# soldasim/BOSS.jl

Measured on AMD Instinct MI355X. Metric: gp_posterior_updates_per_sec (+ acq_evals_per_sec), N=4096 d=8 fp64, higher is better.
Workload: dtype f64; 1 GPU; d=8 synthetic blackbox, GaussianProcess(Matern52) surrogate, N=4096 fp64 posterior update + ExpectedImprovement over 8192 candidates per GPU (BASELINE.json configs[1]+[2]); N=4096, d=8, M_per_gpu=8192, kernel=matern52, parallelism=single GPU: no exchange

## Files before the change

boss.jl_amd/api.py:

```python
from __future__ import annotations

import ctypes as C
import os
from typing import Optional, Sequence

import numpy as np

_HERE = os.path.dirname(os.path.abspath(__file__))
LIB_PATH = os.environ.get("BOSS_LIB_PATH") or os.path.join(_HERE, "libbosship.so")

BOSS_OK, BOSS_E_INVALID, BOSS_E_NO_DEVICE, BOSS_E_NOT_PD, BOSS_E_NEG_VAR, BOSS_E_NOT_FITTED, BOSS_E_ALLOC = range(7)
KERNELS = {"matern32": 0, "matern52": 1, "sqexp": 2}
FIT_NO_SYNC = 1

_c_dp = C.POINTER(C.c_double)
_c_ucp = C.POINTER(C.c_ubyte)

SIGNATURES = {
    "boss_version": (C.c_char_p, []),
    "boss_last_error": (C.c_char_p, []),
    "boss_device_count": (C.c_int, [C.POINTER(C.c_int)]),
    "boss_set_stream": (C.c_int, [C.c_int, C.c_void_p]),
    "boss_device_sync": (C.c_int, [C.c_int]),
    "boss_gp_create": (C.c_int, [C.c_int, C.c_int, C.c_int, C.c_int, _c_dp, _c_dp, _c_ucp, C.POINTER(C.c_void_p)]),
# ... 1942 lines not shown
    def _set_args(self, gps, Xs, mean_Xs, mean_grad):
        S = len(gps)
        P = len(gps[0]) if S else 0
        if S < 1 or P < 1 or any(len(row) != P for row in gps):
            raise BossError(BOSS_E_INVALID, "gps must be S rows of P posteriors")
        Xs = _f64(Xs, 2)
        du, M = Xs.shape
        dm = self.d_model if self.d_model is not None else du
        arr = (C.c_void_p * (P * S))()
        for s in range(S):
            for p in range(P):
                arr[p + P * s] = gps[s][p]._h
        ms = None if mean_Xs is None else np.ascontiguousarray(np.asarray(mean_Xs, dtype=np.float64).reshape(S, P, M))
        mg = None
        if mean_grad is not None:
            mg = np.ascontiguousarray(np.asarray(mean_grad, dtype=np.float64).reshape(S, P, dm, M).transpose(0, 1, 3, 2))
        return S, P, M, du, arr, Xs, ms, mg

    def predict(self, gps, Xs, mean_Xs=None):
        S, P, M, du, arr, Xs, ms, _ = self._set_args(gps, Xs, mean_Xs, None)
        mu, var = np.zeros((S, P, M)), np.zeros((S, P, M))
        bad = C.c_long(-1)
        try:
            _check(load_library().boss_warp_predict(self._h, P, S, arr, M, _dp(Xs), _dp(ms), _dp(mu), _dp(var), C.byref(bad)))
        except DomainError as e:
            e.bad_index = bad.value
            raise
        return mu, var

    def predict_grad(self, gps, Xs, mean_Xs=None, mean_grad=None):
        S, P, M, du, arr, Xs, ms, mg = self._set_args(gps, Xs, mean_Xs, mean_grad)
        mu, var = np.zeros((S, P, M)), np.zeros((S, P, M))
        dmu, dvar = np.zeros((S, P, M, du)), np.zeros((S, P, M, du))
        bad = C.c_long(-1)
        try:
            _check(load_library().boss_warp_predict_grad(self._h, P, S, arr, M, _dp(Xs), _dp(ms), _dp(mg), _dp(mu), _dp(var), _dp(dmu),
                                                         _dp(dvar), C.byref(bad)))
        except DomainError as e:
            e.bad_index = bad.value
            raise
        return mu, var, dmu.transpose(0, 1, 3, 2), dvar.transpose(0, 1, 3, 2)

    @staticmethod
    def _acq_args(fit_coefs, y_max, valid_mask):
        coefs = _f64(np.asarray(fit_coefs).reshape(-1), 1)
        ym = None if y_max is None else _f64(np.asarray(y_max).reshape(-1), 1)
        mask = None if valid_mask is None else np.ascontiguousarray(np.asarray(valid_mask, dtype=bool).astype(np.uint8))
        return coefs, ym, mask

    def acq_ei(self, gps, Xs, fit_coefs, y_max=None, best=None, valid_mask=None, mean_Xs=None, want_acq: bool = True):
        S, P, M, du, arr, Xs, ms, _ = self._set_args(gps, Xs, mean_Xs, None)
        coefs, ym, mask = self._acq_args(fit_coefs, y_max, valid_mask)
        acq = np.zeros(M) if want_acq else None
        am = C.c_long(-1)
        mx = C.c_double(0.0)
        _check(load_library().boss_acq_ei_warp(self._h, P, S, arr, M, _dp(Xs), _dp(ms), _dp(coefs), _dp(ym), 0 if best is None else 1,
                                               0.0 if best is None else float(best), _ucp(mask), _dp(acq), C.byref(am), C.byref(mx)))
        return acq, am.value, mx.value

    def acq_ei_grad(self, gps, Xs, fit_coefs, y_max=None, best=None, valid_mask=None, mean_Xs=None, mean_grad=None):
        S, P, M, du, arr, Xs, ms, mg = self._set_args(gps, Xs, mean_Xs, mean_grad)
        coefs, ym, mask = self._acq_args(fit_coefs, y_max, valid_mask)
        acq = np.zeros(M)
        dacq = np.zeros((du, M), order="F")
        _check(load_library().boss_acq_ei_grad_warp(self._h, P, S, arr, M, _dp(Xs), _dp(ms), _dp(mg), _dp(coefs), _dp(ym),
                                                    0 if best is None else 1, 0.0 if best is None else float(best), _ucp(mask), _dp(acq),
                                                    _dp(dacq)))
        return acq, dacq

    def workgroup(self, stage: int, n: int, grad: bool, d_model: int = 0):
        lib = load_library()
        lib.boss_debug_warp_block.restype = C.c_int
        lib.boss_debug_warp_block.argtypes = [C.c_void_p, C.c_int, C.c_int, C.c_int, C.c_int, C.POINTER(C.c_int)]
        lds = C.c_int(0)
        return lib.boss_debug_warp_block(self._h, int(stage), 1 if grad else 0, int(n), int(d_model), C.byref(lds)), lds.value

    def close(self):
        if self._h:
            load_library().boss_warp_free(self._h)
            self._h = C.c_void_p()

    def __del__(self):
        try:
            self.close()
        except Exception:
            pass


def init() -> int:
    n = C.c_int(0)
    _check(load_library().boss_init(C.byref(n)))
    return n.value


def comm_info():
    n, r = C.c_int(0), C.c_int(0)
    _check(load_library().boss_comm_info(C.byref(n), C.byref(r)))
    return n.value, bool(r.value)


def shutdown():
    load_library().boss_shutdown()


def multi_update(replicas: Sequence[GP], lengthscale, amplitude, noise_std, mean_X=None) -> float:
    G = len(replicas)
    arr = (C.c_void_p * G)(*[r._h for r in replicas])
    lam = _f64(np.asarray(lengthscale).reshape(-1), 1)
    if lam.shape[0] != replicas[0].d:
        raise BossError(BOSS_E_INVALID, "length(lengthscales) must equal x_dim")
    m = None if mean_X is None else _f64(np.asarray(mean_X).reshape(-1), 1)
    out = C.c_double(0.0)
    _check(load_library().boss_multi_gp_update(G, arr, _dp(lam), float(amplitude), float(noise_std), _dp(m), C.byref(out)))
    for r in replicas:
        r.logpdf = out.value
    return out.value


def _acq_common(P, S, M, fit_coefs, y_max, valid_mask, mean_Xs):
    coefs = _f64(np.asarray(fit_coefs).reshape(-1), 1)
    ym = None if y_max is None else _f64(np.asarray(y_max).reshape(-1), 1)
    mask = None if valid_mask is None else np.ascontiguousarray(np.asarray(valid_mask, dtype=bool).astype(np.uint8))
    ms = None
    if mean_Xs is not None:
        a = np.asarray(mean_Xs, dtype=np.float64).reshape(S, P, M)
        ms = np.ascontiguousarray(a.transpose(0, 2, 1))
    return coefs, ym, mask, ms


def multi_acq_ei(replicas: Sequence[Sequence[Sequence[GP]]], Xs, fit_coefs, y_max=None, best=None, valid_mask=None,
                 mean_Xs=None, want_acq: bool = True):
    G, S, P = len(replicas), len(replicas[0]), len(replicas[0][0])
    Xs = _f64(Xs, 2)
    M = Xs.shape[1]
    arr = (C.c_void_p * (G * S * P))()
    for g in range(G):
        for s in range(S):
            for p in range(P):
                arr[p + P * (s + S * g)] = replicas[g][s][p]._h
    coefs, ym, mask, ms = _acq_common(P, S, M, fit_coefs, y_max, valid_mask, mean_Xs)
    acq = np.zeros(M) if want_acq else None
    am, mx = C.c_long(-1), C.c_double(0.0)
    _check(load_library().boss_multi_acq_ei(G, P, S, arr, M, _dp(Xs), _dp(ms), _dp(coefs), _dp(ym), 0 if best is None else 1,
                                            0.0 if best is None else float(best), _ucp(mask), _dp(acq), C.byref(am), C.byref(mx)))
    return acq, am.value, mx.value


class MultiCandidates:

    def __init__(self, Xs, G: int):
        Xs = _f64(Xs, 2)
        self.d, self.M, self.G = Xs.shape[0], Xs.shape[1], int(G)
        self._h = C.c_void_p()
        _check(load_library().boss_multi_cand_create(self.G, self.d, self.M, _dp(Xs), C.byref(self._h)))

    def close(self):
        if getattr(self, "_h", None) is not None and self._h:
            load_library().boss_multi_cand_free(self._h)
            self._h = None

    def __del__(self):
        try:
            self.close()
        except Exception:
            pass


def multi_acq_ei_cand(replicas: Sequence[Sequence[Sequence[GP]]], cand: MultiCandidates, fit_coefs, y_max=None, best=None,
                      valid_mask=None, mean_Xs=None, want_acq: bool = True):
    G, S, P = len(replicas), len(replicas[0]), len(replicas[0][0])
    M = cand.M
    arr = (C.c_void_p * (G * S * P))()
    for g in range(G):
        for s in range(S):
            for p in range(P):
                arr[p + P * (s + S * g)] = replicas[g][s][p]._h
    coefs, ym, mask, ms = _acq_common(P, S, M, fit_coefs, y_max, valid_mask, mean_Xs)
    acq = np.zeros(M) if want_acq else None
    am, mx = C.c_long(-1), C.c_double(0.0)
    _check(load_library().boss_multi_acq_ei_cand(G, P, S, arr, cand._h, _dp(ms), _dp(coefs), _dp(ym), 0 if best is None else 1,
                                                 0.0 if best is None else float(best), _ucp(mask), _dp(acq), C.byref(am), C.byref(mx)))
    return acq, am.value, mx.value


def _multi_handles(fn_name, gps, Xs, fit_coefs, y_max, best, valid_mask, mean_Xs, want_acq):
    S, P = len(gps), len(gps[0])
    Xs = _f64(Xs, 2)
    M = Xs.shape[1]
    arr = (C.c_void_p * (P * S))()
    for s in range(S):
        for p in range(P):
            arr[p + P * s] = gps[s][p]._h
    coefs, ym, mask, ms = _acq_common(P, S, M, fit_coefs, y_max, valid_mask, mean_Xs)
    acq = np.zeros(M) if want_acq else None
    am, mx = C.c_long(-1), C.c_double(0.0)
    _check(getattr(load_library(), fn_name)(P, S, arr, M, _dp(Xs), _dp(ms), _dp(coefs), _dp(ym), 0 if best is None else 1,
                                            0.0 if best is None else float(best), _ucp(mask), _dp(acq), C.byref(am), C.byref(mx)))
    return acq, am.value, mx.value


def multi_acq_ei_outputs(gps: Sequence[Sequence[GP]], Xs, fit_coefs, y_max=None, best=None, valid_mask=None, mean_Xs=None,
                         want_acq: bool = True):
    return _multi_handles("boss_multi_acq_ei_outputs", gps, Xs, fit_coefs, y_max, best, valid_mask, mean_Xs, want_acq)


def multi_acq_ei_samples(gps: Sequence[Sequence[GP]], Xs, fit_coefs, y_max=None, best=None, valid_mask=None, mean_Xs=None,
                         want_acq: bool = True):
    return _multi_handles("boss_multi_acq_ei_samples", gps, Xs, fit_coefs, y_max, best, valid_mask, mean_Xs, want_acq)


def multi_loglike_batch(G: int, X, y, kernel, lengthscales, amplitudes, noise_stds, mean_X=None, discrete=None):
    X = _f64(X, 2)
    y = _f64(np.asarray(y).reshape(-1), 1)
    lam = _f64(lengthscales, 2)
    d, N = X.shape
    S = lam.shape[1]
    if lam.shape[0] != d:
        raise BossError(BOSS_E_INVALID, "lengthscales must be d×S")
    amp = _f64(np.asarray(amplitudes).reshape(-1), 1)
    sig = _f64(np.asarray(noise_stds).reshape(-1), 1)
    stride, m = 0, None
    if mean_X is not None:
        m = np.asarray(mean_X, dtype=np.float64)
        if m.ndim == 2:
            m, stride = np.ascontiguousarray(m), N
        else:
            m = np.ascontiguousarray(m.reshape(-1))
    disc = None if discrete is None else np.ascontiguousarray(np.asarray(discrete, dtype=bool).astype(np.uint8))
    ll = np.zeros(S)
    st = np.zeros(S, dtype=np.int32)
    _check(load_library().boss_multi_loglike_batch(G, _kernel_id(kernel), d, N, _dp(X), _dp(y), _dp(m), stride, _ucp(disc), S,
                                                   _dp(lam), _dp(amp), _dp(sig), _dp(ll), st.ctypes.data_as(C.POINTER(C.c_int))))
    return ll, st


def bench_mfma_f64(device: int = 0, iters: int = 20000) -> float:
    out = C.c_double(0.0)
    _check(load_library().boss_bench_mfma_f64(device, iters, C.byref(out)))
    return out.value


def prof_enable(device: int, on: bool):
    _check(load_library().boss_prof_enable(device, 1 if on else 0))


def prof_reset(device: int):
    _check(load_library().boss_prof_reset(device))


def prof_get(device: int, kernel_class: str):
    ms = C.c_double(0.0)
    n = C.c_long(0)
    _check(load_library().boss_prof_get(device, kernel_class.encode(), C.byref(ms), C.byref(n)))
    return ms.value, n.value


def _update_path(g: GP):
    lib = load_library()
    fn = lib.boss_debug_update_path
    fn.restype = C.c_int
    fn.argtypes = [C.c_void_p, C.POINTER(C.c_int), C.POINTER(C.c_int), C.POINTER(C.c_int)]
    ch, tm, fb = C.c_int(0), C.c_int(0), C.c_int(0)
    _check(fn(g._h, C.byref(ch), C.byref(tm), C.byref(fb)))
    return ch.value, tm.value, fb.value


def _append_path(g: GP) -> int:
    fn = load_library().boss_debug_append_path
    fn.restype = C.c_int
    fn.argtypes = [C.c_void_p, C.POINTER(C.c_int)]
    out = C.c_int(-1)
    _check(fn(g._h, C.byref(out)))
    return out.value


def _fallbacks(device: int = 0):
    lib = load_library()
    fn = lib.boss_debug_fallbacks
    fn.restype = C.c_int
    fn.argtypes = [C.c_int, C.POINTER(C.c_long), C.POINTER(C.c_int)]
    n, off = C.c_long(0), C.c_int(0)
    _check(fn(device, C.byref(n), C.byref(off)))
    return n.value, off.value


def _set_launches(device: int = 0):
    lib = load_library()
    fn = lib.boss_debug_set_launches
    fn.restype = C.c_int
    fn.argtypes = [C.c_int, C.POINTER(C.c_long), C.POINTER(C.c_long)]
    a, b = C.c_long(0), C.c_long(0)
    fn(device, C.byref(a), C.byref(b))
    return a.value, b.value


def _set_grad_launches(device: int = 0):
    lib = load_library()
    fn = lib.boss_debug_set_grad_launches
    fn.restype = C.c_int
    fn.argtypes = [C.c_int, C.POINTER(C.c_long)]
    a = C.c_long(0)
    fn(device, C.byref(a))
    return a.value
```

boss.jl_amd/csrc/bosship.hip:

```cpp
#include "../../include/bosship.h"

#include <hip/hip_runtime.h>

#include <algorithm>
#include <cmath>
#include <cstdint>
#include <cstdio>
#include <cstdlib>
#include <atomic>
#include <chrono>
#include <cstring>
#include <functional>
#include <limits>
#include <map>
#include <mutex>
#include <string>
#include <thread>
#include <vector>

#include "gp_kernels.hpp"
#include "potrf.hpp"
#include "chain.hpp"
#include "small_calls.hpp"
#include "rider.hpp"
#include "latent_kernels.hpp"
#include "nfit_kernels.hpp"
#include "fitness.hpp"
#include "mean_program.hpp"
#include "warp_kernels.hpp"

using namespace boss;

#ifndef BOSS_PRED_D
#define BOSS_PRED_D 10
#endif
typedef GemmDirect<4, 1, 4, 2, BOSS_PRED_D> PredG32;
typedef GemmDirect<4, 1, 2, 4, 4> PredG64;

static thread_local std::string g_last_error;
static int fail(int code, const std::string& msg) {
    g_last_error = msg;
    return code;
}
#define HIPCHK(expr)                                                                                     \
    do {                                                                                                 \
        hipError_t e_ = (expr);                                                                          \
        if (e_ != hipSuccess)                                                                            \
            return fail(e_ == hipErrorOutOfMemory ? BOSS_E_ALLOC : BOSS_E_NO_DEVICE,                     \
                        std::string(#expr) + ": " + hipGetErrorString(e_));                              \
    } while (0)

constexpr size_t PINNED_UP_OFF = 4096, PINNED_UP_BYTES = 1024 * 1024, PINNED_DOWN_OFF = PINNED_UP_OFF + PINNED_UP_BYTES,
                 PINNED_DOWN_BYTES = 512 * 1024, PINNED_BYTES = PINNED_DOWN_OFF + PINNED_DOWN_BYTES;

static bool release_cached_slabs();
static std::atomic<int> g_fail_allocs{0};
static hipError_t dev_malloc(void** p, size_t bytes) {
    static const bool poison = getenv("BOSS_POISON_ALLOC") && atoi(getenv("BOSS_POISON_ALLOC"));
    hipError_t e = hipErrorOutOfMemory;
    if (g_fail_allocs.load(std::memory_order_relaxed) > 0 && g_fail_allocs.fetch_sub(1) > 0) *p = nullptr;
    else e = hipMalloc(p, bytes);
    if (e != hipSuccess) (void)hipGetLastError();
    if (e != hipSuccess && release_cached_slabs()) {
        e = hipMalloc(p, bytes);
        if (e != hipSuccess) (void)hipGetLastError();
    }
    if (e == hipSuccess && poison) {
        (void)hipMemset(*p, 0xff, bytes);
        (void)hipDeviceSynchronize();
    }
    return e;
}

constexpr size_t MULTI_RES_OFF = 384;
constexpr size_t FEW_RES_OFF = 400;

struct Workspace {
    void* p = nullptr;
    size_t bytes = 0;
};

struct Ctx {
    int device = -1;
    int logical = -1;
    hipStream_t own_stream = nullptr;
    hipStream_t stream = nullptr;
    hipStream_t side_stream = nullptr;
    std::vector<hipEvent_t> ev_panel, ev_rest;
    hipEvent_t ev_fork = nullptr, ev_up = nullptr;
    unsigned long long* sig_panel = nullptr;
    unsigned long long* sig_panel_host = nullptr;
    unsigned long long sig_seq = 0;
    hipStream_t chain_stream = nullptr, strip_stream = nullptr;
    unsigned long long chain_seq = 0, crit_seq = 0, up_seq = 0;
    int n_cus = 256;
    bool chain_ok = false;
    bool test_drop_chain = false;
    unsigned long long acq_seq = 0;
    unsigned long long few_seq = 0;
    std::mutex slab_mtx;
    void* slab_cache = nullptr;
    size_t slab_cache_bytes = 0;
    void* hostblk_cache = nullptr;
    size_t hostblk_cache_bytes = 0;
    unsigned long long* few_done = nullptr;
    unsigned long long few_done_cnt = 0;
    long set_launches = 0, set_pre_launches = 0;
    long set_grad_launches = 0;
    bool lookahead = true;
    bool prof_on = false;
    std::map<std::string, std::vector<std::pair<hipEvent_t, hipEvent_t>>> prof;
    std::vector<hipEvent_t> ev_pool;
    Workspace vscratch, csc, pred, acq, batchA, batchX, batchMisc, craw, lgA, lgB, lgC, few, setdesc, setmom, gsetdesc, nlatjobs, mceps, meanws, warpws;
    static constexpr int LLG_BANKS = 4;
    Workspace lgbank[LLG_BANKS - 1][3];
    hipStream_t llg_stream[LLG_BANKS - 1] = {nullptr, nullptr, nullptr};
    hipEvent_t llg_join[LLG_BANKS - 1] = {nullptr, nullptr, nullptr};
    void* pinned = nullptr;
    struct TrailTab {
        TrailWork* dev = nullptr;
        std::vector<TrailWork> host;
        std::vector<int> off;
    };
    TrailTab trail[65];
    std::mutex mtx;
};

static void chain_quiesce(Ctx* c) {
    if (c->chain_stream) (void)hipStreamSynchronize(c->chain_stream);
    if (c->strip_stream) (void)hipStreamSynchronize(c->strip_stream);
}

static std::mutex g_ctx_mtx;
static std::map<int, Ctx*> g_ctx;

static bool release_cached_slabs() {
    int dev = -1;
    if (hipGetDevice(&dev) != hipSuccess) return false;
    std::vector<void*> blocks;
    {
        std::lock_guard<std::mutex> lk(g_ctx_mtx);
        for (auto& kv : g_ctx) {
            Ctx* c = kv.second;
            if (c->device != dev) continue;
            std::lock_guard<std::mutex> sl(c->slab_mtx);
            if (c->slab_cache) blocks.push_back(c->slab_cache);
            c->slab_cache = nullptr;
            c->slab_cache_bytes = 0;
        }
    }
    for (void* b : blocks) (void)hipFree(b);
    return !blocks.empty();
}
extern "C" int boss_debug_fail_next_alloc(int n) {
    g_fail_allocs.store(n > 0 ? n : 0);
    return BOSS_OK;
}
extern "C" int boss_debug_slab_cache_bytes(int device, size_t* bytes_out) {
    std::lock_guard<std::mutex> lk(g_ctx_mtx);
    auto it = g_ctx.find(device);
    if (bytes_out) *bytes_out = 0;
    if (it != g_ctx.end() && bytes_out) {
        std::lock_guard<std::mutex> sl(it->second->slab_mtx);
        *bytes_out = it->second->slab_cache_bytes;
    }
    return BOSS_OK;
}

extern "C" int boss_debug_set_launches(int device, long* all_out, long* pre_out) {
    std::lock_guard<std::mutex> lk(g_ctx_mtx);
    auto it = g_ctx.find(device);
    if (all_out) *all_out = it != g_ctx.end() ? it->second->set_launches : 0;
    if (pre_out) *pre_out = it != g_ctx.end() ? it->second->set_pre_launches : 0;
    return BOSS_OK;
}

extern "C" int boss_debug_set_grad_launches(int device, long* out) {
    std::lock_guard<std::mutex> lk(g_ctx_mtx);
    auto it = g_ctx.find(device);
    if (out) *out = it != g_ctx.end() ? it->second->set_grad_launches : 0;
    return BOSS_OK;
}

static void ctx_destroy(Ctx* c) {
    if (!c) return;
    if (c->own_stream) (void)hipStreamDestroy(c->own_stream);
    if (c->side_stream) (void)hipStreamDestroy(c->side_stream);
    if (c->chain_stream) (void)hipStreamDestroy(c->chain_stream);
    if (c->strip_stream) (void)hipStreamDestroy(c->strip_stream);
    if (c->ev_fork) (void)hipEventDestroy(c->ev_fork);
    if (c->sig_panel && !c->sig_panel_host) (void)hipFree(c->sig_panel);
    if (c->few_done) (void)hipFree(c->few_done);
    for (auto& t : c->trail)
        if (t.dev) (void)hipFree(t.dev);
    if (c->slab_cache) (void)hipFree(c->slab_cache);
    if (c->hostblk_cache) (void)hipHostFree(c->hostblk_cache);
    if (c->ev_up) (void)hipEventDestroy(c->ev_up);
    for (int i = 0; i < Ctx::LLG_BANKS - 1; ++i) {
        if (c->llg_stream[i]) (void)hipStreamDestroy(c->llg_stream[i]);
        if (c->llg_join[i]) (void)hipEventDestroy(c->llg_join[i]);
    }
    if (c->pinned) (void)hipHostFree(c->pinned);
    delete c;
}

static int ctx_init(Ctx* c) {
    {
        int least = 0, greatest = 0;
        (void)hipDeviceGetStreamPriorityRange(&least, &greatest);
        static const int cu_mask = getenv("BOSS_CU_MASK") ? atoi(getenv("BOSS_CU_MASK")) : 0;
        if (cu_mask) {
            hipDeviceProp_t prop;
            HIPCHK(hipGetDeviceProperties(&prop, c->device));
            const int ncu = prop.multiProcessorCount, words = (ncu + 31) / 32;
            auto make = [&](hipStream_t* st, int lo, int hi) {
                std::vector<uint32_t> m(words, 0u);
                for (int b = lo; b < hi && b < ncu; ++b) m[b / 32] |= 1u << (b % 32);
                return hipExtStreamCreateWithCUMask(st, (uint32_t)words, m.data());
            };
            HIPCHK(make(&c->chain_stream, 0, 16));
            HIPCHK(make(&c->strip_stream, 16, 32));
            HIPCHK(make(&c->own_stream, 32, ncu));
            HIPCHK(make(&c->side_stream, cu_mask >= 2 ? 40 : 32, cu_mask >= 2 ? ncu : ncu - 8));
            c->stream = c->own_stream;
            std::fprintf(stderr, "[bosship] BOSS_CU_MASK=%d: chain on CU bits 0-15, strips on 16-31, main stream on 32-%d, side stream %d-%d\n",
                         cu_mask, ncu - 1, cu_mask >= 2 ? 40 : 32, (cu_mask >= 2 ? ncu : ncu - 8) - 1);
        } else {
        HIPCHK(hipStreamCreateWithPriority(&c->own_stream, hipStreamNonBlocking, greatest));
        c->stream = c->own_stream;
        HIPCHK(hipStreamCreateWithPriority(&c->side_stream, hipStreamNonBlocking, least));
        HIPCHK(hipStreamCreateWithPriority(&c->chain_stream, hipStreamNonBlocking, greatest));
        HIPCHK(hipStreamCreateWithPriority(&c->strip_stream, hipStreamNonBlocking, greatest));
        }
    }
    HIPCHK(hipEventCreateWithFlags(&c->ev_fork, hipEventDisableTiming));
    HIPCHK(hipEventCreateWithFlags(&c->ev_up, hipEventDisableTiming));
    for (int i = 0; i < Ctx::LLG_BANKS - 1; ++i) {
        HIPCHK(hipStreamCreateWithFlags(&c->llg_stream[i], hipStreamNonBlocking));
        HIPCHK(hipEventCreateWithFlags(&c->llg_join[i], hipEventDisableTiming));
    }
    c->lookahead = !(getenv("BOSS_NO_LOOKAHEAD") && atoi(getenv("BOSS_NO_LOOKAHEAD")));
    {
        auto set_nonzero = [](const char* name) {
            const char* v = getenv(name);
            return v && *v && std::strcmp(v, "0") != 0;
        };
        static const bool gate_off = set_nonzero("BOSS_NO_GATE") || set_nonzero("ROCPROF_COUNTER_COLLECTION") || getenv("ROCPROF_COUNTERS") ||
                                     getenv("ROCPROF_COUNTER_GROUPS") || set_nonzero("ROCPROF_ADVANCED_THREAD_TRACE") ||
                                     getenv("ROCPROF_ATT_PARAM_SERIALIZE_ALL") || getenv("ROCP_METRICS") || set_nonzero("AMD_SERIALIZE_KERNEL");
        if (!gate_off) {
            if (set_nonzero("BOSS_DEBUG_WATCH")) {
                unsigned long long* hp = nullptr;
                HIPCHK(hipHostMalloc((void**)&hp, SIG_WORDS * sizeof(unsigned long long), hipHostMallocMapped));
                std::memset(hp, 0, SIG_WORDS * sizeof(unsigned long long));
                HIPCHK(hipHostGetDevicePointer((void**)&c->sig_panel, hp, 0));
                c->sig_panel_host = hp;
#ifdef BOSS_DEBUG_WATCH_BUILD
                HIPCHK(hipMemcpyToSymbol(HIP_SYMBOL(boss::g_dbg), &c->sig_panel, sizeof(void*)));
#endif
                std::thread([hp]() {
                    unsigned long long last[SIG_WORDS] = {0};
                    for (;;) {
                        std::this_thread::sleep_for(std::chrono::milliseconds(500));
                        unsigned long long now[SIG_WORDS];
                        for (int i = 0; i < SIG_WORDS; ++i) now[i] = ((volatile unsigned long long*)hp)[i];
                        if (std::memcmp(now, last, sizeof now) == 0) continue;
                        std::memcpy(last, now, sizeof now);
                        std::fprintf(stderr, "[bosship watch] up %llu wdone %llu panel %llu crit %llu | gate %llu near %llu bulk %llu | strips",
                                     now[SIGW_UP], now[SIGW_WDONE], now[SIGW_PANEL], now[SIGW_CRIT], now[SIGW_GATE], now[SIGW_NEAR], now[SIGW_BULK]);
                        for (int q = 0; q < 8; ++q) std::fprintf(stderr, " %llu", now[SIGW_PROG + SIGW_PROG_STRIDE * q]);
                        std::fprintf(stderr, " | give-ups: first %llu n %llu last %llu; waits ended by mark %llu, by clock %llu", now[SIGW_DBG], now[SIGW_DBG + 1],
                                     now[SIGW_DBG + 2], now[SIGW_DBG + 4], now[SIGW_DBG + 5]);
                        std::fprintf(stderr, "\n");
                    }
                }).detach();
            } else {
                HIPCHK(hipMalloc((void**)&c->sig_panel, SIG_WORDS * sizeof(unsigned long long)));
                HIPCHK(hipMemset(c->sig_panel, 0, SIG_WORDS * sizeof(unsigned long long)));
            }
        }
        c->chain_ok = !gate_off && !set_nonzero("BOSS_NO_CHAIN") && !set_nonzero("HIP_LAUNCH_BLOCKING");
        c->test_drop_chain = set_nonzero("BOSS_TEST_DROP_CHAIN");
        if (c->chain_ok) {
            int* okw = nullptr;
            HIPCHK(hipMalloc((void**)&okw, 4 * sizeof(int)));
            HIPCHK(hipMemset(okw, 0, 4 * sizeof(int)));
            hipStream_t probed[4] = {c->own_stream, c->side_stream, c->chain_stream, c->strip_stream};
            for (int i = 0; i < 4; ++i)
                hipLaunchKernelGGL(chain_probe_wait_kernel, dim3(1), dim3(64), 0, probed[i], c->sig_panel + SIGW_NEAR + 1, 4ull, okw + i);
            int okh[4] = {0, 0, 0, 0};
            bool fine = hipDeviceSynchronize() == hipSuccess && hipMemcpy(okh, okw, sizeof okh, hipMemcpyDeviceToHost) == hipSuccess;
            (void)hipFree(okw);
            if (!(fine && okh[0] && okh[1] && okh[2] && okh[3])) c->chain_ok = false;
            if (getenv("BOSS_CHAIN_VERBOSE"))
                std::fprintf(stderr, "[bosship] resident chain: %s (main / side / chain / strip streams side by side: %d %d %d %d)\n",
                             c->chain_ok ? "on" : "off", okh[0], okh[1], okh[2], okh[3]);
        }
    }
    HIPCHK(hipHostMalloc(&c->pinned, PINNED_BYTES, hipHostMallocDefault));
    std::memset(c->pinned, 0, PINNED_UP_OFF);
    HIPCHK(hipFuncSetAttribute((const void*)potrf_diag_kernel, hipFuncAttributeMaxDynamicSharedMemorySize, DIAG_LDS_BYTES));
    HIPCHK(hipFuncSetAttribute((const void*)potrf_chain_kernel, hipFuncAttributeMaxDynamicSharedMemorySize, CHAIN_LDS_BYTES));
    HIPCHK(hipFuncSetAttribute((const void*)potrf_strips_kernel, hipFuncAttributeMaxDynamicSharedMemorySize, STRIPS_LDS_BYTES));
    {
        int cus = 0;
        if (hipDeviceGetAttribute(&cus, hipDeviceAttributeMultiprocessorCount, c->device) != hipSuccess) cus = 0;
        if (cus > 0) c->n_cus = cus;
    }
    HIPCHK(hipFuncSetAttribute((const void*)small_fit_kernel, hipFuncAttributeMaxDynamicSharedMemorySize, SMALL_LDS_BYTES));
    HIPCHK(hipFuncSetAttribute((const void*)small_llgrad_kernel, hipFuncAttributeMaxDynamicSharedMemorySize, SMALL_LLG_LDS_BYTES));
    HIPCHK(hipFuncSetAttribute((const void*)small_fit_batch_kernel, hipFuncAttributeMaxDynamicSharedMemorySize, SMALL_LDS_BYTES));
    HIPCHK(hipFuncSetAttribute((const void*)small_predict_grad_kernel<true>, hipFuncAttributeMaxDynamicSharedMemorySize, SPG_LDS_BYTES));
    HIPCHK(hipFuncSetAttribute((const void*)small_predict_grad_kernel<false>, hipFuncAttributeMaxDynamicSharedMemorySize, SPG_LDS_BYTES));
    HIPCHK(hipFuncSetAttribute((const void*)potrf_syrk_kernel<2, true>, hipFuncAttributeMaxDynamicSharedMemorySize, 96 * 1024));
    HIPCHK(hipFuncSetAttribute((const void*)rider_step_kernel, hipFuncAttributeMaxDynamicSharedMemorySize, 96 * 1024));
    HIPCHK(hipFuncSetAttribute((const void*)predict_kernel<PredG32>, hipFuncAttributeMaxDynamicSharedMemorySize,
                               PredictLds<PredG32>::BYTES));
    HIPCHK(hipFuncSetAttribute((const void*)predict_kernel_set<PredG32>, hipFuncAttributeMaxDynamicSharedMemorySize,
                               PredictLds<PredG32>::BYTES));
    HIPCHK(hipFuncSetAttribute((const void*)grad_accum_kernel, hipFuncAttributeMaxDynamicSharedMemorySize, 150 * 1024));
    HIPCHK(hipFuncSetAttribute((const void*)winv_gemv_kernel<1>, hipFuncAttributeMaxDynamicSharedMemorySize, 150 * 1024));
    HIPCHK(hipFuncSetAttribute((const void*)winv_gemv_kernel<2>, hipFuncAttributeMaxDynamicSharedMemorySize, 150 * 1024));
    HIPCHK(hipFuncSetAttribute((const void*)winv_gemv_kernel<4>, hipFuncAttributeMaxDynamicSharedMemorySize, 150 * 1024));
    HIPCHK(hipFuncSetAttribute((const void*)winv_args_kernel<1>, hipFuncAttributeMaxDynamicSharedMemorySize, 150 * 1024));
    HIPCHK(hipFuncSetAttribute((const void*)winv_args_kernel<2>, hipFuncAttributeMaxDynamicSharedMemorySize, 150 * 1024));
    HIPCHK(hipFuncSetAttribute((const void*)winv_args_kernel<4>, hipFuncAttributeMaxDynamicSharedMemorySize, 150 * 1024));
    HIPCHK(hipFuncSetAttribute((const void*)winv_args_kernel<1, true>, hipFuncAttributeMaxDynamicSharedMemorySize, 150 * 1024));
    HIPCHK(hipFuncSetAttribute((const void*)few_back_finish_kernel<PredG32>, hipFuncAttributeMaxDynamicSharedMemorySize,
                               PredictLds<PredG32>::BYTES));
    HIPCHK(hipFuncSetAttribute((const void*)few_w_kernel<PredG32>, hipFuncAttributeMaxDynamicSharedMemorySize, PredictLds<PredG32>::BYTES));
    HIPCHK(hipFuncSetAttribute((const void*)few_finish_kernel<PredG32>, hipFuncAttributeMaxDynamicSharedMemorySize,
                               PredictLds<PredG32>::BYTES));
    HIPCHK(hipFuncSetAttribute((const void*)linvt_kernel<PredG32>, hipFuncAttributeMaxDynamicSharedMemorySize,
                               PredictLds<PredG32>::BYTES));
    HIPCHK(hipFuncSetAttribute((const void*)backsolve_kernel<PredG32>, hipFuncAttributeMaxDynamicSharedMemorySize,
                               PredictLds<PredG32>::BYTES));
    HIPCHK(hipFuncSetAttribute((const void*)backsolve_set_kernel<PredG32>, hipFuncAttributeMaxDynamicSharedMemorySize,
                               PredictLds<PredG32>::BYTES));
    HIPCHK(hipFuncSetAttribute((const void*)grad_accum_set_kernel, hipFuncAttributeMaxDynamicSharedMemorySize, 150 * 1024));
    HIPCHK(hipFuncSetAttribute((const void*)predict_kernel<PredG64>, hipFuncAttributeMaxDynamicSharedMemorySize,
                               PredictLds<PredG64>::BYTES));
    HIPCHK(hipFuncSetAttribute((const void*)predict_kernel<PredG32, true>, hipFuncAttributeMaxDynamicSharedMemorySize,
                               PredictLds<PredG32>::BYTES));
    HIPCHK(hipFuncSetAttribute((const void*)predict_kernel<PredG64, true>, hipFuncAttributeMaxDynamicSharedMemorySize,
                               PredictLds<PredG64>::BYTES));
    HIPCHK(hipFuncSetAttribute((const void*)ei_mc_grad_set_kernel, hipFuncAttributeMaxDynamicSharedMemorySize, MC_GRAD_MAX_LDS));
    HIPCHK(hipFuncSetAttribute((const void*)mean_eval_kernel<true>, hipFuncAttributeMaxDynamicSharedMemorySize, MEAN_MAX_LDS));
    return BOSS_OK;
}

static int virtual_devices() {
    static const int v = getenv("BOSS_VIRTUAL_DEVICES") ? std::max(0, atoi(getenv("BOSS_VIRTUAL_DEVICES"))) : 0;
    return v;
}
static int visible_devices(int* nphys_out = nullptr) {
    int n = 0;
    if (hipGetDeviceCount(&n) != hipSuccess || n <= 0) return 0;
    if (nphys_out) *nphys_out = n;
    return virtual_devices() > 0 ? virtual_devices() : n;
}

static int get_ctx(int device, Ctx** out) {
    std::lock_guard<std::mutex> lk(g_ctx_mtx);
    auto it = g_ctx.find(device);
    if (it != g_ctx.end()) {
        *out = it->second;
        HIPCHK(hipSetDevice(it->second->device));
        return BOSS_OK;
    }
    int nphys = 0;
    const int n = visible_devices(&nphys);
    if (n <= 0) return fail(BOSS_E_NO_DEVICE, "no HIP device visible (bosship has no CPU fallback)");
    if (device < 0 || device >= n) return fail(BOSS_E_INVALID, "device index out of range");
    const int phys = device % nphys;
    HIPCHK(hipSetDevice(phys));
    Ctx* c = new Ctx();
    c->device = phys;
    c->logical = device;
    int rc = ctx_init(c);
    if (rc) {
        ctx_destroy(c);
        return rc;
    }
    g_ctx[device] = c;
    *out = c;
    return BOSS_OK;
}

static int ws_reserve(Workspace& w, size_t bytes) {
    if (w.bytes >= bytes) return BOSS_OK;
    if (w.p) (void)hipFree(w.p);
    w.p = nullptr;
    w.bytes = 0;
    HIPCHK(dev_malloc(&w.p, bytes));
    w.bytes = bytes;
    return BOSS_OK;
}

struct ProfScope {
    Ctx* c;
    hipEvent_t e0 = nullptr, e1 = nullptr;
    const char* name;
    ProfScope(Ctx* ctx, const char* n) : c(ctx), name(n) {
        if (!c->prof_on) return;
        e0 = take();
        e1 = take();
        (void)hipEventRecord(e0, c->stream);
    }
    ~ProfScope() {
        if (!c->prof_on) return;
        (void)hipEventRecord(e1, c->stream);
        c->prof[name].push_back({e0, e1});
    }
    hipEvent_t take() {
        if (!c->ev_pool.empty()) {
            hipEvent_t e = c->ev_pool.back();
            c->ev_pool.pop_back();
            return e;
        }
        hipEvent_t e;
        (void)hipEventCreate(&e);
        return e;
    }
};

struct boss_gpset {
    Ctx* ctx = nullptr;
    std::atomic<int> refs{0};
    void* slab = nullptr;
    void* host_block = nullptr;
    size_t slab_bytes = 0, host_bytes = 0;
};
static bool slab_cache_on() {
    static const bool v = !(getenv("BOSS_SLAB_CACHE") && atoi(getenv("BOSS_SLAB_CACHE")) == 0) &&
                          !(getenv("BOSS_POISON_ALLOC") && atoi(getenv("BOSS_POISON_ALLOC")));
    return v;
}
static void gpset_release_storage(boss_gpset* st) {
    Ctx* c = st->ctx;
    void *slab = st->slab, *hb = st->host_block;
    if (c && slab_cache_on()) {
        std::lock_guard<std::mutex> lk(c->slab_mtx);
        if (slab && st->slab_bytes > c->slab_cache_bytes) {
            std::swap(slab, c->slab_cache);
            c->slab_cache_bytes = st->slab_bytes;
        }
        if (hb && st->host_bytes > c->hostblk_cache_bytes) {
            std::swap(hb, c->hostblk_cache);
            c->hostblk_cache_bytes = st->host_bytes;
        }
    }
    if (slab) (void)hipFree(slab);
    if (hb) (void)hipHostFree(hb);
    st->slab = st->host_block = nullptr;
}

struct boss_gp {
    Ctx* ctx = nullptr;
    boss_gpset* set = nullptr;
    int kernel = 0, d = 0, N = 0, Np = 0, nblk = 0, ld = 0;
    double *Xraw = nullptr, *Xsc = nullptr, *y = nullptr, *mean = nullptr, *A = nullptr;
    double *LT = nullptr, *DT2 = nullptr, *avec = nullptr;
    bool have_lt = false;
    double *inv16 = nullptr, *Dinv = nullptr, *Dinv2 = nullptr, *hyp = nullptr, *invlam = nullptr, *scal = nullptr;
    int* info = nullptr;
    unsigned char* discrete_dev = nullptr;
    std::vector<unsigned char> discrete;
    double amp2 = 0.0;
    bool has_mean = false, fitted = false, pending = false, have_dinv = false;
    bool dinv_used = false;
    bool dinv_used_prev = false;
    bool gated = false;
    bool chained = false;
    bool fell_back = false;
    int trail_used = -1;
    double* host_res = nullptr;
    double* host_res_dev = nullptr;
    bool par_in_args = false;
    unsigned long long res_seq = 0;
    bool res_polled = false;
    double* host_par = nullptr;
    hipEvent_t par_ev = nullptr;
    unsigned long long epoch = 0;
    unsigned long long factor_gen = 0, dinv0_gen = ~0ull;
    hipEvent_t dinv_ev = nullptr;
    bool dinv_pending = false;
    bool aug = false;
    int npts = 0, ldx = 0, nhead = 0;
    bool gibbs = false;
    double *lamX = nullptr, *ampX = nullptr, *noiseX = nullptr;
    double *Winv = nullptr, *Linv = nullptr;
    double* W2 = nullptr;
    int w2_np = 0;
    unsigned long long w2_gen = ~0ull;
    bool w2_used = false;
    bool have_winv = false;
    int few_calls = 0;
    int append_calls = 0;
    int append_path = 0;
};

struct boss_cand {
    Ctx* ctx = nullptr;
    int d = 0, M = 0, Mp = 0;
    double* Craw = nullptr;
};

struct boss_track {
    Ctx* ctx = nullptr;
    boss_gp* gp = nullptr;
    int d = 0, M = 0, Mp = 0, tiles = 0, Ncap = 0, N = 0;
    unsigned long long epoch = 0;
    double *V = nullptr, *Csc = nullptr, *mu = nullptr, *var = nullptr, *mean = nullptr;
    bool has_mean = false;
    bool gibbs = false;
    double *Clam = nullptr, *Camp = nullptr;
    bool aug = false;
};

static inline int round_up(int x, int m) { return (x + m - 1) / m * m; }
struct SetBatch {
    int nb = 1;
    size_t sA = 0, sInv16 = 0, sDinv = 0, sDinv2 = 0, sW = 0, sX = 0;
    size_t sPar = 0;
};
struct MeanFold {
    const double* J = nullptr;
    size_t sJ = 0;
    int T = 0;
    double* dmean = nullptr;
    double* dtheta = nullptr;
};
static void linv_enqueue(boss_gp* g, hipStream_t s, double* U, double* Lw, const SetBatch& B = SetBatch());
constexpr int MAX_ROWS = 46080;

extern "C" const char* boss_version(void) { return "bosship 0.1.0 (gfx950, fp64 MFMA)"; }
extern "C" const char* boss_last_error(void) { return g_last_error.c_str(); }

extern "C" int boss_device_count(int* n_out) {
    const int n = visible_devices();
    hipError_t e = n > 0 ? hipSuccess : hipErrorNoDevice;
    if (e != hipSuccess || n <= 0) {
        if (n_out) *n_out = 0;
        return fail(BOSS_E_NO_DEVICE, "no HIP device visible (bosship has no CPU fallback)");
    }
    if (n_out) *n_out = n;
    return BOSS_OK;
}

extern "C" int boss_set_stream(int device, void* hip_stream) {
    Ctx* c;
    int rc = get_ctx(device, &c);
    if (rc) return rc;
    std::lock_guard<std::mutex> lk(c->mtx);
    HIPCHK(hipStreamSynchronize(c->stream));
    c->stream = hip_stream ? (hipStream_t)hip_stream : c->own_stream;
    return BOSS_OK;
}

extern "C" int boss_device_sync(int device) {
    Ctx* c;
    int rc = get_ctx(device, &c);
    if (rc) return rc;
    HIPCHK(hipStreamSynchronize(c->stream));
    return BOSS_OK;
}

static bool few_done_ensure(Ctx* c, hipStream_t s) {
    if (c->few_done) return true;
    if (hipMalloc((void**)&c->few_done, sizeof(unsigned long long)) != hipSuccess) {
        (void)hipGetLastError();
        c->few_done = nullptr;
        return false;
    }
    (void)hipMemsetAsync(c->few_done, 0, sizeof(unsigned long long), s);
    c->few_done_cnt = 0;
    return true;
}
static bool few_fused() {
    static const bool v = !(getenv("BOSS_FEW_FUSED") && atoi(getenv("BOSS_FEW_FUSED")) == 0);
    return v;
}

#include "host_factor.inc"
#include "host_append.inc"
#include "host_batch.inc"
#include "host_latent.inc"
#include "host_nfit.inc"
struct McEpi {
    const FitProg* g;
    int n_eps;
    const double* eps;
};
static int mc_stage(Ctx* c, hipStream_t s, int P, const McEpi& mc, const double** deps_out);
static void mc_accumulate_launch(hipStream_t s, const double* mu, const double* var, size_t sstride, int ldm, int M, int s0, int s1, int S_total,
                                 const EiPar& par, const McEpi& mc, const double* deps, double* acq_sum, int add);
static void mc_grad_launch(hipStream_t s, const double* mu, const double* var, const double* dmu, const double* dvar, int M, int d, int S,
                           const EiPar& par, const McEpi& mc, const double* deps, const unsigned char* mask, double* acq, double* dacq);
#include "host_predict.inc"
#include "host_acq.inc"
#include "host_fitness.inc"
#include "host_mean.inc"
#include "host_warp.inc"
#include "host_rider.inc"
#include "host_track.inc"
#include "host_multi.inc"

extern "C" int boss_bench_mfma_f64(int device, int iters, double* tflops_out) {
    Ctx* c;
    int rc = get_ctx(device, &c);
    if (rc) return rc;
    hipDeviceProp_t prop;
    HIPCHK(hipGetDeviceProperties(&prop, device));
    const int blocks = prop.multiProcessorCount;
    double* sink;
    HIPCHK(dev_malloc((void**)&sink, 8));
    hipEvent_t e0, e1;
    HIPCHK(hipEventCreate(&e0));
    HIPCHK(hipEventCreate(&e1));
    hipLaunchKernelGGL(mfma_f64_rate_kernel, dim3(blocks), dim3(256), 0, c->stream, iters / 8 + 1, sink);
    HIPCHK(hipEventRecord(e0, c->stream));
    hipLaunchKernelGGL(mfma_f64_rate_kernel, dim3(blocks), dim3(256), 0, c->stream, iters, sink);
    HIPCHK(hipEventRecord(e1, c->stream));
    HIPCHK(hipEventSynchronize(e1));
    float ms = 0.f;
    HIPCHK(hipEventElapsedTime(&ms, e0, e1));
    const double flops = (double)blocks * 4.0 * (double)iters * 16.0 * 2048.0;
    if (tflops_out) *tflops_out = flops / (ms * 1e-3) / 1e12;
    (void)hipEventDestroy(e0);
    (void)hipEventDestroy(e1);
    (void)hipFree(sink);
    return BOSS_OK;
}

extern "C" int boss_prof_enable(int device, int on) {
    Ctx* c;
    int rc = get_ctx(device, &c);
    if (rc) return rc;
    c->prof_on = on != 0;
    return BOSS_OK;
}

extern "C" int boss_prof_reset(int device) {
    Ctx* c;
    int rc = get_ctx(device, &c);
    if (rc) return rc;
    HIPCHK(hipStreamSynchronize(c->stream));
    for (auto& kv : c->prof)
        for (auto& pr : kv.second) {
            c->ev_pool.push_back(pr.first);
            c->ev_pool.push_back(pr.second);
        }
    c->prof.clear();
    return BOSS_OK;
}

extern "C" int boss_prof_get(int device, const char* kernel_class, double* ms_total, long* launches) {
    Ctx* c;
    int rc = get_ctx(device, &c);
    if (rc) return rc;
    if (!kernel_class) return fail(BOSS_E_INVALID, "kernel_class is NULL");
    HIPCHK(hipStreamSynchronize(c->stream));
    double tot = 0.0;
    long n = 0;
    auto it = c->prof.find(kernel_class);
    if (it != c->prof.end()) {
        for (auto& pr : it->second) {
            float ms = 0.f;
            if (hipEventElapsedTime(&ms, pr.first, pr.second) == hipSuccess) tot += ms;
            ++n;
        }
    }
    if (ms_total) *ms_total = tot;
    if (launches) *launches = n;
    return BOSS_OK;
}

extern "C" int boss_debug_colupd_decode(int G, int k, int m, int ncols, int jfirst, int skipdiag, int xblk, int critical,
                                        int* R0, int* C0, int* crit) {
    if (G < 1 || !R0 || !C0 || !crit) return fail(BOSS_E_INVALID, "bad argument");
    for (int t = 0; t < G; ++t) {
        const ColupdWork w = colupd_decode(t, G, k, m, ncols, jfirst, skipdiag, xblk, critical != 0);
        R0[t] = w.R0;
        C0[t] = w.C0;
        crit[t] = w.crit;
    }
    return BOSS_OK;
}

extern "C" int boss_debug_trail_plan(int nblk, int panels, int lag, int* n_items, int* off, int* items, int cap) {
    if (nblk < 2 || nblk > 64 || panels < 1 || panels > 8 || lag < 1 || lag > 8 || !n_items || !off) return fail(BOSS_E_INVALID, "bad argument");
    std::vector<TrailWork> plan;
    std::vector<int> o;
    trail_plan(nblk, panels, lag, plan, o);
    *n_items = (int)plan.size();
    for (int k = 0; k < nblk; ++k) off[k] = o[k];
    if (!items) return BOSS_OK;
    if (cap < (int)plan.size()) return fail(BOSS_E_INVALID, "cap too small");
    for (size_t t = 0; t < plan.size(); ++t) {
        const TrailWork& w = plan[t];
        int* it = items + 5 * t;
        it[0] = w.R0;
        it[1] = w.C0;
        it[2] = w.k0;
        it[3] = w.npc & 255;
        it[4] = w.npc >> 8;
    }
    return BOSS_OK;
}

extern "C" int boss_debug_update_path(const boss_gp* g, int* chained, int* trail_mode, int* fell_back) {
    if (!g || !chained || !trail_mode || !fell_back) return fail(BOSS_E_INVALID, "bad argument");
    *chained = g->chained ? 1 : 0;
    *trail_mode = g->chained ? g->trail_used : -1;
    *fell_back = g->fell_back ? 1 : 0;
    return BOSS_OK;
}

#ifdef BOSS_CHAIN_TRACE
extern "C" int boss_debug_ctrace(unsigned long long* chain , unsigned long long* colupd , int reset) {
    if (hipDeviceSynchronize() != hipSuccess) return 1;
    if (chain && hipMemcpyFromSymbol(chain, HIP_SYMBOL(boss::g_ctrace), sizeof(unsigned long long) * 64 * 16) != hipSuccess) return 1;
    if (colupd && hipMemcpyFromSymbol(colupd, HIP_SYMBOL(boss::g_cutrace), sizeof(unsigned long long) * 64 * 4) != hipSuccess) return 1;
    if (colupd && hipMemcpyFromSymbol(colupd + 64 * 4, HIP_SYMBOL(boss::g_ptrace), sizeof(unsigned long long) * 64 * 32) != hipSuccess) return 1;
    if (reset) {
        static unsigned long long a[64 * 16], b[64 * 4];
        for (int i = 0; i < 64; ++i) {
            for (int j = 0; j < 16; ++j) a[i * 16 + j] = (j == 5) ? ~0ull : 0ull;
            b[i * 4 + 0] = ~0ull;
            b[i * 4 + 1] = b[i * 4 + 2] = b[i * 4 + 3] = 0;
        }
        (void)hipMemcpyToSymbol(HIP_SYMBOL(boss::g_ctrace), a, sizeof a);
        (void)hipMemcpyToSymbol(HIP_SYMBOL(boss::g_cutrace), b, sizeof b);
    }
    return 0;
}
extern "C" int boss_debug_rtrace(unsigned long long* rider , int reset) {
    if (hipDeviceSynchronize() != hipSuccess) return 1;
    if (rider && hipMemcpyFromSymbol(rider, HIP_SYMBOL(boss::g_rtrace), sizeof(unsigned long long) * 64 * 4) != hipSuccess) return 1;
    if (reset) {
        static unsigned long long a[64 * 4];
        for (int i = 0; i < 64; ++i) {
            a[i * 4 + 0] = ~0ull;
            a[i * 4 + 1] = a[i * 4 + 2] = a[i * 4 + 3] = 0;
        }
        (void)hipMemcpyToSymbol(HIP_SYMBOL(boss::g_rtrace), a, sizeof a);
    }
    return 0;
}
#endif
```

boss.jl_amd/csrc/host_acq.inc:

```

static int acq_ei_impl(int P, int S, boss_gp_t* const* gps, const boss_cand_t* cand, const double* mean_Xs,
                       const double* fit_coefs, const double* y_max, int has_best, double best,
                       const unsigned char* valid_mask, double* acq_out, long* argmax_out, double* max_out,
                       double* dpair, long idx_off, bool defer, const McEpi* mc = nullptr) {
    if (P < 1 || S < 1 || !gps || !cand || (!fit_coefs && !mc)) return fail(BOSS_E_INVALID, "bad arguments");
    Ctx* c = cand->ctx;
    HIPCHK(hipSetDevice(c->device));
    for (int i = 0; i < P * S; ++i) {
        if (!gps[i]) return fail(BOSS_E_INVALID, "NULL posterior handle");
        if (gps[i]->ctx != c) return fail(BOSS_E_INVALID, "all handles and candidates must live on one device");
        if (!gps[i]->fitted) return fail(BOSS_E_NOT_FITTED, "handle has no valid factorisation");
    }
    std::lock_guard<std::mutex> lk(c->mtx);
    hipStream_t s = c->stream;
    const int M = cand->M;
    const size_t nd = (size_t)3 * P * M + M + 2 * P;
    {
        int rc = ws_reserve(c->acq, sizeof(double) * nd + M);
        if (rc) return rc;
    }
    double* dev = (double*)c->acq.p;
    double* dmu = dev;
    double* dvar = dmu + (size_t)P * M;
    double* dacq = dvar + (size_t)P * M;
    double* dmean = dacq + M;
    double* dcoef = dmean + (size_t)P * M;
    double* dymax = dcoef + P;
    unsigned char* dmask = (unsigned char*)(dev + nd);
    double* hres = (double*)c->pinned + (defer ? MULTI_RES_OFF : 0);
    EiPar par;
    const double no_coefs[EI_MAXP] = {};
    int rc = ei_params(c, s, P, mc ? no_coefs : fit_coefs, y_max, has_best, best, &par, dcoef, dymax);
    if (rc) return rc;
    const double* deps = nullptr;
    if (mc) {
        rc = mc_stage(c, s, P, *mc, &deps);
        if (rc) return rc;
    }
    EiPar par0 = par;
    par0.mode = 0;
    if (valid_mask) (void)hipMemcpyAsync(dmask, valid_mask, M, hipMemcpyHostToDevice, s);
    if (S > 1) (void)hipMemsetAsync(dacq, 0, sizeof(double) * M, s);
    std::vector<double> hmean;
    static const bool set_off = getenv("BOSS_NO_SET_PREDICT") && atoi(getenv("BOSS_NO_SET_PREDICT"));
    if (S > 1 && par.mode != 0 && !set_off && predict_set_ok(P * S, gps, cand)) {
        const size_t pm = (size_t)P * M;
        rc = ws_reserve(c->setmom, sizeof(double) * pm * S * (mean_Xs ? 3 : 2));
        if (rc) return rc;
        double* mu_all = (double*)c->setmom.p;
        double* var_all = mu_all + pm * S;
        double* mean_all = mean_Xs ? var_all + pm * S : nullptr;
        if (mean_Xs) {
            hmean.resize(pm * S);
            for (int sm = 0; sm < S; ++sm)
                for (int j = 0; j < M; ++j)
                    for (int p = 0; p < P; ++p) hmean[pm * sm + (size_t)p * M + j] = mean_Xs[p + (size_t)P * (j + (size_t)M * sm)];
            (void)hipMemcpyAsync(mean_all, hmean.data(), sizeof(double) * pm * S, hipMemcpyHostToDevice, s);
            (void)hipStreamSynchronize(s);
        }
        rc = predict_set_enqueue(P * S, gps, cand, mean_all, mu_all, var_all, (size_t)M);
        if (rc) {
            (void)hipStreamSynchronize(s);
            return rc;
        }
        if (mc) mc_accumulate_launch(s, mu_all, var_all, pm, M, M, 0, S, S, par, *mc, deps, dacq, 0);
        else
        hipLaunchKernelGGL(ei_accumulate_set_kernel, dim3((M + 255) / 256), dim3(256), 0, s, (const double*)mu_all, (const double*)var_all, pm, M, M,
                           0, S - 1, par, dcoef, dymax, dacq);
        hipLaunchKernelGGL(acq_epilogue_kernel, dim3(1), dim3(ACQ_EPI_THREADS), 0, s, (const double*)(mu_all + pm * (S - 1)),
                           (const double*)(var_all + pm * (S - 1)), M, M, mc ? par0 : par, dcoef, dymax, dacq, 1, 1.0 / S, valid_mask ? dmask : nullptr, hres,
                           (acq_out || defer) ? 0ull : ++c->acq_seq, dpair, idx_off);
    } else
    for (int sm = 0; sm < S; ++sm) {
        if (par.mode != 0) {
            if (mean_Xs) {
                hmean.resize((size_t)P * M);
                for (int j = 0; j < M; ++j)
                    for (int p = 0; p < P; ++p) hmean[(size_t)p * M + j] = mean_Xs[p + (size_t)P * (j + (size_t)M * sm)];
                (void)hipMemcpyAsync(dmean, hmean.data(), sizeof(double) * P * M, hipMemcpyHostToDevice, s);
                (void)hipStreamSynchronize(s);
            }
            for (int p = 0; p < P; ++p) {
                rc = predict_enqueue(gps[p + (size_t)P * sm], cand, mean_Xs ? dmean + (size_t)p * M : nullptr,
                                     dmu + (size_t)p * M, dvar + (size_t)p * M);
                if (rc) {
                    (void)hipStreamSynchronize(s);
                    return rc;
                }
            }
        }
        ProfScope ps(c, sm + 1 < S ? "ei" : "argmax");
        if (mc) {
            mc_accumulate_launch(s, dmu, dvar, 0, M, M, 0, 1, S, par, *mc, S > 1 ? deps + (size_t)sm * P : deps, dacq, sm > 0 ? 1 : 0);
            if (sm + 1 == S)
                hipLaunchKernelGGL(acq_epilogue_kernel, dim3(1), dim3(ACQ_EPI_THREADS), 0, s, dmu, dvar, M, M, par0, dcoef, dymax, dacq, 1, 1.0 / S,
                                   valid_mask ? dmask : nullptr, hres, (acq_out || defer) ? 0ull : ++c->acq_seq, dpair, idx_off);
        } else if (sm + 1 < S)
            hipLaunchKernelGGL(ei_accumulate_kernel, dim3((M + 255) / 256), dim3(256), 0, s, dmu, dvar, M, M, par, dcoef, dymax,
                               dacq);
        else
            hipLaunchKernelGGL(acq_epilogue_kernel, dim3(1), dim3(ACQ_EPI_THREADS), 0, s, dmu, dvar, M, M, par, dcoef, dymax,
                               dacq, S > 1 ? 1 : 0, 1.0 / S, valid_mask ? dmask : nullptr, hres, (acq_out || defer) ? 0ull : ++c->acq_seq,
                               dpair, idx_off);
    }
    if (acq_out) (void)hipMemcpyAsync(acq_out, dacq, sizeof(double) * M, hipMemcpyDeviceToHost, s);
    if (defer) {
        hipError_t e0 = hipGetLastError();
        return e0 == hipSuccess ? BOSS_OK : fail(BOSS_E_NO_DEVICE, hipGetErrorString(e0));
    }
    bool got = false;
    if (!acq_out) {
        volatile unsigned long long* seq = reinterpret_cast<volatile unsigned long long*>(hres) + 2;
        for (unsigned long i = 1;; ++i) {
            if (*seq == c->acq_seq) {
                got = true;
                break;
            }
            if ((i & 0x3fff) == 0 && hipStreamQuery(s) != hipErrorNotReady) break;
        }
        std::atomic_thread_fence(std::memory_order_acquire);
    }
    hipError_t e = got ? hipSuccess : hipStreamSynchronize(s);
    hipError_t e2 = hipGetLastError();
    if (e != hipSuccess) return fail(BOSS_E_NO_DEVICE, hipGetErrorString(e));
    if (e2 != hipSuccess) return fail(BOSS_E_NO_DEVICE, hipGetErrorString(e2));
    if (argmax_out) std::memcpy(argmax_out, &hres[1], sizeof(long));
    if (max_out) *max_out = hres[0];
    return BOSS_OK;
}

extern "C" int boss_acq_ei(int P, int S, boss_gp_t* const* gps, const boss_cand_t* cand, const double* mean_Xs,
                           const double* fit_coefs, const double* y_max, int has_best, double best,
                           const unsigned char* valid_mask, double* acq_out, long* argmax_out, double* max_out) {
    return acq_ei_impl(P, S, gps, cand, mean_Xs, fit_coefs, y_max, has_best, best, valid_mask, acq_out, argmax_out, max_out, nullptr, 0, false);
}

extern "C" int boss_acq_ei_moments(int device, int P, int S, int M, const double* mu, const double* var,
                                   const double* fit_coefs, const double* y_max, int has_best, double best,
                                   const unsigned char* valid_mask, double* acq_out, long* argmax_out,
                                   double* max_out) {
    if (P < 1 || S < 1 || M < 1 || !mu || !var || !fit_coefs) return fail(BOSS_E_INVALID, "bad arguments");
    Ctx* c;
    int rc = get_ctx(device, &c);
    if (rc) return rc;
    HIPCHK(hipSetDevice(c->device));
    std::lock_guard<std::mutex> lk(c->mtx);
    hipStream_t s = c->stream;
    const size_t pm = (size_t)P * M;
    const size_t nd = 2 * pm * S + M + 2 * P;
    rc = ws_reserve(c->acq, sizeof(double) * nd + M);
    if (rc) return rc;
    double* dev = (double*)c->acq.p;
    double* dmu = dev;
    double* dvar = dmu + pm * S;
    double* dacq = dvar + pm * S;
    double* dcoef = dacq + M;
    double* dymax = dcoef + P;
    unsigned char* dmask = (unsigned char*)(dev + nd);
    double* hres = (double*)c->pinned;
    EiPar par;
    rc = ei_params(c, s, P, fit_coefs, y_max, has_best, best, &par, dcoef, dymax);
    if (rc) return rc;
    (void)hipMemcpyAsync(dmu, mu, sizeof(double) * pm * S, hipMemcpyHostToDevice, s);
    (void)hipMemcpyAsync(dvar, var, sizeof(double) * pm * S, hipMemcpyHostToDevice, s);
    if (valid_mask) (void)hipMemcpyAsync(dmask, valid_mask, M, hipMemcpyHostToDevice, s);
    if (S > 1) (void)hipMemsetAsync(dacq, 0, sizeof(double) * M, s);
    for (int sm = 0; sm + 1 < S; ++sm)
        hipLaunchKernelGGL(ei_accumulate_kernel, dim3((M + 255) / 256), dim3(256), 0, s, dmu + pm * sm, dvar + pm * sm, M, M, par,
                           dcoef, dymax, dacq);
    hipLaunchKernelGGL(acq_epilogue_kernel, dim3(1), dim3(ACQ_EPI_THREADS), 0, s, dmu + pm * (S - 1), dvar + pm * (S - 1), M, M,
                       par, dcoef, dymax, dacq, S > 1 ? 1 : 0, 1.0 / S, valid_mask ? dmask : nullptr, hres, 0ull);
    if (acq_out) (void)hipMemcpyAsync(acq_out, dacq, sizeof(double) * M, hipMemcpyDeviceToHost, s);
    hipError_t e = hipStreamSynchronize(s);
    if (e != hipSuccess) return fail(BOSS_E_NO_DEVICE, hipGetErrorString(e));
    if (argmax_out) std::memcpy(argmax_out, &hres[1], sizeof(long));
    if (max_out) *max_out = hres[0];
    return BOSS_OK;
}

static int llgrad_enqueue(boss_gp* g, hipStream_t s, double* sums_out, int bank, const SetBatch& B, const double* amp2_dev,
                          int amp2_stride, const MeanFold* mf) {
    Ctx* c = g->ctx;
    const int d = g->d, N = g->N, Np = g->Np, ld = g->ld, nb = B.nb;
    const int nt = Np / 64, ntiles = nt * (nt + 1) / 2, nv = g->aug ? d + 3 : d + 2, nch = 8;
    const int gibbs_js = std::max(1, std::min(16, Np / 64));
    const size_t sW = (size_t)ld * Np,
                 sC = (size_t)nch * Np + (g->gibbs ? (size_t)gibbs_js * 4 * (d + 1) * Np : (size_t)ntiles * nv);
    Workspace &wA = bank ? c->lgbank[bank - 1][0] : c->lgA, &wB = bank ? c->lgbank[bank - 1][1] : c->lgB,
              &wC = bank ? c->lgbank[bank - 1][2] : c->lgC;
    int rc = ws_reserve(wA, sizeof(double) * sW * nb);
    if (rc) return rc;
    rc = ws_reserve(wB, sizeof(double) * sW * nb);
    if (rc) return rc;
    rc = ws_reserve(wC, sizeof(double) * sC * nb);
    if (rc) return rc;
    double* LinvT = (double*)wA.p;
    double* Kinv = (double*)wB.p;
    double* apart = (double*)wC.p;
    double* parts = apart + (size_t)nch * Np;
    SetBatch Bw = B;
    Bw.sW = nb > 1 ? sW : 0;
    dinv_join(g);
    if (!g->have_dinv) {
        dinv_launch(g, s, B);
        g->have_dinv = true;
    }
    g->dinv_used = true;
    typedef PredG32 G;
    static const bool linvt_solve = getenv("BOSS_LINVT_SOLVE") && atoi(getenv("BOSS_LINVT_SOLVE"));
    if (linvt_solve && nb == 1) {
        hipLaunchKernelGGL(linvt_kernel<G>, dim3(Np / 32), dim3(G::NTHREADS), PredictLds<G>::BYTES, s, (const double*)g->A, ld, Np,
                           (const double*)g->Dinv2, LinvT, ld);
    } else {
        linv_enqueue(g, s, LinvT, Kinv, Bw);
    }
    hipLaunchKernelGGL(kinv_syrk_kernel<SyrkG>, dim3(g->nblk * (g->nblk + 1) / 2, 1, nb), dim3(256), 0, s, (const double*)LinvT, ld, Np,
                       Kinv, ld, Bw.sW);
    hipLaunchKernelGGL(avec_partial_kernel, dim3(Np / 256, nch, nb), dim3(256), 0, s, (const double*)LinvT, ld, Np, N,
                       (const double*)g->A, ld, apart, Bw.sW, B.sA, nb > 1 ? sC : (size_t)0);
    if (mf && (mf->dmean || (mf->dtheta && mf->T > 0))) {
        const int T = mf->dtheta ? mf->T : 0;
        hipLaunchKernelGGL(mean_fold_kernel, dim3(std::max(1, (T + MFOLD_COLS - 1) / MFOLD_COLS), 1, nb), dim3(MFOLD_THREADS), 0, s,
                           (const double*)apart, nch, Np, N, T ? mf->J : (const double*)nullptr, T, mf->dmean, T ? mf->dtheta : (double*)nullptr,
                           nb > 1 ? sC : (size_t)0, mf->sJ);
    }
    const size_t zC = nb > 1 ? sC : (size_t)0, zPar = nb > 1 ? B.sPar : (size_t)0;
    if (g->gibbs) {
        hipLaunchKernelGGL(mirror_lower_kernel, dim3(Np / 64, Np / 64, nb), dim3(256), 0, s, Kinv, ld, Np, Bw.sW);
        hipLaunchKernelGGL(mirror_diag_kernel, dim3(Np / 64, 1, nb), dim3(256), 0, s, Kinv, ld, Bw.sW);
        hipLaunchKernelGGL(gibbs_llgrad_kernel, dim3(Np / 64, gibbs_js, nb), dim3(256), 0, s, (const double*)g->Xraw, (const double*)g->lamX,
                           (const double*)g->ampX, d, N, Np, (const double*)Kinv, ld, (const double*)apart, nch, parts, zPar, Bw.sW, zC);
        hipLaunchKernelGGL(gibbs_llgrad_reduce_kernel, dim3((Np + 255) / 256, 1, nb), dim3(256), 0, s, (const double*)parts, gibbs_js * 4, d, N,
                           Np, (const double*)g->noiseX, (const double*)Kinv, ld, (const double*)apart, nch, sums_out, zPar, Bw.sW, zC,
                           nb > 1 ? (size_t)(d + 3) * Np : (size_t)0);
        return BOSS_OK;
    }
    if (g->aug)
        hipLaunchKernelGGL(aug_llgrad_tile_kernel, dim3(ntiles, 1, nb), dim3(256), 0, s, (const double*)g->Xraw, g->ldx, d, g->nhead, N, Np,
                           g->kernel, (const double*)g->hyp, (const double*)g->invlam, zPar, (const double*)Kinv, ld, (const double*)apart, nch,
                           parts, Bw.sW, zC);
    else
    hipLaunchKernelGGL(llgrad_tile_kernel, dim3(ntiles, 1, nb), dim3(256), 0, s, (const double*)g->Xsc, d, N, Np, g->kernel, amp2_dev,
                       amp2_stride, (const double*)Kinv, ld, (const double*)apart, nch, parts, B.sX, Bw.sW, nb > 1 ? sC : (size_t)0,
                       nb > 1 ? sC : (size_t)0);
    hipLaunchKernelGGL(llgrad_reduce_kernel, dim3(nv, 1, nb), dim3(256), 0, s, (const double*)parts, ntiles, nv, sums_out,
                       nb > 1 ? sC : (size_t)0, (size_t)nv);
    return BOSS_OK;
}

static void llgrad_finalize(int d, int N, const double* invlam, double amp2, double sig2, double zz, const double* h, double* grad_out) {
    const double amp = std::sqrt(amp2), sig = std::sqrt(sig2), trK = h[d], aa = h[d + 1];
    for (int m = 0; m < d; ++m) grad_out[m] = -h[m] * invlam[m];
    grad_out[d] = (zz - N - sig2 * (aa - trK)) / amp;
    grad_out[d + 1] = sig * (aa - trK);
}

static int llgrad_download(boss_gp* g, std::vector<double>& h, size_t n_mean = 0) {
    Ctx* c = g->ctx;
    hipStream_t s = c->stream;
    int rc = ws_reserve(c->pred, sizeof(double) * h.size());
    if (rc) return rc;
    double* sums = (double*)c->pred.p;
    MeanFold mf;
    if (n_mean) mf.dmean = sums + (h.size() - n_mean);
    rc = llgrad_enqueue(g, s, sums, 0, SetBatch(), g->gibbs ? (const double*)nullptr : (const double*)g->hyp, 0, n_mean ? &mf : nullptr);
    if (rc) return rc;
    HIPCHK(hipMemcpyAsync(h.data(), sums, sizeof(double) * h.size(), hipMemcpyDeviceToHost, s));
    HIPCHK(hipStreamSynchronize(s));
    HIPCHK(hipGetLastError());
    return BOSS_OK;
}

extern "C" int boss_gp_loglike_grad(boss_gp_t* g, double* logpdf_out, double* grad_out) {
    if (!g || !grad_out) return fail(BOSS_E_INVALID, "NULL argument");
    NOT_FOR_AUG(g);
    Ctx* c = g->ctx;
    HIPCHK(hipSetDevice(c->device));
    std::lock_guard<std::mutex> lk(c->mtx);
    int rc = gp_settle(g);
    if (rc) return rc;
    const int d = g->d, nv = d + 2;
    if (d > LLG_MAX_D) return fail(BOSS_E_INVALID, "x_dim too large for the likelihood-gradient kernel");
    hipStream_t s = c->stream;
    if (small_fit_ok(c, g->N, d) && !g->gibbs) {
        dinv_join(g);
        hipLaunchKernelGGL(small_llgrad_kernel, dim3(1), dim3(DIAG_THREADS), SMALL_LLG_LDS_BYTES, s, (const double*)g->A, g->ld, g->Np,
                           g->N, d, g->kernel, g->amp2, (const double*)g->inv16, (const double*)g->Xsc, g->ldx, g->host_res_dev + 8, (size_t)0, (size_t)0,
                           (size_t)0, (const double*)nullptr, 0, 0, ++g->res_seq, (const double*)nullptr, 0, (size_t)0, (double*)nullptr,
                           (double*)nullptr);
        HIPCHK(hipGetLastError());
        {
            volatile unsigned long long* seq = reinterpret_cast<volatile unsigned long long*>(g->host_res + 7);
            bool got = false;
            for (unsigned long i = 1;; ++i) {
                if (*seq == g->res_seq) {
                    got = true;
                    break;
                }
                if ((i & 0x3fff) == 0 && hipStreamQuery(s) != hipErrorNotReady) break;
            }
            std::atomic_thread_fence(std::memory_order_acquire);
            if (!got) HIPCHK(hipStreamSynchronize(s));
        }
        llgrad_finalize(d, g->N, g->host_par, g->host_par[d], g->host_par[d + 1], g->host_res[1], g->host_res + 8, grad_out);
        if (logpdf_out) *logpdf_out = loglik(g->N, g->host_res[0], g->host_res[1]);
        return BOSS_OK;
    }
    std::vector<double> h(nv);
    rc = llgrad_download(g, h);
    if (rc) return rc;
    llgrad_finalize(d, g->N, g->host_par, g->host_par[d], g->host_par[d + 1], g->host_res[1], h.data(), grad_out);
    if (logpdf_out) *logpdf_out = loglik(g->N, g->host_res[0], g->host_res[1]);
    return BOSS_OK;
}

extern "C" int boss_gp_loglike_grad_mean(boss_gp_t* g, double* logpdf_out, double* grad_out, double* dmean_out) {
    if (!g || !grad_out || !dmean_out) return fail(BOSS_E_INVALID, "NULL argument");
    NOT_FOR_AUG(g);
    Ctx* c = g->ctx;
    HIPCHK(hipSetDevice(c->device));
    std::lock_guard<std::mutex> lk(c->mtx);
    int rc = gp_settle(g);
    if (rc) return rc;
    const int d = g->d, nv = d + 2, N = g->N;
    if (d > LLG_MAX_D) return fail(BOSS_E_INVALID, "x_dim too large for the likelihood-gradient kernel");
    hipStream_t s = c->stream;
    std::vector<double> h((size_t)nv + N);
    if (small_fit_ok(c, N, d)) {
        rc = ws_reserve(c->pred, sizeof(double) * h.size());
        if (rc) return rc;
        double* sums = (double*)c->pred.p;
        dinv_join(g);
        hipLaunchKernelGGL(small_llgrad_kernel, dim3(1), dim3(DIAG_THREADS), SMALL_LLG_LDS_BYTES, s, (const double*)g->A, g->ld, g->Np, N, d,
                           g->kernel, g->amp2, (const double*)g->inv16, (const double*)g->Xsc, g->ldx, sums, (size_t)0, (size_t)0, (size_t)0,
                           (const double*)nullptr, 0, 0, 0ull, (const double*)nullptr, 0, (size_t)0, sums + nv, (double*)nullptr);
        HIPCHK(hipGetLastError());
        HIPCHK(hipMemcpyAsync(h.data(), sums, sizeof(double) * h.size(), hipMemcpyDeviceToHost, s));
        HIPCHK(hipStreamSynchronize(s));
    } else {
        rc = llgrad_download(g, h, (size_t)N);
        if (rc) return rc;
    }
    llgrad_finalize(d, N, g->host_par, g->host_par[d], g->host_par[d + 1], g->host_res[1], h.data(), grad_out);
    std::copy(h.begin() + nv, h.end(), dmean_out);
    if (logpdf_out) *logpdf_out = loglik(N, g->host_res[0], g->host_res[1]);
// ... 53 lines not shown
```

boss.jl_amd/csrc/host_factor.inc:

```


struct LaunchStamps {
    static constexpr int CAP = 512;
    int n = 0;
    int tag[CAP];
    std::chrono::steady_clock::time_point t[CAP];
    void reset() { n = 0; }
    void add(int what) {
        if (n < CAP) {
            tag[n] = what;
            t[n++] = std::chrono::steady_clock::now();
        }
    }
};
static std::atomic<int> g_stamps_on{-1};
static std::atomic<long long> g_stall_us{2500};
static std::mutex g_stall_mtx;
static std::string g_stall_log;
static bool launch_stamps_on() {
    int v = g_stamps_on.load(std::memory_order_relaxed);
    if (v < 0) {
        v = (getenv("BOSS_LAUNCH_STAMPS") && atoi(getenv("BOSS_LAUNCH_STAMPS"))) ? 1 : 0;
        if (getenv("BOSS_STALL_MS")) g_stall_us.store((long long)(atof(getenv("BOSS_STALL_MS")) * 1000.0));
        g_stamps_on.store(v);
// ... 173 lines not shown
    p.cbase = c->chain_seq;
    c->chain_seq += 8ull * nblk + 16;
    p.critbase = c->crit_seq;
    c->crit_seq += 8ull * (nblk - 2);
#ifdef BOSS_EXPERIMENTS
    static const bool drop_chain = getenv("BOSS_EXP_DROP_CHAIN") && atoi(getenv("BOSS_EXP_DROP_CHAIN"));
#else
    constexpr bool drop_chain = false;
#endif
    if (!(drop_chain || c->test_drop_chain)) {
        const unsigned budget = poll_budget_ticks(Np);
        hipLaunchKernelGGL(potrf_chain_kernel, dim3(2), dim3(DIAG_THREADS), CHAIN_LDS_BYTES, c->chain_stream, A, ld, nblk, inv16, info, c->sig_panel,
                           p.cbase, p.critbase, budget);
        hipLaunchKernelGGL(potrf_strips_kernel, dim3(8), dim3(TRSM_THREADS), STRIPS_LDS_BYTES, c->strip_stream, A, ld, nblk, (const double*)inv16,
                           c->sig_panel, p.cbase, p.critbase, info, budget);
        c->up_seq += 2 + 8;
        p.up_want = c->up_seq;
    }
    return p;
}
static void chain_ready(Ctx* c, const ChainPlan& p, int Np, int* info) {
    if (!p.on || c->test_drop_chain) return;
    static const int force = getenv("BOSS_CHAIN_READY") ? atoi(getenv("BOSS_CHAIN_READY")) : -1;
    const int followers = (Np - 2 * BLK) / 16 + 1;
    const bool need = followers + 16 > c->n_cus;
    if (force == 0 || (force < 0 && !need)) return;
    hipLaunchKernelGGL(chain_ready_kernel, dim3(1), dim3(64), 0, c->stream, c->sig_panel, p.up_want, info, poll_budget_ticks(Np));
}
static void potrf_enqueue(Ctx* c, double* A, int ld, int Np, int batch, size_t bstride, double* inv16,
                          size_t inv16_bstride, int* info, bool gates = true, const ChainPlan* plan = nullptr,
                          const std::function<void(int)>* step_hook = nullptr) {
    const int nblk = Np / BLK;
    hipStream_t s = c->stream;
    const unsigned budget = poll_budget_ticks(Np);
    if (Np > 8192) gates = false;
    static const int pair_min_batch = getenv("BOSS_PAIR_MIN_BATCH") ? atoi(getenv("BOSS_PAIR_MIN_BATCH")) : 4;
    static const int la_batch_max = getenv("BOSS_LA_BATCH_MAX") ? atoi(getenv("BOSS_LA_BATCH_MAX")) : 8;
    const bool la_batch = batch <= la_batch_max && c->lookahead && !c->prof_on && nblk >= 3;
    if (batch >= pair_min_batch && nblk >= 3 && !la_batch) {
        for (int k = 0; k < nblk; k += 2) {
            for (int kk = k; kk < k + 2 && kk < nblk; ++kk) {
                {
                    ProfScope ps(c, "potrf_diag");
                    hipLaunchKernelGGL(potrf_diag_kernel, dim3(1, 1, batch), dim3(DIAG_THREADS), DIAG_LDS_BYTES, s, A, ld, bstride,
                                       kk, inv16, inv16_bstride, info, (unsigned long long*)nullptr, 0ull);
                }
                const int nrows16 = (Np - (kk + 1) * BLK) / 16 + 1;
                {
                    ProfScope ps(c, "potrf_trsm");
                    hipLaunchKernelGGL(potrf_trsm_kernel, dim3(nrows16, 1, batch), dim3(TRSM_THREADS), 0, s, A, ld, bstride, kk, inv16,
                                       inv16_bstride, (kk + 1) * BLK);
                }
                const int m = nblk - 1 - kk;
                if (kk == k && m > 0) {
                    ProfScope ps(c, "potrf_syrk");
                    hipLaunchKernelGGL(potrf_colupd_kernel, dim3(4 * m + 1, 1, batch), dim3(256), 0, s, A, ld, bstride, kk, m, 1, 0, 1, (unsigned long long*)nullptr, 0ull, info, 0, -1, (unsigned long long*)nullptr, budget);
                }
            }
            const int m2 = nblk - (k + 2);
            if (m2 > 0) {
                ProfScope ps(c, "potrf_syrk");
                hipLaunchKernelGGL(potrf_syrk_kernel<2>, dim3((m2 * (m2 + 1) / 2 + m2) * batch, 1, 1), dim3(256), 0, s, A, ld, bstride,
                                   k, k + 2, m2, batch);
            } else if (m2 == 0 && k + 1 < nblk) {
            }
        }
        return;
    }
    const bool la = c->lookahead && !c->prof_on && nblk >= 3;
    if (la) {
        while ((int)c->ev_panel.size() < nblk) {
            hipEvent_t e0, e1;
            (void)hipEventCreateWithFlags(&e0, hipEventDisableTiming);
            (void)hipEventCreateWithFlags(&e1, hipEventDisableTiming);
            c->ev_panel.push_back(e0);
            c->ev_rest.push_back(e1);
        }
    }
    const int small_m = sched_small_m();
    const bool no_pairs = sched_no_pairs();
    const bool chain = plan && plan->on;
    const unsigned long long cbase = chain ? plan->cbase : 0;
    unsigned long long* const critw = chain ? c->sig_panel + SIGW_CRIT : nullptr;
    auto launch_follow = [&](int kk, unsigned long long gateval) {
        const int row0 = std::min((kk + 2) * BLK, Np);
        const int nrows16 = (Np - row0) / 16 + 1;
        hipLaunchKernelGGL(potrf_follow_kernel, dim3(nrows16), dim3(TRSM_THREADS), 0, s, A, ld, kk, (const double*)inv16, row0,
                           kk + 1 < nblk ? 1 : 0, c->sig_panel, cbase, gateval, info, budget);
        BOSS_STAMP(1000 + kk);
    };
    int kstart = 0, tail_join = -1;
    unsigned long long pending_sig = 0;
    int gated_kk = 0, gated_m3 = 0;
    unsigned long long bulk_pub = 0;
    int bulk_pub_word = SIGW_BULK;
    unsigned long long far_pub = 0;
    std::function<void()> flush_gated_bulk = []() {};
    const int chain_trail = chain_trail_mode(nblk);
    const bool chain_inline = chain && chain_trail != 2;
    static const int pairs_until_env = getenv("BOSS_CHAIN_PAIRS_UNTIL") ? atoi(getenv("BOSS_CHAIN_PAIRS_UNTIL")) : -1;
    const int pairs_until = chain_trail == 1 ? nblk : (chain_trail == 0 && pairs_until_env > 0 ? pairs_until_env : 0);
    if (chain_inline && pairs_until > 0) {
        int k = 0;
        for (; k + 3 < nblk && k < pairs_until; k += 2) {
            launch_follow(k, 0);
            int m = nblk - 1 - k;
            hipLaunchKernelGGL(potrf_colupd_kernel, dim3(4 * m + 1 + 4, 1, 1), dim3(256), 0, s, A, ld, bstride, k, m, 1, 0, 1,
                               (unsigned long long*)nullptr, 0ull, info, 1, k + 2, critw, budget);
            if (step_hook) (*step_hook)(k);
            launch_follow(k + 1, 0);
            m = nblk - 2 - k;
            hipLaunchKernelGGL(potrf_colupd_kernel, dim3(2 * m * (m + 1) + m, 1, 1), dim3(256), 0, s, A, ld, bstride, k + 1, m, m, 0, 2,
                               (unsigned long long*)nullptr, 0ull, info, 1, -1, critw, budget);
            if (step_hook) (*step_hook)(k + 1);
        }
        kstart = k;
    }
    if (!chain_inline && la && !no_pairs && (batch == 1 || la_batch) && nblk - 1 > small_m + 2) {
        int last = -1;
        int k = 0;
        static const bool half_tiles = !(getenv("BOSS_BULK_HALF") && !atoi(getenv("BOSS_BULK_HALF")));
        static const int bulk_lds = (getenv("BOSS_BULK_LDS") ? atoi(getenv("BOSS_BULK_LDS")) : 81) * 1024;
        auto launch_bulk = [=](int kk, int m3, int first, int skip00) {
            if (half_tiles && batch == 1 && Np <= 8192) {
                hipLaunchKernelGGL((potrf_syrk_kernel<2, true>), dim3(m3 * (m3 + 1) / 2 + m3, 2, 1), dim3(256), bulk_lds, c->side_stream,
                                   A, ld, bstride, kk - 1, first, m3, 0, skip00);
            } else
                hipLaunchKernelGGL(potrf_syrk_kernel<2>, dim3(m3 * (m3 + 1) / 2 + m3, 1, batch), dim3(256), 0, c->side_stream, A, ld,
                                   bstride, kk - 1, first, m3, 0, skip00);
            (void)hipEventRecord(c->ev_rest[kk], c->side_stream);
        };
        static const bool split_off = getenv("BOSS_NO_BULK_SPLIT") && atoi(getenv("BOSS_NO_BULK_SPLIT"));
        flush_gated_bulk = [&, launch_bulk]() {
            if (!pending_sig) return;
            hipLaunchKernelGGL(potrf_gate_kernel, dim3(1), dim3(64), 0, c->side_stream, c->sig_panel, pending_sig, info, budget);
            const bool last_pair = nblk - 2 - gated_kk <= small_m + 1;
            if (chain && !split_off && !last_pair && gated_m3 > 2) {
                const int kk = gated_kk, m = gated_m3 + 2;
                hipLaunchKernelGGL(potrf_colupd_kernel, dim3((4 * (m - 2) + 1) + (4 * (m - 3) + 1) + 4, 1, 1), dim3(256), 0, c->side_stream, A, ld,
                                   bstride, kk, m, 2, 2, 2, (unsigned long long*)nullptr, 0ull, info, 1, kk + 5, (unsigned long long*)nullptr, budget);
                bulk_pub = ++c->sig_seq;
                bulk_pub_word = SIGW_NEAR;
                hipLaunchKernelGGL(potrf_publish_kernel, dim3(1), dim3(64), 0, c->side_stream, c->sig_panel + SIGW_NEAR, bulk_pub);
                launch_bulk(kk, gated_m3 - 2, kk + 5, 1);
                far_pub = ++c->sig_seq;
                hipLaunchKernelGGL(potrf_publish_kernel, dim3(1), dim3(64), 0, c->side_stream, c->sig_panel + SIGW_BULK, far_pub);
            } else {
                launch_bulk(gated_kk, gated_m3, gated_kk + 3, chain ? 1 : 0);
                bulk_pub = ++c->sig_seq;
                bulk_pub_word = SIGW_BULK;
                far_pub = bulk_pub;
                hipLaunchKernelGGL(potrf_publish_kernel, dim3(1), dim3(64), 0, c->side_stream, c->sig_panel + SIGW_BULK, bulk_pub);
            }
            pending_sig = 0;
        };
        for (; k + 1 < nblk; k += 2) {
            if (nblk - 1 - k <= small_m + 1) break;
            for (int kk = k; kk < k + 2; ++kk) {
                if (chain) {
                    launch_follow(kk, pending_sig);
                    flush_gated_bulk();
                } else {
                    hipLaunchKernelGGL(potrf_diag_kernel, dim3(1, 1, batch), dim3(DIAG_THREADS), DIAG_LDS_BYTES, s, A, ld, bstride, kk, inv16,
                                       inv16_bstride, info, pending_sig ? c->sig_panel : (unsigned long long*)nullptr, pending_sig);
                    flush_gated_bulk();
                    const int nrows16 = (Np - (kk + 1) * BLK) / 16 + 1;
                    hipLaunchKernelGGL(potrf_trsm_kernel, dim3(nrows16, 1, batch), dim3(TRSM_THREADS), 0, s, A, ld, bstride, kk, inv16, inv16_bstride,
                                       (kk + 1) * BLK);
                }
                const int m = nblk - 1 - kk;
                if (kk == k) {
                    const int xblk = (chain && m >= 2) ? kk + 2 : -1;
                    hipLaunchKernelGGL(potrf_colupd_kernel, dim3(4 * m + 1 + (xblk >= 0 ? 4 : 0), 1, batch), dim3(256), 0, s, A, ld, bstride, kk, m, 1, 0, 1,
                                       (unsigned long long*)nullptr, 0ull, info, chain ? 1 : 0, xblk, critw, budget);
                } else {
                    const bool poll = bulk_pub != 0;
                    if (last >= 0 && !poll) (void)hipStreamWaitEvent(s, c->ev_rest[last], 0);
                    const int nc = m >= 2 ? 2 : 1;
                    const int xblk = (chain && m - 2 > 0) ? kk + 3 : -1;
                    hipLaunchKernelGGL(potrf_colupd_kernel, dim3((4 * m + 1) + (nc == 2 ? 4 * (m - 1) + 1 : 0) + (xblk >= 0 ? 4 : 0), 1, batch), dim3(256), 0, s,
                                       A, ld, bstride, kk, m, nc, 0, 2, poll ? c->sig_panel + bulk_pub_word : (unsigned long long*)nullptr, bulk_pub, info,
                                       chain ? 1 : 0, xblk, critw, budget);
                    const int m3 = m - 2;
                    if (m3 > 0) {
                        if (gates && c->sig_panel && batch == 1) {
                            pending_sig = ++c->sig_seq;
                            gated_kk = kk;
                            gated_m3 = m3;
                        } else {
                            (void)hipEventRecord(c->ev_panel[kk], s);
                            (void)hipStreamWaitEvent(c->side_stream, c->ev_panel[kk], 0);
                            launch_bulk(kk, m3, kk + 3, chain ? 1 : 0);
                        }
                        last = kk;
                    }
                }
            }
        }
        tail_join = last;
        kstart = k;
    }
    int last_rest = tail_join;
    for (int k = kstart; k < nblk; ++k) {
        if (chain) {
            launch_follow(k, pending_sig);
            flush_gated_bulk();
        } else {
            {
                ProfScope ps(c, "potrf_diag");
                hipLaunchKernelGGL(potrf_diag_kernel, dim3(1, 1, batch), dim3(DIAG_THREADS), DIAG_LDS_BYTES, s, A, ld, bstride,
                                   k, inv16, inv16_bstride, info, pending_sig ? c->sig_panel : (unsigned long long*)nullptr, pending_sig);
                flush_gated_bulk();
            }
            const int nrows16 = (Np - (k + 1) * BLK) / 16 + 1;
            {
                ProfScope ps(c, "potrf_trsm");
                hipLaunchKernelGGL(potrf_trsm_kernel, dim3(nrows16, 1, batch), dim3(TRSM_THREADS), 0, s, A, ld, bstride, k, inv16,
                                   inv16_bstride, (k + 1) * BLK);
            }
        }
        const int m = nblk - 1 - k;
        if (m == 0) {
            if (step_hook && chain_inline) (*step_hook)(k);
            break;
        }
        if (la && (m <= small_m + 1 || chain)) {
            const bool poll = last_rest >= 0 && last_rest == tail_join && bulk_pub != 0;
            if (last_rest >= 0 && !poll) (void)hipStreamWaitEvent(s, c->ev_rest[last_rest], 0);
            last_rest = -1;
            if (chain_inline && plan->tab) {
                const int* off = plan->tab_off;
                hipLaunchKernelGGL(potrf_colupd_tab_kernel, dim3(off[k + 1] - off[k]), dim3(256), 0, s, A, ld, plan->tab + off[k], k, critw);
            } else
                hipLaunchKernelGGL(potrf_colupd_kernel, dim3(2 * m * (m + 1) + m, 1, batch), dim3(256), 0, s, A, ld, bstride, k,
                                   m, m, 0, 1, poll ? c->sig_panel + bulk_pub_word : (unsigned long long*)nullptr, bulk_pub, info, chain ? 1 : 0, -1, critw, budget);
            BOSS_STAMP(2000 + k);
            if (step_hook && chain_inline) (*step_hook)(k);
            continue;
        }
        if (!la) {
            ProfScope ps(c, "potrf_syrk");
            hipLaunchKernelGGL(potrf_syrk_kernel<1>, dim3(m * (m + 1) / 2 + m, 1, batch), dim3(256), 0, s, A, ld, bstride, k,
                               k + 1, m, 0);
            continue;
        }
        {
            const bool poll = last_rest >= 0 && last_rest == tail_join && bulk_pub != 0;
            if (last_rest >= 0 && !poll) (void)hipStreamWaitEvent(s, c->ev_rest[last_rest], 0);
            hipLaunchKernelGGL(potrf_colupd_kernel, dim3(4 * m + 1, 1, batch), dim3(256), 0, s, A, ld, bstride, k, m, 1, 0, 1,
                               poll ? c->sig_panel + bulk_pub_word : (unsigned long long*)nullptr, bulk_pub, info, 0, -1, (unsigned long long*)nullptr, budget);
        }
        last_rest = -1;
#ifdef BOSS_EXPERIMENTS
        static const int exp_norest = getenv("BOSS_EXP_NOREST") ? atoi(getenv("BOSS_EXP_NOREST")) : 0;
#else
        constexpr int exp_norest = 0;
#endif
        if (m >= 2 && exp_norest != 1) {
            const int m2 = m - 1;
            (void)hipEventRecord(c->ev_panel[k], s);
            (void)hipStreamWaitEvent(c->side_stream, c->ev_panel[k], 0);
            if (exp_norest != 2)
                hipLaunchKernelGGL(potrf_syrk_kernel<1>, dim3(m2 * (m2 + 1) / 2 + m2, 1, batch), dim3(256), 0, c->side_stream, A,
                                   ld, bstride, k, k + 2, m2, 0);
            (void)hipEventRecord(c->ev_rest[k], c->side_stream);
            last_rest = k;
        }
    }
    if (la && last_rest >= 0) (void)hipStreamWaitEvent(s, c->ev_rest[last_rest], 0);
}

static void gram_enqueue(Ctx* c, const double* Xsc, size_t xs_bstride, int d, int N, int Np, int kern,
                         const double* hyp, double* A, int ld, size_t bstride, int batch) {
    ProfScope ps(c, "gram");
    const int nt = Np / 64;
    hipLaunchKernelGGL(gram_kernel, dim3(nt * (nt + 1) / 2, 1, batch), dim3(256), 0, c->stream, Xsc, xs_bstride, d, N,
                       Np, kern, hyp, A, ld, bstride, 0);
}

static void gp_release(boss_gp* g) {
    if (!g) return;
    if (g->ctx) (void)hipSetDevice(g->ctx->device);
    if (g->ctx) chain_quiesce(g->ctx);
    if (g->set) {
        if (g->ctx) (void)hipStreamSynchronize(g->ctx->stream);
        if (g->dinv_pending && g->ctx) (void)hipStreamSynchronize(g->ctx->side_stream);
        boss_gpset* st = g->set;
        if (st->refs.fetch_sub(1) == 1) {
            gpset_release_storage(st);
            delete st;
        }
        g->Xraw = g->Xsc = g->y = g->mean = g->A = g->inv16 = g->Dinv = g->Dinv2 = g->invlam = g->scal = nullptr;
        g->lamX = g->ampX = g->noiseX = nullptr;
        g->host_res = g->host_par = nullptr;
        g->set = nullptr;
    }
    void* ptrs[] = {g->Xraw, g->Xsc, g->y, g->mean, g->A, g->inv16, g->Dinv, g->Dinv2, g->LT, g->DT2, g->avec, g->invlam, g->scal, g->discrete_dev};
    for (void* p : ptrs)
        if (p) (void)hipFree(p);
    if (g->host_res) (void)hipHostFree(g->host_res);
    if (g->Winv) (void)hipFree(g->Winv);
    if (g->Linv) (void)hipFree(g->Linv);
    if (g->W2) (void)hipFree(g->W2);
    if (g->lamX) (void)hipFree(g->lamX);
    if (g->ampX) (void)hipFree(g->ampX);
    if (g->noiseX) (void)hipFree(g->noiseX);
    if (g->host_par) (void)hipHostFree(g->host_par);
    if (g->par_ev) (void)hipEventDestroy(g->par_ev);
    if (g->dinv_ev) (void)hipEventDestroy(g->dinv_ev);
    delete g;
}

static void pack_points(std::vector<double>& dst, const double* X, int d, int n, int ldp,
                        const unsigned char* discrete) {
    dst.assign((size_t)d * ldp, 0.0);
    for (int j = 0; j < n; ++j)
        for (int k = 0; k < d; ++k) {
            double v = X[(size_t)j * d + k];
            if (discrete && discrete[k]) v = std::nearbyint(v);
            dst[(size_t)k * ldp + j] = v;
        }
}

static int gp_create_common(int device, int kernel, int d, int npts, int N, const double* X, const double* y,
                            const unsigned char* discrete, bool aug, boss_gp_t** out) {
    if (!out) return fail(BOSS_E_INVALID, "out is NULL");
    *out = nullptr;
    if (kernel < 0 || kernel > 2) return fail(BOSS_E_INVALID, "unknown kernel id");
    if (d < 1 || N < 1 || !X || !y) return fail(BOSS_E_INVALID, "need d >= 1, N >= 1 and non-NULL X, y");
    if (N > MAX_ROWS) return fail(BOSS_E_INVALID, "more than 46080 rows (observations, or n (1 + d) with gradients) are not supported");
    Ctx* c;
    int rc = get_ctx(device, &c);
    if (rc) return rc;
    boss_gp* g = new boss_gp();
    g->ctx = c;
    g->kernel = kernel;
    g->d = d;
    g->N = N;
    g->Np = round_up(N, PRED_RB);
    g->nblk = g->Np / BLK;
    g->ld = g->Np + RHS_ROWS;
    g->aug = aug;
    g->npts = npts;
    g->nhead = npts;
    g->ldx = aug ? round_up(npts, 64) : g->Np;
    const size_t Np = g->Np, ldx = g->ldx;
#define GALLOC(ptr, bytes)                                        \
    do {                                                          \
        hipError_t e_ = dev_malloc((void**)&(ptr), (bytes));       \
        if (e_ != hipSuccess) {                                   \
            gp_release(g);                                        \
            return fail(BOSS_E_ALLOC, "device allocation failed"); \
        }                                                         \
    } while (0)
    GALLOC(g->Xraw, sizeof(double) * d * ldx);
    GALLOC(g->Xsc, sizeof(double) * d * ldx);
    GALLOC(g->y, sizeof(double) * Np);
    GALLOC(g->mean, sizeof(double) * Np);
    GALLOC(g->A, sizeof(double) * (size_t)g->ld * Np);
    GALLOC(g->inv16, sizeof(double) * g->nblk * 8 * 256);
    GALLOC(g->Dinv, sizeof(double) * g->nblk * BLK * BLK);
    GALLOC(g->Dinv2, sizeof(double) * (g->Np / PRED_RB) * PRED_RB * PRED_RB);
    GALLOC(g->invlam, sizeof(double) * (d + 4));
    g->hyp = g->invlam + d;
    GALLOC(g->scal, sizeof(double) * 4);
    g->info = (int*)(g->scal + 2);
    if (hipHostMalloc((void**)&g->host_res, 512, hipHostMallocDefault) != hipSuccess ||
        hipHostMalloc((void**)&g->host_par, sizeof(double) * (d + 4), hipHostMallocDefault) != hipSuccess ||
        hipEventCreateWithFlags(&g->par_ev, hipEventDisableTiming) != hipSuccess ||
        hipEventCreateWithFlags(&g->dinv_ev, hipEventDisableTiming) != hipSuccess ||
        hipHostGetDevicePointer((void**)&g->host_res_dev, g->host_res, 0) != hipSuccess) {
        gp_release(g);
        return fail(BOSS_E_ALLOC, "pinned allocation failed");
    }
    std::memset(g->host_res, 0, 512);
    if (discrete) {
        g->discrete.assign(discrete, discrete + d);
        bool any = false;
        for (int k = 0; k < d; ++k) any |= discrete[k] != 0;
        if (any) {
            GALLOC(g->discrete_dev, d);
            (void)hipMemcpy(g->discrete_dev, discrete, d, hipMemcpyHostToDevice);
        } else {
            g->discrete.clear();
        }
    }
#undef GALLOC
    std::vector<double> buf;
    pack_points(buf, X, d, npts, (int)ldx, g->discrete.empty() ? nullptr : g->discrete.data());
    std::vector<double> yb(Np, 0.0);
    std::copy(y, y + N, yb.begin());
    {
        std::lock_guard<std::mutex> lk(c->mtx);
        hipError_t e = hipMemcpyAsync(g->Xraw, buf.data(), sizeof(double) * d * ldx, hipMemcpyHostToDevice, c->stream);
        if (e == hipSuccess) e = hipMemcpyAsync(g->y, yb.data(), sizeof(double) * Np, hipMemcpyHostToDevice, c->stream);
        if (e == hipSuccess) e = hipMemsetAsync(g->mean, 0, sizeof(double) * Np, c->stream);
        if (e == hipSuccess) e = hipMemsetAsync(g->A, 0, sizeof(double) * (size_t)g->ld * Np, c->stream);
        if (e == hipSuccess) e = hipStreamSynchronize(c->stream);
        if (e != hipSuccess) {
            gp_release(g);
            return fail(BOSS_E_NO_DEVICE, std::string("uploading the observations: ") + hipGetErrorString(e));
        }
    }
    *out = g;
    return BOSS_OK;
}

extern "C" int boss_gp_create(int device, int kernel, int d, int N, const double* X, const double* y,
                              const unsigned char* discrete, boss_gp_t** out) {
    return gp_create_common(device, kernel, d, N, N, X, y, discrete, false, out);
}

extern "C" int boss_ggp_create(int device, int kernel, int d, int n, const double* X, const double* y, const double* dY,
                               boss_gp_t** out) {
    if (!out) return fail(BOSS_E_INVALID, "out is NULL");
    *out = nullptr;
    if (d < 1 || n < 1 || !X || !y || !dY) return fail(BOSS_E_INVALID, "need d >= 1, n >= 1 and non-NULL X, y, dY");
    if (d > AUG_MAX_D) return fail(BOSS_E_INVALID, "gradient observations: x_dim above 16 is not supported");
    if ((long long)n * (1 + d) > MAX_ROWS) return fail(BOSS_E_INVALID, "augmented system too large (n (1 + d) > 46080)");
    std::vector<double> yt((size_t)n * (1 + d));
    for (int j = 0; j < n; ++j) {
        yt[j] = y[j];
        for (int l = 0; l < d; ++l) yt[(size_t)n * (1 + l) + j] = dY[(size_t)j * d + l];
    }
    return gp_create_common(device, kernel, d, n, n * (1 + d), X, yt.data(), nullptr, true, out);
}

#define NOT_FOR_AUG(g)                                                                                            \
    do {                                                                                                          \
        if ((g)->aug) return fail(BOSS_E_INVALID, "not available for gradient-observation posteriors (boss_ggp_*)"); \
        if ((g)->gibbs) return fail(BOSS_E_INVALID, "not available for nonstationary posteriors (boss_ngp_*)");      \
    } while (0)

#define NOT_FOR_GIBBS(g, mean_a, mean_b)                                                                            \
    do {                                                                                                            \
        if ((g)->gibbs) return fail(BOSS_E_INVALID, "not available for nonstationary posteriors (boss_ngp_*)");        \
        if ((g)->aug && ((mean_a) || (mean_b)))                                                                      \
            return fail(BOSS_E_INVALID, "gradient-observation posteriors take no prior mean (gradient_gp.jl:307-361)"); \
    } while (0)

extern "C" int boss_ngp_create(int device, int d, int N, const double* X, const double* y, const unsigned char* discrete,
                               boss_gp_t** out) {
    int rc = gp_create_common(device, KERN_SQEXP, d, N, N, X, y, discrete, false, out);
    if (rc) return rc;
    boss_gp* g = *out;
    g->gibbs = true;
    g->kernel = KERN_GIBBS;
    const size_t Np = g->Np;
    if (dev_malloc((void**)&g->lamX, sizeof(double) * d * Np) != hipSuccess ||
        dev_malloc((void**)&g->ampX, sizeof(double) * Np) != hipSuccess ||
        dev_malloc((void**)&g->noiseX, sizeof(double) * Np) != hipSuccess) {
        gp_release(g);
        *out = nullptr;
        return fail(BOSS_E_ALLOC, "device allocation failed");
    }
    return BOSS_OK;
}

struct RiderReq {
    ChainPlan plan;
    unsigned long long end_gate = 0;
    std::function<void(int)> step;
};
static int gp_finish(boss_gp* g, double* logpdf_out);
static int factor_enqueue(boss_gp* g, RiderReq* rider = nullptr);
static int gp_own(boss_gp* g);

constexpr double LOG_2PI = 1.8378770664093453;
static double loglik(int N, double logdet, double zz) { return -0.5 * (N * LOG_2PI + logdet + zz); }

static bool small_fit_ok(const Ctx* c, int N, int d) {
    static const bool small_off = getenv("BOSS_NO_SMALL_FIT") && atoi(getenv("BOSS_NO_SMALL_FIT"));
    return N <= SMALL_MAX_N && d <= SMALL_MAX_D && !c->prof_on && !small_off;
}

static void gp_invalidate(boss_gp* g) {
    g->fitted = false;
    g->have_dinv = false;
    g->have_winv = false;
    g->few_calls = 0;
    g->have_lt = false;
    g->fell_back = false;
    ++g->epoch;
    g->append_calls = 0;
}

static int gp_settle(boss_gp* g, const char* unfitted = "handle has no valid factorisation") {
    if (g->pending) {
        int rc = gp_finish(g, nullptr);
        if (rc) return rc;
    }
    if (!g->fitted) return fail(BOSS_E_NOT_FITTED, unfitted);
    return BOSS_OK;
}

static int update_finish(boss_gp* g, int flags, double* logpdf_out) {
    HIPCHK(hipGetLastError());
    g->pending = true;
    if (flags & BOSS_FIT_NO_SYNC) return BOSS_OK;
    return gp_finish(g, logpdf_out);
}

extern "C" int boss_gp_set_y(boss_gp_t* g, const double* y) {
    if (!g || !y) return fail(BOSS_E_INVALID, "NULL argument");
    if (g->aug) return fail(BOSS_E_INVALID, "not available for gradient-observation posteriors (boss_ggp_*)");
    HIPCHK(hipSetDevice(g->ctx->device));
    std::lock_guard<std::mutex> lk(g->ctx->mtx);
    if (g->pending) (void)gp_finish(g, nullptr);
    {
        int rc = gp_own(g);
        if (rc) return rc;
    }
    HIPCHK(hipMemcpyAsync(g->y, y, sizeof(double) * g->N, hipMemcpyHostToDevice, g->ctx->stream));
    HIPCHK(hipStreamSynchronize(g->ctx->stream));
    g->fitted = false;
    return BOSS_OK;
}

static const char* hyper_fault(int d, const double* lam, double amp, double sig) {
    for (int k = 0; k < d; ++k)
        if (!(lam[k] >= 0.0)) return "lengthscales must be >= 0";
    if (!(amp >= 0.0)) return "amplitude must be >= 0";
    if (!(sig >= 0.0)) return "noise_std must be >= 0";
    return nullptr;
}
static int validate_hyper(int d, const double* lam, double amp, double sig) {
    if (!lam) return fail(BOSS_E_INVALID, "lengthscale is NULL");
    const char* why = hyper_fault(d, lam, amp, sig);
    return why ? fail(BOSS_E_INVALID, why) : BOSS_OK;
}
static bool stage_hyper(int d, const double* lam, double amplitude, double noise_std, double* invlam, double* hyp) {
    const bool ok = !hyper_fault(d, lam, amplitude, noise_std);
    for (int k = 0; k < d; ++k) invlam[k] = 1.0 / ((ok ? lam[k] : 1.0) + MIN_PARAM_VALUE);
    const double amp = (ok ? amplitude : 1.0) + MIN_PARAM_VALUE, sig = (ok ? noise_std : 1.0) + MIN_PARAM_VALUE;
    hyp[0] = amp * amp;
    hyp[1] = sig * sig;
    return ok;
}

static int gp_finish(boss_gp* g, double* logpdf_out) {
    Ctx* c = g->ctx;
    if (g->res_polled) {
        volatile unsigned long long* seq = reinterpret_cast<volatile unsigned long long*>(g->host_res + 3);
        bool got = false;
        static const bool watch = getenv("BOSS_DEBUG_WATCH") && atoi(getenv("BOSS_DEBUG_WATCH"));
        auto t_watch = std::chrono::steady_clock::now();
        for (unsigned long i = 1;; ++i) {
            if (*seq == g->res_seq) {
                got = true;
                break;
            }
            if ((i & 0x3fff) == 0) {
                const hipError_t q = hipStreamQuery(c->stream);
                if (q != hipErrorNotReady) {
                    if (watch) std::fprintf(stderr, "[bosship watch] hipStreamQuery returned %d (%s) before the result word arrived\n", (int)q, hipGetErrorString(q));
                    break;
                }
            }
            if (watch && (i & 0xfffff) == 0 && std::chrono::steady_clock::now() - t_watch > std::chrono::seconds(2) && c->sig_panel) {
                t_watch = std::chrono::steady_clock::now();
                std::fprintf(stderr, "[bosship watch] still waiting for the update's result word\n");
                unsigned long long w[SIG_WORDS];
                int inf = 0;
                (void)hipMemcpy(w, c->sig_panel, sizeof w, hipMemcpyDeviceToHost);
                (void)hipMemcpy(&inf, g->info, sizeof inf, hipMemcpyDeviceToHost);
                const unsigned long long cb = c->chain_seq - (8ull * g->nblk + 16);
                std::fprintf(stderr, "[bosship watch] nblk %d info %d | up %llu/%llu wdone %lld panel %lld (block %lld panel %lld) crit %lld | gate %llu/%llu near %llu bulk %llu | strips",
                             g->nblk, inf, w[SIGW_UP], c->up_seq, (long long)(w[SIGW_WDONE] - cb), (long long)(w[SIGW_PANEL] - cb), (long long)((w[SIGW_PANEL] - cb) / 8),
                             (long long)((w[SIGW_PANEL] - cb) % 8), (long long)(w[SIGW_CRIT] - (c->crit_seq - 8ull * (g->nblk - 2))), w[SIGW_GATE], c->sig_seq,
                             w[SIGW_NEAR], w[SIGW_BULK]);
                for (int q = 0; q < 8; ++q) std::fprintf(stderr, " %lld", (long long)(w[SIGW_PROG + SIGW_PROG_STRIDE * q] - cb));
                std::fprintf(stderr, "\n");
            }
        }
        std::atomic_thread_fence(std::memory_order_acquire);
        g->res_polled = false;
        if (!got) {
            HIPCHK(hipStreamSynchronize(c->stream));
            if (*seq != g->res_seq) {
                g->pending = false;
                g->fitted = false;
                if (c->few_done) (void)hipMemset(c->few_done, 0, sizeof(unsigned long long));
                c->few_done_cnt = 0;
                if (logpdf_out) *logpdf_out = -std::numeric_limits<double>::infinity();
                HIPCHK(hipGetLastError());
                return fail(BOSS_E_NO_DEVICE, "the update's last kernel did not deliver its result (device error)");
            }
        }
    } else {
        HIPCHK(hipStreamSynchronize(c->stream));
    }
    g->pending = false;
    const double logdet = g->host_res[0], zz = g->host_res[1];
    int info;
    std::memcpy(&info, &g->host_res[2], sizeof(int));
    if (info != 0 || !std::isfinite(logdet) || !std::isfinite(zz)) {
        g->fitted = false;
        if (logpdf_out) *logpdf_out = -std::numeric_limits<double>::infinity();
        if (info == INT_MIN) {
            const bool drop_chain = g->chained;
            if (drop_chain || g->gated) {
                (void)hipDeviceSynchronize();
                int code = 0;
                (void)hipMemcpyFromSymbol(&code, HIP_SYMBOL(boss::g_giveup), sizeof(int));
                const int zero = 0;
                (void)hipMemcpyToSymbol(HIP_SYMBOL(boss::g_giveup), &zero, sizeof(int));
// ... 302 lines not shown
```

boss.jl_amd/csrc/host_predict.inc:

```

extern "C" int boss_cand_create(int device, int d, int M, const double* Xs, boss_cand_t** out) {
    if (!out) return fail(BOSS_E_INVALID, "out is NULL");
    *out = nullptr;
    if (d < 1 || M < 1 || !Xs) return fail(BOSS_E_INVALID, "need d >= 1, M >= 1 and non-NULL Xs");
    Ctx* c;
    int rc = get_ctx(device, &c);
    if (rc) return rc;
    boss_cand* cd = new boss_cand();
    cd->ctx = c;
    cd->d = d;
    cd->M = M;
    cd->Mp = round_up(M, 64);
    if (dev_malloc((void**)&cd->Craw, sizeof(double) * d * cd->Mp) != hipSuccess) {
        delete cd;
        return fail(BOSS_E_ALLOC, "device allocation failed");
    }
    std::vector<double> buf;
    pack_points(buf, Xs, d, M, cd->Mp, nullptr);
    HIPCHK(hipMemcpy(cd->Craw, buf.data(), sizeof(double) * d * cd->Mp, hipMemcpyHostToDevice));
    *out = cd;
    return BOSS_OK;
}

static int drain(Ctx* c, int rc) {
    (void)hipStreamSynchronize(c->stream);
    return rc;
}

static int neg_var_error(long* bad_index, unsigned long long bad, double v) {
    if (bad_index) *bad_index = (long)bad;
    char msg[160];
    std::snprintf(msg, sizeof msg, "The posterior GP predicted variance %g but only values above -1e-08 are tolerated. (DomainError)", v);
    return fail(BOSS_E_NEG_VAR, msg);
}

struct DownCopy {
    void* host;
    const void* dev;
    size_t bytes;
};
static int finish(Ctx* c, std::initializer_list<DownCopy> outs) {
    hipStream_t s = c->stream;
    const char* next = (const char*)outs.begin()->dev;
    size_t total = 0;
    bool together = true;
    for (const DownCopy& o : outs) {
        together = together && o.dev == next;
        next = (const char*)o.dev + o.bytes;
        total += o.bytes;
    }
    hipError_t e;
    if (together && total <= PINNED_DOWN_BYTES) {
        char* stage = (char*)c->pinned + PINNED_DOWN_OFF;
        (void)hipMemcpyAsync(stage, outs.begin()->dev, total, hipMemcpyDeviceToHost, s);
        e = hipStreamSynchronize(s);
        for (const DownCopy& o : outs) {
            std::memcpy(o.host, stage, o.bytes);
            stage += o.bytes;
        }
    } else {
        for (const DownCopy& o : outs) (void)hipMemcpyAsync(o.host, o.dev, o.bytes, hipMemcpyDeviceToHost, s);
        e = hipStreamSynchronize(s);
    }
    const hipError_t e2 = hipGetLastError();
    if (e == hipSuccess) e = e2;
    if (e != hipSuccess) return fail(BOSS_E_NO_DEVICE, hipGetErrorString(e));
    return BOSS_OK;
}

static int temp_cand(Ctx* c, int d, int M, const double* Xs, boss_cand* cd) {
    cd->ctx = c;
    cd->d = d;
    cd->M = M;
    cd->Mp = round_up(M, 64);
    int rc = ws_reserve(c->craw, sizeof(double) * (size_t)d * cd->Mp);
    if (rc) return rc;
    cd->Craw = (double*)c->craw.p;
    std::vector<double> buf;
    pack_points(buf, Xs, d, M, cd->Mp, nullptr);
    const size_t bytes = sizeof(double) * d * cd->Mp;
    if (bytes <= PINNED_UP_BYTES) {
        void* stage = (char*)c->pinned + PINNED_UP_OFF;
        HIPCHK(hipEventSynchronize(c->ev_up));
        std::memcpy(stage, buf.data(), bytes);
        HIPCHK(hipMemcpyAsync(cd->Craw, stage, bytes, hipMemcpyHostToDevice, c->stream));
        HIPCHK(hipEventRecord(c->ev_up, c->stream));
        return BOSS_OK;
    }
    HIPCHK(hipMemcpyAsync(cd->Craw, buf.data(), bytes, hipMemcpyHostToDevice, c->stream));
    HIPCHK(hipStreamSynchronize(c->stream));
    return BOSS_OK;
}

extern "C" void boss_cand_free(boss_cand_t* cd) {
    if (!cd) return;
    if (cd->ctx) {
        (void)hipSetDevice(cd->ctx->device);
        (void)hipStreamSynchronize(cd->ctx->stream);
    }
    if (cd->Craw) (void)hipFree(cd->Craw);
    delete cd;
}

__global__ void scale_cand_kernel(const double* __restrict__ Craw, double* __restrict__ Csc, const double* __restrict__ invlam,
                                  const unsigned char* __restrict__ discrete, int d, int Mp) {
    const int j = blockIdx.x * blockDim.x + threadIdx.x;
    if (j >= Mp) return;
    for (int k = 0; k < d; ++k) {
        double v = Craw[(size_t)k * Mp + j];
        if (discrete && discrete[k]) v = rint(v);
        Csc[(size_t)k * Mp + j] = v * invlam[k];
    }
}

static int invgemm_max_tiles() {
    static const int v = getenv("BOSS_INVGEMM_MAX_TILES") ? atoi(getenv("BOSS_INVGEMM_MAX_TILES")) : 128;
    return v;
}

static int slab_bn(int M, bool for_grad) {
    static const bool force64 = getenv("BOSS_FORCE_BN64") && atoi(getenv("BOSS_FORCE_BN64"));
    return !for_grad && (M >= 64 * 256 || force64) ? 64 : 32;
}


static void linv_enqueue(boss_gp* g, hipStream_t s, double* U, double* Lw, const SetBatch& B) {
    const int Np = g->Np, ld = g->ld;
    hipLaunchKernelGGL(linv_seed_kernel, dim3(PRED_RB, Np / PRED_RB, B.nb), dim3(PRED_RB), 0, s, (const double*)g->Dinv2, Lw, ld, U, ld,
                       B.sDinv2, B.sW);
    for (int sz = PRED_RB; sz < Np; sz *= 2) {
        const int pairs = (Np + 2 * sz - 1) / (2 * sz), tiles = (sz / BLK) * (sz / BLK);
        hipLaunchKernelGGL((linv_level_kernel<SyrkG, 1>), dim3(tiles, pairs, B.nb), dim3(256), 0, s, (const double*)g->A, ld, Lw, ld, U, ld,
                           Np, sz, B.sA, B.sW);
        hipLaunchKernelGGL((linv_level_kernel<SyrkG, 2>), dim3(tiles, pairs, B.nb), dim3(256), 0, s, (const double*)g->A, ld, Lw, ld, U, ld,
                           Np, sz, B.sA, B.sW);
    }
}

static void gibbs_kstar32_launch(boss_gp* g, const boss_cand* cd, const double* clam_dev, const double* camp_dev, int tiles,
                                 double* out, hipStream_t s) {
    if (g->d <= GIBBS_KSTAR_MAX_D)
        hipLaunchKernelGGL(gibbs_kstar_cols_kernel, dim3(g->Np / 256, tiles), dim3(256),
                           sizeof(double) * (2 * g->d * 32 + 32 + 2 * 8 * 256), s, (const double*)g->Xraw, (const double*)g->lamX,
                           (const double*)g->ampX, g->d, g->N, g->Np, (const double*)cd->Craw, clam_dev, camp_dev, cd->Mp, out);
    else
        hipLaunchKernelGGL(gibbs_kstar_kernel<32>, dim3(g->Np / 256, tiles), dim3(256), sizeof(double) * (2 * g->d + 1) * 32, s,
                           (const double*)g->Xraw, (const double*)g->lamX, (const double*)g->ampX, g->d, g->N, g->Np,
                           (const double*)cd->Craw, clam_dev, camp_dev, cd->Mp, out);
}

static void small_dinv(boss_gp* g, hipStream_t s) {
    dinv_join(g);
    if (g->have_dinv || g->dinv0_gen == g->factor_gen) return;
    hipLaunchKernelGGL(potrf_dinv_kernel, dim3(8, 1, 1), dim3(64), 0, s, g->A, g->ld, (size_t)0, g->inv16, (size_t)0, g->Dinv, (size_t)0);
    g->dinv0_gen = g->factor_gen;
}
static bool small_predict_ok(const boss_gp* g, int M) {
    const long long cap = std::min<long long>(16384, 1024LL * SMALL_MAX_N * SMALL_MAX_N / ((long long)g->N * g->N));
    return small_fit_ok(g->ctx, g->N, g->d) && M <= cap && !g->aug && !g->gibbs;
}

static int predict_enqueue(boss_gp* g, const boss_cand* cd, const double* mean_s_dev, double* mu, double* var,
                           bool for_grad = false, const double* clam_dev = nullptr, const double* camp_dev = nullptr,
                           bool need_v = false) {
    Ctx* c = g->ctx;
    hipStream_t s = c->stream;
    if (!g->fitted) return fail(BOSS_E_NOT_FITTED, "handle has no valid factorisation");
    if (g->gibbs && !clam_dev)
        return fail(BOSS_E_INVALID, "nonstationary posteriors predict through boss_ngp_predict (λ(x*), α(x*) are needed)");
    if (cd->ctx != c) return fail(BOSS_E_INVALID, "candidates and posterior live on different devices");
    if (cd->d != g->d) return fail(BOSS_E_INVALID, "candidate dimension differs from the model's x_dim");
    if (!for_grad && !need_v && small_predict_ok(g, cd->M)) {
        small_dinv(g, s);
        const int grid = std::min(512, (cd->M + SPG_WAVES - 1) / SPG_WAVES);
        hipLaunchKernelGGL(small_predict_grad_kernel<false>, dim3(grid), dim3(SPG_THREADS), SPG_LDS_BYTES, s, (const double*)g->Dinv,
                           (const double*)g->A, g->ld, g->Np, g->N, g->d, g->kernel, g->amp2, (const double*)g->Xsc, g->ldx,
                           (const double*)cd->Craw, cd->Mp, cd->M, (const double*)g->invlam, (const unsigned char*)g->discrete_dev,
                           mean_s_dev, (const double*)nullptr, mu, var, (double*)nullptr, (double*)nullptr);
        HIPCHK(hipGetLastError());
        return BOSS_OK;
    }
    bool joined = false;
    auto join_dinv = [&]() {
        if (!joined) dinv_join(g);
        joined = true;
    };
    if (!g->have_dinv) {
        join_dinv();
        ProfScope ps(c, "dinv");
        dinv_launch(g, s);
        g->have_dinv = true;
    }
    g->dinv_used = true;
    const int Mp = cd->Mp;
    const int BN = slab_bn(cd->M, for_grad);
    const int tiles = (cd->M + BN - 1) / BN;
    int rc = ws_reserve(c->csc, sizeof(double) * (size_t)g->d * Mp);
    if (rc) return rc;
    rc = ws_reserve(c->vscratch, sizeof(double) * (size_t)tiles * BN * g->Np * (for_grad ? 2 : 1));
    if (rc) return rc;
    double* Csc = (double*)c->csc.p;
    if (!g->gibbs)
        hipLaunchKernelGGL(scale_cand_kernel, dim3((Mp + 255) / 256), dim3(256), 0, s, cd->Craw, Csc, g->invlam,
                           g->discrete_dev, g->d, Mp);
#ifdef BOSS_EXPERIMENTS
    static const int dbg = getenv("BOSS_DBG") ? atoi(getenv("BOSS_DBG")) : 0;
#else
    constexpr int dbg = 0;
#endif
    static const bool no_few = getenv("BOSS_NO_FEW") && atoi(getenv("BOSS_NO_FEW"));
    static const int few_max_tiles = getenv("BOSS_FEW_MAX_TILES") ? atoi(getenv("BOSS_FEW_MAX_TILES")) : 128;
    const int ftiles = (cd->M + 31) / 32;
    const size_t aug_lds = sizeof(double) * ((size_t)g->d * (64 + 256) + g->d);
    if (ftiles <= few_max_tiles && g->Np >= 4 * PRED_RB && g->d <= 64 && !no_few && (BN == 32 || for_grad)) {
        typedef PredG32 G;
        typedef GemmDirect<4, 1, 2, 2, 8> GU;
        ProfScope ps(c, "predict");
        const int nb = g->Np / PRED_RB;
        const int nwg = g->Np / WINV_ROWS;
        const size_t step_part = (size_t)ftiles * nb * FEW_STEP_PARTS * 64;
        rc = ws_reserve(c->few, sizeof(double) * ((size_t)ftiles * ((size_t)g->Np * 32 + 64) + (size_t)nwg * 8 + step_part));
        if (rc) return rc;
        double* R = (double*)c->few.p;
        double* ssmz = R + (size_t)ftiles * g->Np * 32;
        double* part = ssmz + 64 * (size_t)ftiles + (size_t)nwg * 8;
        double* V = (double*)c->vscratch.p;
        static const int winv_after = getenv("BOSS_WINV_AFTER") ? atoi(getenv("BOSS_WINV_AFTER")) : 2;
        const size_t winv_lds = sizeof(double) * (size_t)g->Np * (cd->M == 1 ? 1 : cd->M == 2 ? 2 : WINV_MAX_M);
        if (winv_after > 0 && !g->have_winv && ++g->few_calls >= winv_after) {
            const size_t bytes = sizeof(double) * (size_t)g->ld * g->Np;
            bool ok = (g->Winv != nullptr || dev_malloc((void**)&g->Winv, bytes) == hipSuccess) &&
                      (g->Linv != nullptr || dev_malloc((void**)&g->Linv, bytes) == hipSuccess);
            if (ok) {
                join_dinv();
                linv_enqueue(g, s, g->Winv, g->Linv);
                g->have_winv = true;
            } else {
                (void)hipGetLastError();
                g->few_calls = -(1 << 30);
            }
        }
        const bool use_winv = g->have_winv && !for_grad && !need_v && cd->M <= WINV_MAX_M && winv_lds <= 144 * 1024;
        const bool use_invgemm = g->have_winv && !use_winv && ftiles <= invgemm_max_tiles();
        if (!use_winv) (void)hipMemsetAsync(ssmz, 0, sizeof(double) * 64 * ftiles, s);
        if (g->aug)
            hipLaunchKernelGGL(aug_kstar_kernel, dim3(g->Np / 256, ftiles), dim3(256), aug_lds, s, (const double*)g->Xraw, g->ldx,
                               g->d, g->nhead, g->N, g->Np, (const double*)cd->Craw, Mp, g->kernel, g->amp2,
                               (const double*)g->invlam, R, 32);
        else if (g->gibbs)
            gibbs_kstar32_launch(g, cd, clam_dev, camp_dev, ftiles, R, s);
        else
            hipLaunchKernelGGL(kstar_rows_kernel, dim3(g->Np / 256, ftiles), dim3(256), sizeof(double) * (g->d * 32 + KSTAR_LDS_EXTRA), s,
                               (const double*)g->Xsc, g->Np, g->N, (const double*)Csc, g->d, Mp, g->kernel, g->amp2, R,
                               use_winv ? cd->M : 32);
        join_dinv();
        if (use_invgemm) {
            const int nrb = g->Np / BLK;
            rc = ws_reserve(c->lgC, sizeof(double) * (size_t)ftiles * nrb * 64);
            if (rc) return rc;
            double* ssp = (double*)c->lgC.p;
            hipLaunchKernelGGL(inv_fwd_kernel<GU>, dim3(ftiles, nrb), dim3(GU::NTHREADS), 0, s, (const double*)g->Linv, g->ld, g->Np,
                               (const double*)g->A, g->ld, (const double*)R, V, ssp);
            hipLaunchKernelGGL(inv_fwd_finish_kernel, dim3(ftiles), dim3(256), 0, s, (const double*)ssp, nrb, mean_s_dev, cd->M,
                               g->amp2, g->aug ? 1 : g->gibbs ? 2 : 0, mu, var);
            if (g->gibbs) hipLaunchKernelGGL(gibbs_var_kernel, dim3((cd->M + 255) / 256), dim3(256), 0, s, var, camp_dev, cd->M);
            HIPCHK(hipGetLastError());
            return BOSS_OK;
        }
        if (use_winv) {
            double* part = ssmz + 64 * (size_t)ftiles;
            const int mc = cd->M == 1 ? 1 : cd->M == 2 ? 2 : 4;
            const size_t lds = sizeof(double) * (size_t)g->Np * mc;
            auto kfn = mc == 1 ? winv_gemv_kernel<1> : mc == 2 ? winv_gemv_kernel<2> : winv_gemv_kernel<4>;
            hipLaunchKernelGGL(kfn, dim3(nwg), dim3(256), lds, s, (const double*)g->Winv, g->ld, g->Np,
                               (const double*)g->A, g->ld, (const double*)R, cd->M, part, (double*)nullptr);
            hipLaunchKernelGGL(winv_finish_kernel, dim3(1), dim3(256), 0, s, (const double*)part, nwg, cd->M, mean_s_dev, g->amp2,
                               g->aug ? 1 : g->gibbs ? 2 : 0, mu, var);
            if (g->gibbs) hipLaunchKernelGGL(gibbs_var_kernel, dim3(1), dim3(256), 0, s, var, camp_dev, cd->M);
            HIPCHK(hipGetLastError());
            return BOSS_OK;
        }
        static const bool few_w_off = getenv("BOSS_NO_FEW_W") && atoi(getenv("BOSS_NO_FEW_W"));
        if (!few_w_off && g->W2 && g->w2_np != g->Np) {
            (void)hipStreamSynchronize(s);
            (void)hipFree(g->W2);
            g->W2 = nullptr;
        }
        if (!few_w_off && !g->W2) {
            if (dev_malloc((void**)&g->W2, sizeof(double) * (size_t)nb * FEW_W_SLAB) == hipSuccess) {
                g->w2_np = g->Np;
                g->w2_gen = ~0ull;
            } else {
                (void)hipGetLastError();
                g->W2 = nullptr;
            }
        }
        if (!few_w_off && g->W2) {
            g->w2_used = true;
            if (g->w2_gen != g->factor_gen) {
                hipLaunchKernelGGL(few_w_kernel<G>, dim3(PRED_RB / 32, 2 * nb), dim3(G::NTHREADS), PredictLds<G>::BYTES, s, (const double*)g->A,
                                   g->ld, (const double*)g->Dinv2, g->W2);
                g->w2_gen = g->factor_gen;
            }
            for (int ib = 0; ib < nb; ++ib) {
                const int nblk = ib >= 2 && (ib & 1) == 0 ? (nb - 1 - ib) * (PRED_RB / GU::BM) : 0;
                const int per_x = (nblk >> 3) * ftiles + ((nblk & 7) * ftiles + 7) / 8;
                hipLaunchKernelGGL(few_step_kernel<GU>, dim3(ftiles * FEW_STEP_PARTS + 8 * per_x), dim3(256), 0, s, (const double*)g->A, g->ld,
                                   g->Np, nb, ib, ftiles, R, (const double*)g->Dinv2, (const double*)g->W2, V, part);
            }
            hipLaunchKernelGGL(few_sum_kernel, dim3(ftiles), dim3(256), 0, s, (const double*)part, nb, mean_s_dev, cd->M, g->amp2, mu, var,
                               g->aug ? 1 : g->gibbs ? 2 : 0);
            if (g->gibbs) hipLaunchKernelGGL(gibbs_var_kernel, dim3((cd->M + 255) / 256), dim3(256), 0, s, var, camp_dev, cd->M);
            HIPCHK(hipGetLastError());
            return BOSS_OK;
        }
        for (int ib = 0; ib < nb; ++ib) {
            hipLaunchKernelGGL(few_finish_kernel<G>, dim3(ftiles), dim3(G::NTHREADS), PredictLds<G>::BYTES, s, (const double*)g->A,
                               g->ld, g->Np, ib, (const double*)R, (const double*)g->Dinv2, V, ssmz, ib == nb - 1 ? 1 : 0,
                               mean_s_dev, cd->M, g->amp2, mu, var, g->aug ? 1 : g->gibbs ? 2 : 0);
            const int nupd = (nb - 1 - ib) * (PRED_RB / BLK);
            if (nupd > 0)
                hipLaunchKernelGGL(few_update_kernel<GU>, dim3(ftiles, nupd), dim3(GU::NTHREADS), 0, s, (const double*)g->A, g->ld,
                                   g->Np, ib, (const double*)V, R);
        }
        if (g->gibbs) hipLaunchKernelGGL(gibbs_var_kernel, dim3((cd->M + 255) / 256), dim3(256), 0, s, var, camp_dev, cd->M);
        HIPCHK(hipGetLastError());
        return BOSS_OK;
    }
    join_dinv();
    if (g->aug || g->gibbs) {
        ProfScope ps(c, "predict");
        double* V = (double*)c->vscratch.p;
        if (g->aug)
            hipLaunchKernelGGL(aug_kstar_kernel, dim3(g->Np / 256, tiles), dim3(256), aug_lds, s, (const double*)g->Xraw, g->ldx, g->d,
                               g->nhead, g->N, g->Np, (const double*)cd->Craw, Mp, g->kernel, g->amp2, (const double*)g->invlam, V, BN);
        else if (BN == 32)
            gibbs_kstar32_launch(g, cd, clam_dev, camp_dev, tiles, V, s);
        else
            hipLaunchKernelGGL(gibbs_kstar_kernel<64>, dim3(g->Np / 256, tiles), dim3(256), sizeof(double) * (2 * g->d + 1) * 64, s,
                               (const double*)g->Xraw, (const double*)g->lamX, (const double*)g->ampX, g->d, g->N, g->Np,
                               (const double*)cd->Craw, clam_dev, camp_dev, Mp, V);
        if (BN == 32) {
            typedef PredG32 G;
            hipLaunchKernelGGL((predict_kernel<G, true>), dim3(tiles), dim3(G::NTHREADS), PredictLds<G>::BYTES, s, g->A, g->ld, g->Np,
                               g->N, g->Dinv2, g->Xsc, Csc, g->d, Mp, g->kernel, g->amp2, V, mean_s_dev, cd->M, mu, var, dbg);
        } else {
            typedef PredG64 G;
            hipLaunchKernelGGL((predict_kernel<G, true>), dim3(tiles), dim3(G::NTHREADS), PredictLds<G>::BYTES, s, g->A, g->ld, g->Np,
                               g->N, g->Dinv, g->Xsc, Csc, g->d, Mp, g->kernel, g->amp2, V, mean_s_dev, cd->M, mu, var, dbg);
        }
        if (g->gibbs) hipLaunchKernelGGL(gibbs_var_kernel, dim3((cd->M + 255) / 256), dim3(256), 0, s, var, camp_dev, cd->M);
        HIPCHK(hipGetLastError());
        return BOSS_OK;
    }
    {
        ProfScope ps(c, "predict");
        if (BN == 32) {
            typedef PredG32 G;
            hipLaunchKernelGGL(predict_kernel<G>, dim3(tiles), dim3(G::NTHREADS), PredictLds<G>::BYTES, s, g->A, g->ld, g->Np,
                               g->N, g->Dinv2, g->Xsc, Csc, g->d, Mp, g->kernel, g->amp2, (double*)c->vscratch.p, mean_s_dev, cd->M, mu, var, dbg);
        } else {
            typedef PredG64 G;
            hipLaunchKernelGGL(predict_kernel<G>, dim3(tiles), dim3(G::NTHREADS), PredictLds<G>::BYTES, s, g->A, g->ld, g->Np,
                               g->N, g->Dinv, g->Xsc, Csc, g->d, Mp, g->kernel, g->amp2, (double*)c->vscratch.p, mean_s_dev, cd->M, mu, var, dbg);
        }
    }
    HIPCHK(hipGetLastError());
    return BOSS_OK;
}

__global__ void scale_cand_set_kernel(const double* __restrict__ Craw, const PredSet* __restrict__ sets,
                                      const unsigned char* __restrict__ discrete, int d, int Mp) {
    const PredSet ps = sets[blockIdx.y];
    double* Csc = const_cast<double*>(ps.Csc);
    const int j = blockIdx.x * blockDim.x + threadIdx.x;
    if (j >= Mp) return;
    for (int k = 0; k < d; ++k) {
        double v = Craw[(size_t)k * Mp + j];
        if (discrete && discrete[k]) v = rint(v);
        Csc[(size_t)k * Mp + j] = v * ps.invlam[k];
    }
}

static int set_np_max() {
    static const int v = getenv("BOSS_SET_NP_MAX") ? atoi(getenv("BOSS_SET_NP_MAX")) : 2048;
    return v;
}
static bool predict_set_ok(int n, boss_gp_t* const* gps, const boss_cand* cd, bool with_latents = false) {
    if (n < 2) return false;
    const boss_gp* g0 = gps[0];
    if (!g0 || g0->Np > set_np_max() || g0->ctx->prof_on || g0->d > 64) return false;
    if (g0->gibbs && (!with_latents || g0->d > GIBBS_KSTAR_MAX_D)) return false;
    const bool model = g0->aug || g0->gibbs;
    for (int i = 0; i < n; ++i) {
        const boss_gp* g = gps[i];
        if (!g || g->aug != g0->aug || g->gibbs != g0->gibbs || !g->fitted || g->pending || g->ctx != cd->ctx || g->N != g0->N || g->Np != g0->Np ||
            g->ld != g0->ld || g->d != g0->d || g->d != cd->d || g->kernel != g0->kernel || g->discrete != g0->discrete)
            return false;
        if (model && (g->npts != g0->npts || g->ldx != g0->ldx || g->nhead != g0->nhead)) return false;
    }
    return true;
}
static void set_dinv_enqueue(int n, boss_gp_t* const* gps, hipStream_t s) {
    boss_gp* g0 = gps[0];
    bool uniform = n >= 2 && g0->set != nullptr;
    const ptrdiff_t sA = n >= 2 ? gps[1]->A - gps[0]->A : 0, sI = n >= 2 ? gps[1]->inv16 - gps[0]->inv16 : 0,
                    sD = n >= 2 ? gps[1]->Dinv - gps[0]->Dinv : 0, sD2 = n >= 2 ? gps[1]->Dinv2 - gps[0]->Dinv2 : 0;
    for (int i = 0; i < n && uniform; ++i) {
        const boss_gp* g = gps[i];
        uniform = g->set == g0->set && !g->have_dinv && !g->dinv_pending && g->A - g0->A == sA * i && g->inv16 - g0->inv16 == sI * i &&
                  g->Dinv - g0->Dinv == sD * i && g->Dinv2 - g0->Dinv2 == sD2 * i && sA > 0 && sI > 0 && sD > 0 && sD2 > 0;
    }
    if (uniform) {
        SetBatch B;
        B.nb = n;
        B.sA = (size_t)sA;
        B.sInv16 = (size_t)sI;
        B.sDinv = (size_t)sD;
        B.sDinv2 = (size_t)sD2;
        dinv_launch(gps[0], s, B);
        for (int i = 0; i < n; ++i) gps[i]->have_dinv = true;
    }
    for (int i = 0; i < n; ++i) {
        boss_gp* g = gps[i];
        dinv_join(g);
        if (!g->have_dinv) {
            dinv_launch(g, s);
            g->have_dinv = true;
        }
        g->dinv_used = true;
    }
}
static int predict_set_enqueue(int n, boss_gp_t* const* gps, const boss_cand* cd, const double* mean_all, double* mu_all,
                               double* var_all, size_t mstride, const double* clam_all = nullptr, const double* camp_all = nullptr,
                               const std::function<int(int, int)>* after_group = nullptr) {
    boss_gp* g0 = gps[0];
    Ctx* c = g0->ctx;
    hipStream_t s = c->stream;
    typedef PredG32 G;
    const int Mp = cd->Mp, d = g0->d, Np = g0->Np;
    const int tiles = (cd->M + G::BN - 1) / G::BN;
    set_dinv_enqueue(n, gps, s);
    static const size_t v_cap = (size_t)(getenv("BOSS_SET_V_GIB") ? atof(getenv("BOSS_SET_V_GIB")) : 8.0) * ((size_t)1 << 30);
    const size_t v_one = sizeof(double) * (size_t)tiles * G::BN * Np;
    int group = (int)std::max<size_t>(1, std::min<size_t>((size_t)n, std::min<size_t>(v_cap / v_one, 65535)));
    int rc = ws_reserve(c->vscratch, v_one * group);
    while (rc == BOSS_E_ALLOC && group > 1) {
        group = (group + 1) / 2;
        rc = ws_reserve(c->vscratch, v_one * group);
    }
    if (rc) return rc;
    const bool pre = g0->aug || g0->gibbs;
    if (!pre) rc = ws_reserve(c->csc, sizeof(double) * (size_t)d * Mp * n);
    if (rc) return rc;
    rc = ws_reserve(c->setdesc, sizeof(PredSet) * (size_t)n);
    if (rc) return rc;
    std::vector<PredSet> desc(n);
    for (int i = 0; i < n; ++i) {
        const boss_gp* g = gps[i];
        desc[i].A = g->A;
        desc[i].Dinv = g->Dinv2;
        desc[i].Xsc = g->Xsc;
        desc[i].Csc = pre ? nullptr : (const double*)c->csc.p + (size_t)i * d * Mp;
        desc[i].mean_s = mean_all ? mean_all + (size_t)i * mstride : nullptr;
        desc[i].invlam = g->invlam;
        desc[i].mu = mu_all + (size_t)i * mstride;
        desc[i].var = var_all + (size_t)i * mstride;
        desc[i].amp2 = g->amp2;
        desc[i].Xraw = pre ? g->Xraw : nullptr;
        if (g->gibbs) {
            desc[i].lamX = g->lamX;
            desc[i].ampX = g->ampX;
            desc[i].clam = clam_all + (size_t)i * d * Mp;
            desc[i].camp = camp_all + (size_t)i * Mp;
        }
    }
    const size_t bytes = sizeof(PredSet) * (size_t)n;
    if (bytes <= PINNED_UP_BYTES) {
        void* stage = (char*)c->pinned + PINNED_UP_OFF;
        HIPCHK(hipEventSynchronize(c->ev_up));
        std::memcpy(stage, desc.data(), bytes);
        HIPCHK(hipMemcpyAsync(c->setdesc.p, stage, bytes, hipMemcpyHostToDevice, s));
        HIPCHK(hipEventRecord(c->ev_up, s));
    } else {
        HIPCHK(hipMemcpyAsync(c->setdesc.p, desc.data(), bytes, hipMemcpyHostToDevice, s));
        HIPCHK(hipStreamSynchronize(s));
    }
    const PredSet* dsets = (const PredSet*)c->setdesc.p;
    if (!pre)
        for (int i0 = 0; i0 < n; i0 += 65535)
            hipLaunchKernelGGL(scale_cand_set_kernel, dim3((Mp + 255) / 256, std::min(65535, n - i0)), dim3(256), 0, s, (const double*)cd->Craw,
                               dsets + i0, (const unsigned char*)g0->discrete_dev, d, Mp);
    for (int i0 = 0; i0 < n; i0 += group) {
        const int cnt = std::min(group, n - i0);
        ++c->set_launches;
        if (!pre) {
            hipLaunchKernelGGL(predict_kernel_set<G>, dim3(tiles, cnt), dim3(G::NTHREADS), PredictLds<G>::BYTES, s, dsets + i0, g0->ld, Np, g0->N, d,
                               Mp, g0->kernel, (double*)c->vscratch.p, cd->M);
            if (after_group && (rc = (*after_group)(i0, cnt)) != BOSS_OK) return rc;
            continue;
        }
        ++c->set_pre_launches;
        if (g0->aug)
            hipLaunchKernelGGL(aug_kstar_set_kernel, dim3(Np / 256, tiles, cnt), dim3(256), sizeof(double) * ((size_t)d * (G::BN + 256) + d), s,
                               g0->ldx, d, g0->nhead, g0->N, Np, (const double*)cd->Craw, Mp, g0->kernel, dsets + i0,
                               (double*)c->vscratch.p, (int)G::BN);
        else
            hipLaunchKernelGGL(gibbs_kstar_set_kernel, dim3(Np / 256, tiles, cnt), dim3(256), sizeof(double) * (2 * d * 32 + 32 + 2 * 8 * 256), s,
                               d, g0->N, Np, (const double*)cd->Craw, Mp, dsets + i0, (double*)c->vscratch.p);
        hipLaunchKernelGGL((predict_kernel_set<G, true>), dim3(tiles, cnt), dim3(G::NTHREADS), PredictLds<G>::BYTES, s, dsets + i0, g0->ld, Np,
                           g0->N, d, Mp, g0->kernel, (double*)c->vscratch.p, cd->M);
        if (g0->gibbs) hipLaunchKernelGGL(gibbs_var_set_kernel, dim3((cd->M + 255) / 256, cnt), dim3(256), 0, s, dsets + i0, cd->M);
        if (after_group && (rc = (*after_group)(i0, cnt)) != BOSS_OK) return rc;
    }
    HIPCHK(hipGetLastError());
    return BOSS_OK;
}

extern "C" int boss_gp_predict(boss_gp_t* g, int M, const double* Xs, const double* mean_Xs, double* mu, double* var,
                               long* bad_index) {
    if (!g || !Xs || !mu || !var) return fail(BOSS_E_INVALID, "NULL argument");
    if (M < 1) return fail(BOSS_E_INVALID, "M must be >= 1");
    if (bad_index) *bad_index = -1;
    if (g->aug && mean_Xs) return fail(BOSS_E_INVALID, "gradient-observation posteriors take no prior mean (gradient_gp.jl:334-337)");
    if (!g->fitted) return fail(BOSS_E_NOT_FITTED, "handle has no valid factorisation");
    Ctx* c = g->ctx;
    HIPCHK(hipSetDevice(c->device));
    std::lock_guard<std::mutex> lk(c->mtx);
    {
        static const bool args_off = getenv("BOSS_NO_FEW_ARGS") && atoi(getenv("BOSS_NO_FEW_ARGS"));
        const size_t winv_lds = sizeof(double) * (size_t)g->Np * (M == 1 ? 1 : M == 2 ? 2 : WINV_MAX_M);
        if (!args_off && M <= WINV_MAX_M && g->have_winv && !g->pending && !g->aug && !g->gibbs && g->d <= FEW_ARGS_MAX_D && !c->prof_on &&
// ... 1126 lines not shown
```

Baseline: 894.4 updates/s.

## Add bound-based candidate pruning for expected-improvement argmax

Adds a pruning path to the EI argmax call. It computes cheap per-candidate upper bounds from a partial head factor and an alpha vector, radix-selects the top K candidates and evaluates them exactly. Only candidates whose bound beats the exact threshold are then refined, which avoids the full posterior variance solve over all 8192 candidates. The cost is extra kernels, a host poll on pinned memory, a fallback when the bounds fail, and some risk to correctness in edge cases.

```diff
diff --git a/boss.jl_amd/api.py b/boss.jl_amd/api.py
--- a/boss.jl_amd/api.py
+++ b/boss.jl_amd/api.py
@@ -2268,3 +2268,43 @@
     a = C.c_long(0)
     fn(device, C.byref(a))
     return a.value
+
+
+def _acq_path(device: int = 0):
+    fn = load_library().boss_debug_acq_path
+    fn.restype = C.c_int
+    fn.argtypes = [C.c_int, C.POINTER(C.c_int)]
+    out = (C.c_int * 5)()
+    _check(fn(device, out))
+    return tuple(out)
+
+
+def _acq_prune_set(device: int = 0, min_tiles: int = -1, K: int = -1, s: int = -1, cap: int = -1, slack: Optional[float] = None):
+    lib = load_library()
+    fn = lib.boss_debug_acq_prune_set
+    fn.restype = C.c_int
+    fn.argtypes = [C.c_int] * 5
+    _check(fn(device, int(min_tiles), int(K), int(s), int(cap)))
+    if slack is not None:
+        fs = lib.boss_debug_acq_prune_slack
+        fs.restype = C.c_int
+        fs.argtypes = [C.c_int, C.c_double]
+        _check(fs(device, float(slack)))
+
+
+def _acq_prune_bounds(M: int, device: int = 0):
+    fn = load_library().boss_debug_acq_prune_bounds
+    fn.restype = C.c_int
+    fn.argtypes = [C.c_int, C.c_int, C.c_void_p, C.c_void_p, C.c_void_p]
+    mua, vs, ub = np.zeros(M), np.zeros(M), np.zeros(M)
+    _check(fn(device, int(M), mua.ctypes.data, vs.ctypes.data, ub.ctypes.data))
+    return mua, vs, ub
+
+
+def _acq_counters(g: GP):
+    fn = load_library().boss_debug_acq_counters
+    fn.restype = C.c_int
+    fn.argtypes = [C.c_void_p, C.POINTER(C.c_long)]
+    out = (C.c_long * 4)()
+    _check(fn(g._h, out))
+    return tuple(out)
diff --git a/boss.jl_amd/csrc/bosship.hip b/boss.jl_amd/csrc/bosship.hip
--- a/boss.jl_amd/csrc/bosship.hip
+++ b/boss.jl_amd/csrc/bosship.hip
@@ -28,6 +28,7 @@
 #include "fitness.hpp"
 #include "mean_program.hpp"
 #include "warp_kernels.hpp"
+#include "prune_kernels.hpp"
 
 using namespace boss;
 
@@ -54,10 +55,12 @@
                  PINNED_DOWN_BYTES = 512 * 1024, PINNED_BYTES = PINNED_DOWN_OFF + PINNED_DOWN_BYTES;
 
 static bool release_cached_slabs();
+static std::atomic<long> g_dev_allocs{0};
 static std::atomic<int> g_fail_allocs{0};
 static hipError_t dev_malloc(void** p, size_t bytes) {
     static const bool poison = getenv("BOSS_POISON_ALLOC") && atoi(getenv("BOSS_POISON_ALLOC"));
     hipError_t e = hipErrorOutOfMemory;
+    g_dev_allocs.fetch_add(1, std::memory_order_relaxed);
     if (g_fail_allocs.load(std::memory_order_relaxed) > 0 && g_fail_allocs.fetch_sub(1) > 0) *p = nullptr;
     else e = hipMalloc(p, bytes);
     if (e != hipSuccess) (void)hipGetLastError();
@@ -111,12 +114,15 @@
     bool prof_on = false;
     std::map<std::string, std::vector<std::pair<hipEvent_t, hipEvent_t>>> prof;
     std::vector<hipEvent_t> ev_pool;
-    Workspace vscratch, csc, pred, acq, batchA, batchX, batchMisc, craw, lgA, lgB, lgC, few, setdesc, setmom, gsetdesc, nlatjobs, mceps, meanws, warpws;
+    Workspace vscratch, csc, pred, acq, batchA, batchX, batchMisc, craw, lgA, lgB, lgC, few, setdesc, setmom, gsetdesc, nlatjobs, mceps, meanws, warpws, prunews;
     static constexpr int LLG_BANKS = 4;
     Workspace lgbank[LLG_BANKS - 1][3];
     hipStream_t llg_stream[LLG_BANKS - 1] = {nullptr, nullptr, nullptr};
     hipEvent_t llg_join[LLG_BANKS - 1] = {nullptr, nullptr, nullptr};
     void* pinned = nullptr;
+    int prune_last[5] = {0, 0, 0, 0, 0};
+    long prune_launches = 0;
+    int prune_M = 0;
     struct TrailTab {
         TrailWork* dev = nullptr;
         std::vector<TrailWork> host;
@@ -315,6 +321,8 @@
     HIPCHK(hipFuncSetAttribute((const void*)potrf_syrk_kernel<2, true>, hipFuncAttributeMaxDynamicSharedMemorySize, 96 * 1024));
     HIPCHK(hipFuncSetAttribute((const void*)rider_step_kernel, hipFuncAttributeMaxDynamicSharedMemorySize, 96 * 1024));
     HIPCHK(hipFuncSetAttribute((const void*)predict_kernel<PredG32>, hipFuncAttributeMaxDynamicSharedMemorySize,
+                               PredictLds<PredG32>::BYTES));
+    HIPCHK(hipFuncSetAttribute((const void*)prune_head_kernel<PredG32>, hipFuncAttributeMaxDynamicSharedMemorySize,
                                PredictLds<PredG32>::BYTES));
     HIPCHK(hipFuncSetAttribute((const void*)predict_kernel_set<PredG32>, hipFuncAttributeMaxDynamicSharedMemorySize,
                                PredictLds<PredG32>::BYTES));
@@ -497,6 +505,10 @@
     bool have_winv = false;
     int few_calls = 0;
     int append_calls = 0;
+    double* prune_a = nullptr;
+    int prune_a_np = 0;
+    unsigned long long prune_a_gen = ~0ull;
+    int prune_skip = 0, prune_backoff = 0;
     int append_path = 0;
 };
 
@@ -598,6 +610,7 @@
 static void mc_grad_launch(hipStream_t s, const double* mu, const double* var, const double* dmu, const double* dvar, int M, int d, int S,
                            const EiPar& par, const McEpi& mc, const double* deps, const unsigned char* mask, double* acq, double* dacq);
 #include "host_predict.inc"
+#include "host_prune.inc"
 #include "host_acq.inc"
 #include "host_fitness.inc"
 #include "host_mean.inc"
diff --git a/boss.jl_amd/csrc/host_acq.inc b/boss.jl_amd/csrc/host_acq.inc
--- a/boss.jl_amd/csrc/host_acq.inc
+++ b/boss.jl_amd/csrc/host_acq.inc
@@ -41,6 +41,22 @@
     par0.mode = 0;
     if (valid_mask) (void)hipMemcpyAsync(dmask, valid_mask, M, hipMemcpyHostToDevice, s);
     if (S > 1) (void)hipMemsetAsync(dacq, 0, sizeof(double) * M, s);
+    if (!acq_out && !defer) {
+        for (int i = 0; i < 5; ++i) c->prune_last[i] = 0;
+        if (prune_eligible(gps[0], cand, P, S, par, acq_out != nullptr, defer, mc != nullptr, dpair)) {
+            if (mean_Xs) (void)hipMemcpyAsync(dmean, mean_Xs, sizeof(double) * M, hipMemcpyHostToDevice, s);
+            bool done = false;
+            double pmax = 0.0;
+            long pidx = 0;
+            rc = acq_prune_try(gps[0], cand, mean_Xs ? dmean : nullptr, valid_mask ? dmask : nullptr, par, &done, &pmax, &pidx);
+            if (rc) return rc;
+            if (done) {
+                if (argmax_out) *argmax_out = pidx;
+                if (max_out) *max_out = pmax;
+                return BOSS_OK;
+            }
+        }
+    }
     std::vector<double> hmean;
     static const bool set_off = getenv("BOSS_NO_SET_PREDICT") && atoi(getenv("BOSS_NO_SET_PREDICT"));
     if (S > 1 && par.mode != 0 && !set_off && predict_set_ok(P * S, gps, cand)) {
diff --git a/boss.jl_amd/csrc/host_factor.inc b/boss.jl_amd/csrc/host_factor.inc
--- a/boss.jl_amd/csrc/host_factor.inc
+++ b/boss.jl_amd/csrc/host_factor.inc
@@ -499,6 +499,7 @@
     if (g->Winv) (void)hipFree(g->Winv);
     if (g->Linv) (void)hipFree(g->Linv);
     if (g->W2) (void)hipFree(g->W2);
+    if (g->prune_a) (void)hipFree(g->prune_a);
     if (g->lamX) (void)hipFree(g->lamX);
     if (g->ampX) (void)hipFree(g->ampX);
     if (g->noiseX) (void)hipFree(g->noiseX);
diff --git a/boss.jl_amd/csrc/host_predict.inc b/boss.jl_amd/csrc/host_predict.inc
--- a/boss.jl_amd/csrc/host_predict.inc
+++ b/boss.jl_amd/csrc/host_predict.inc
@@ -162,7 +162,7 @@
 
 static int predict_enqueue(boss_gp* g, const boss_cand* cd, const double* mean_s_dev, double* mu, double* var,
                            bool for_grad = false, const double* clam_dev = nullptr, const double* camp_dev = nullptr,
-                           bool need_v = false) {
+                           bool need_v = false, bool internal = false) {
     Ctx* c = g->ctx;
     hipStream_t s = c->stream;
     if (!g->fitted) return fail(BOSS_E_NOT_FITTED, "handle has no valid factorisation");
@@ -227,7 +227,7 @@
         double* V = (double*)c->vscratch.p;
         static const int winv_after = getenv("BOSS_WINV_AFTER") ? atoi(getenv("BOSS_WINV_AFTER")) : 2;
         const size_t winv_lds = sizeof(double) * (size_t)g->Np * (cd->M == 1 ? 1 : cd->M == 2 ? 2 : WINV_MAX_M);
-        if (winv_after > 0 && !g->have_winv && ++g->few_calls >= winv_after) {
+        if (winv_after > 0 && !g->have_winv && !internal && ++g->few_calls >= winv_after) {
             const size_t bytes = sizeof(double) * (size_t)g->ld * g->Np;
             bool ok = (g->Winv != nullptr || dev_malloc((void**)&g->Winv, bytes) == hipSuccess) &&
                       (g->Linv != nullptr || dev_malloc((void**)&g->Linv, bytes) == hipSuccess);
diff --git a/boss.jl_amd/csrc/host_prune.inc b/boss.jl_amd/csrc/host_prune.inc
--- /dev/null
+++ b/boss.jl_amd/csrc/host_prune.inc
@@ -0,0 +1,256 @@
+
+struct PruneCfg {
+    int min_tiles = -1;
+    int K = 64;
+    int s = 1;
+    int cap = 1024;
+    double slack = 1.0;
+};
+static PruneCfg g_prune;
+constexpr double PRUNE_KMU = 1.2e-4, PRUNE_KVAR = 1e-10;
+constexpr size_t PRUNE_RES_OFF = 16;
+
+static bool prune_enabled() {
+    static const bool on = !(getenv("BOSS_ACQ_PRUNE") && atoi(getenv("BOSS_ACQ_PRUNE")) == 0);
+    static const bool once = [] {
+        if (getenv("BOSS_ACQ_PRUNE_BLOCKS")) g_prune.s = std::max(1, atoi(getenv("BOSS_ACQ_PRUNE_BLOCKS")));
+        if (getenv("BOSS_ACQ_PRUNE_CAP")) g_prune.cap = std::max(0, atoi(getenv("BOSS_ACQ_PRUNE_CAP")));
+        return true;
+    }();
+    (void)once;
+    return on;
+}
+
+extern "C" int boss_debug_acq_path(int device, int* out) {
+    if (!out) return fail(BOSS_E_INVALID, "out is NULL");
+    Ctx* c;
+    int rc = get_ctx(device, &c);
+    if (rc) return rc;
+    std::lock_guard<std::mutex> lk(c->mtx);
+    for (int i = 0; i < 5; ++i) out[i] = c->prune_last[i];
+    return BOSS_OK;
+}
+extern "C" int boss_debug_acq_prune_set(int device, int min_tiles, int K, int s, int cap) {
+    (void)device;
+    (void)prune_enabled();
+    const PruneCfg def;
+    if (min_tiles != -1) g_prune.min_tiles = min_tiles < -1 ? def.min_tiles : min_tiles;
+    if (K != -1) g_prune.K = K < 1 ? def.K : K;
+    if (s != -1) g_prune.s = s < 1 ? def.s : s;
+    if (cap != -1) g_prune.cap = cap < -1 ? def.cap : cap;
+    return BOSS_OK;
+}
+extern "C" int boss_debug_acq_counters(const boss_gp* g, long* out) {
+    if (!g || !out) return fail(BOSS_E_INVALID, "NULL argument");
+    out[0] = g->have_winv ? 1 : 0;
+    out[1] = g->few_calls;
+    out[2] = g_dev_allocs.load();
+    out[3] = g->ctx->prune_launches;
+    return BOSS_OK;
+}
+extern "C" int boss_debug_acq_prune_slack(int device, double scale) {
+    (void)device;
+    if (!(scale >= 0.0)) return fail(BOSS_E_INVALID, "scale must be >= 0");
+    g_prune.slack = scale;
+    return BOSS_OK;
+}
+extern "C" int boss_debug_acq_prune_bounds(int device, int M, double* mua_out, double* vars_out, double* ub_out) {
+    Ctx* c;
+    int rc = get_ctx(device, &c);
+    if (rc) return rc;
+    std::lock_guard<std::mutex> lk(c->mtx);
+    if (M < 1 || M != c->prune_M || !c->prunews.p) return fail(BOSS_E_INVALID, "no pruned attempt with that many candidates");
+    HIPCHK(hipStreamSynchronize(c->stream));
+    const double* base = (const double*)c->prunews.p;
+    if (mua_out) HIPCHK(hipMemcpy(mua_out, base, sizeof(double) * M, hipMemcpyDeviceToHost));
+    if (vars_out) HIPCHK(hipMemcpy(vars_out, base + M, sizeof(double) * M, hipMemcpyDeviceToHost));
+    if (ub_out) HIPCHK(hipMemcpy(ub_out, base + 2 * (size_t)M, sizeof(double) * M, hipMemcpyDeviceToHost));
+    return BOSS_OK;
+}
+
+static int prune_few_max_tiles() {
+    static const int few_max_tiles = getenv("BOSS_FEW_MAX_TILES") ? atoi(getenv("BOSS_FEW_MAX_TILES")) : 128;
+    return few_max_tiles;
+}
+static bool prune_eligible(const boss_gp* g, const boss_cand* cd, int P, int S, const EiPar& par, bool has_out, bool defer, bool has_mc,
+                           const double* dpair) {
+    if (!prune_enabled() || has_out || defer || dpair || has_mc || P != 1 || S != 1 || par.mode != 1) return false;
+    if (g->aug || g->gibbs || g->ctx->prof_on) return false;
+    static const bool no_few = getenv("BOSS_NO_FEW") && atoi(getenv("BOSS_NO_FEW"));
+    const int ftiles = (cd->M + 31) / 32, few_max_tiles = prune_few_max_tiles();
+    const int min_tiles = g_prune.min_tiles >= 0 ? g_prune.min_tiles : few_max_tiles;
+    if (no_few || ftiles <= min_tiles || g->Np < 4 * PRED_RB || g->d > 64 || cd->d != g->d || slab_bn(cd->M, false) != 32) return false;
+    if (small_predict_ok(g, cd->M) || cd->M <= g_prune.K || cd->M > PRUNE_THREADS * PRUNE_CPT_MAX) return false;
+    if (g_prune.K > 32 * few_max_tiles) return false;
+    return g_prune.s < g->Np / PRED_RB;
+}
+
+static bool prune_poll(Ctx* c, hipStream_t s, const double* res, unsigned long long want) {
+    volatile const unsigned long long* seq = reinterpret_cast<volatile const unsigned long long*>(res) + 4;
+    bool got = false;
+    for (unsigned long i = 1;; ++i) {
+        if (*seq == want) {
+            got = true;
+            break;
+        }
+        if ((i & 0x3fff) == 0 && hipStreamQuery(s) != hipErrorNotReady) break;
+    }
+    std::atomic_thread_fence(std::memory_order_acquire);
+    if (!got) {
+        (void)hipStreamSynchronize(s);
+        got = *seq == want;
+    }
+    return got;
+}
+
+static int prune_avec(boss_gp* g, hipStream_t s, const double** a_out, bool* rebuilt) {
+    *rebuilt = false;
+    if (g->have_lt && g->avec) {
+        *a_out = g->avec;
+        return BOSS_OK;
+    }
+    if (g->prune_a && g->prune_a_np != g->Np) {
+        (void)hipStreamSynchronize(s);
+        (void)hipFree(g->prune_a);
+        g->prune_a = nullptr;
+    }
+    if (!g->prune_a) {
+        if (dev_malloc((void**)&g->prune_a, sizeof(double) * 2 * (size_t)g->Np) != hipSuccess) {
+            g->prune_a = nullptr;
+            return fail(BOSS_E_ALLOC, "device allocation failed");
+        }
+        g->prune_a_np = g->Np;
+        g->prune_a_gen = ~0ull;
+    }
+    if (g->prune_a_gen != g->factor_gen) {
+        const int nb = g->Np / PRED_RB;
+        for (int ib = nb - 1; ib >= 0; --ib)
+            hipLaunchKernelGGL(prune_avec_step_kernel, dim3(std::max(1, 2 * ib)), dim3(PRUNE_AVEC_THREADS), 0, s, (const double*)g->A, g->ld, g->Np, g->N,
+                               (const double*)g->Dinv2, ib, ib == nb - 1 ? 1 : 0, g->prune_a + g->Np, g->prune_a);
+        g->prune_a_gen = g->factor_gen;
+        *rebuilt = true;
+    }
+    *a_out = g->prune_a;
+    return BOSS_OK;
+}
+
+static int acq_prune_try(boss_gp* g, const boss_cand* cd, const double* mean_dev, const unsigned char* mask_dev, const EiPar& par,
+                         bool* done, double* res_out, long* idx_out) {
+    *done = false;
+    Ctx* c = g->ctx;
+    hipStream_t s = c->stream;
+    int* last = c->prune_last;
+    last[0] = 0;
+    last[1] = last[2] = last[4] = 0;
+    last[3] = g_prune.s;
+    if (g->prune_skip > 0) {
+        --g->prune_skip;
+        last[0] = 3;
+        return BOSS_OK;
+    }
+    const int M = cd->M, Mp = cd->Mp, d = g->d, Np = g->Np, nch = Np / PRUNE_MU_ROWS, sblk = g_prune.s, K = g_prune.K;
+    const int cap = std::min(g_prune.cap, 32 * prune_few_max_tiles()), tiles = (M + 31) / 32;
+    const size_t nint = (size_t)round_up(std::max(K, cap), 64);
+    const size_t nd = (size_t)4 * M + (size_t)nch * M + 3 * nint + (size_t)d * nint + 2;
+    int rc = ws_reserve(c->prunews, sizeof(double) * nd + sizeof(int) * (nint + (size_t)M) + (size_t)M);
+    if (rc) return rc;
+    rc = ws_reserve(c->csc, sizeof(double) * (size_t)d * Mp);
+    if (rc) return rc;
+    rc = ws_reserve(c->vscratch, sizeof(double) * (size_t)tiles * 32 * Np);
+    if (rc) return rc;
+    double* mua = (double*)c->prunews.p;
+    double* vars = mua + M;
+    double* ub = vars + M;
+    unsigned long long* keys = (unsigned long long*)(ub + M);
+    double* part = ub + 2 * (size_t)M;
+    double* imu = part + (size_t)nch * M;
+    double* ivar = imu + nint;
+    double* imean = ivar + nint;
+    double* icraw = imean + nint;
+    double* tpair = icraw + (size_t)d * nint;
+    int* sel = (int*)(tpair + 2);
+    int* surv = sel + nint;
+    unsigned char* insel = (unsigned char*)(surv + M);
+    c->prune_M = M;
+    double* res = (double*)c->pinned + PRUNE_RES_OFF;
+
+    if (!g->have_dinv) {
+        dinv_join(g);
+        dinv_launch(g, s);
+        g->have_dinv = true;
+    }
+    dinv_join(g);
+    g->dinv_used = true;
+    const double* avec = nullptr;
+    bool rebuilt = false;
+    rc = prune_avec(g, s, &avec, &rebuilt);
+    if (rc) return rc;
+    last[4] = rebuilt ? 1 : 0;
+    c->prune_launches += (rebuilt ? Np / PRED_RB : 0) + 7;
+    double* Csc = (double*)c->csc.p;
+    hipLaunchKernelGGL(scale_cand_kernel, dim3((Mp + 255) / 256), dim3(256), 0, s, cd->Craw, Csc, g->invlam, g->discrete_dev, d, Mp);
+    typedef PredG32 G;
+    hipLaunchKernelGGL(prune_head_kernel<G>, dim3(tiles), dim3(G::NTHREADS), PredictLds<G>::BYTES, s, (const double*)g->A, g->ld, Np, g->N,
+                       (const double*)g->Dinv2, (const double*)g->Xsc, (const double*)Csc, d, Mp, g->kernel, g->amp2, (double*)c->vscratch.p, M,
+                       sblk, vars);
+    const size_t mu_lds = sizeof(double) * ((size_t)d + 1) * PRUNE_MU_STAGE;
+    auto mu_fn = d <= 16 ? prune_mu_kernel<true> : prune_mu_kernel<false>;
+    hipLaunchKernelGGL(mu_fn, dim3((M + PRUNE_MU_CANDS - 1) / PRUNE_MU_CANDS, nch), dim3(256), mu_lds, s, (const double*)g->Xsc, Np, g->N, (const double*)Csc, d, Mp, M,
+                       g->kernel, g->amp2, avec, part);
+    PrunePar pp;
+    pp.coef = par.coefs[0];
+    pp.best = par.best;
+    pp.amp2 = g->amp2;
+    pp.kmu = PRUNE_KMU * g_prune.slack;
+    pp.kvar = PRUNE_KVAR * g_prune.slack;
+    hipLaunchKernelGGL(prune_bound_kernel, dim3((M + 255) / 256), dim3(256), 0, s, (const double*)part, nch, mean_dev, (const double*)vars, mask_dev, M,
+                       pp, mua, ub, keys);
+    hipLaunchKernelGGL(prune_select_kernel, dim3(1), dim3(PRUNE_THREADS), 0, s, (const unsigned long long*)keys, M, K, sel, insel);
+
+    boss_cand icd;
+    icd.ctx = c;
+    icd.d = d;
+    auto finish_exact = [&](const int* list, int n) -> int {
+        icd.M = n;
+        icd.Mp = round_up(n, 64);
+        icd.Craw = icraw;
+        hipLaunchKernelGGL(prune_gather_kernel, dim3((icd.Mp + 255) / 256), dim3(256), 0, s, list, n, (const double*)cd->Craw, Mp, d, mean_dev,
+                           icraw, icd.Mp, mean_dev ? imean : (double*)nullptr);
+        return predict_enqueue(g, &icd, mean_dev ? imean : nullptr, imu, ivar, false, nullptr, nullptr, false, true);
+    };
+    rc = finish_exact(sel, K);
+    if (rc) return drain(c, rc);
+    unsigned long long seq = ++c->acq_seq;
+    hipLaunchKernelGGL(prune_decide_kernel, dim3(1), dim3(PRUNE_THREADS), 0, s, (const int*)sel, K, (const double*)imu, (const double*)ivar,
+                       (const double*)mua, mask_dev, par, pp, M, (const double*)ub, (const unsigned char*)insel, surv, tpair, res, seq);
+    bool ok = prune_poll(c, s, res, seq);
+    hipError_t e = hipGetLastError();
+    if (!ok || e != hipSuccess) return fail(BOSS_E_NO_DEVICE, e != hipSuccess ? hipGetErrorString(e) : "the pruned acquisition did not report");
+    long cnt = reinterpret_cast<const long*>(res)[2], bad = reinterpret_cast<const long*>(res)[3];
+    last[1] = K;
+    last[2] = (int)std::min<long>(cnt, 0x7fffffff);
+    if (!bad && cnt > 0 && cnt <= cap) {
+        rc = finish_exact(surv, (int)cnt);
+        if (rc) return drain(c, rc);
+        c->prune_launches += 2;
+        seq = ++c->acq_seq;
+        hipLaunchKernelGGL(prune_merge_kernel, dim3(1), dim3(PRUNE_THREADS), 0, s, (const int*)surv, (int)cnt, (const double*)imu,
+                           (const double*)ivar, (const double*)mua, mask_dev, par, pp, (const double*)tpair, res, seq);
+        ok = prune_poll(c, s, res, seq);
+        e = hipGetLastError();
+        if (!ok || e != hipSuccess) return fail(BOSS_E_NO_DEVICE, e != hipSuccess ? hipGetErrorString(e) : "the pruned acquisition did not report");
+        bad = reinterpret_cast<const long*>(res)[3];
+    }
+    if (bad || cnt > cap) {
+        g->prune_backoff = g->prune_backoff ? std::min(64, 2 * g->prune_backoff) : 1;
+        g->prune_skip = g->prune_backoff;
+        last[0] = 2;
+        return BOSS_OK;
+    }
+    g->prune_backoff = 0;
+    last[0] = 1;
+    *res_out = res[0];
+    *idx_out = reinterpret_cast<const long*>(res)[1];
+    *done = true;
+    return BOSS_OK;
+}
diff --git a/boss.jl_amd/csrc/prune_kernels.hpp b/boss.jl_amd/csrc/prune_kernels.hpp
--- /dev/null
+++ b/boss.jl_amd/csrc/prune_kernels.hpp
@@ -0,0 +1,567 @@
+#pragma once
+#include "acq_kernels.hpp"
+
+namespace boss {
+
+template <int NC>
+__device__ __forceinline__ void prune_wave_sums(double (&v)[NC], int lane) {
+#pragma unroll
+    for (int h = NC / 2; h >= 1; h >>= 1) {
+        const bool up = (lane & h) != 0;
+#pragma unroll
+        for (int j = 0; j < h; ++j) {
+            const double keep = up ? v[j + h] : v[j], send = up ? v[j] : v[j + h];
+            v[j] = keep + __shfl_xor(send, h);
+        }
+    }
+#pragma unroll
+    for (int off = NC; off < 64; off <<= 1) v[0] += __shfl_xor(v[0], off);
+}
+constexpr int PRUNE_AVEC_THREADS = 1024;
+__global__ __launch_bounds__(PRUNE_AVEC_THREADS) void prune_avec_step_kernel(const double* __restrict__ A, int ld, int Np, int N,
+                                                                             const double* __restrict__ Dinv2, int ib, int first,
+                                                                             double* __restrict__ r, double* __restrict__ a) {
+    __shared__ double rv[PRED_RB], av[PRED_RB];
+    const int tid = threadIdx.x, lane = tid & 63;
+    const int wave = __builtin_amdgcn_readfirstlane(tid >> 6);
+    const int i0 = ib * PRED_RB;
+    if (tid < PRED_RB) {
+        const int i = i0 + tid;
+        rv[tid] = first ? (i < N ? A[(size_t)i * ld + Np] : 0.0) : r[i];
+    }
+    __syncthreads();
+    const double* D = Dinv2 + (size_t)ib * PRED_RB * PRED_RB;
+    double r4[4];
+#pragma unroll
+    for (int q = 0; q < 4; ++q) r4[q] = rv[lane + 64 * q];
+    {
+        double sums[16];
+#pragma unroll
+        for (int j = 0; j < 16; ++j) {
+            const int c = 16 * j + wave;
+            const double* col = D + (size_t)c * PRED_RB;
+            double sacc = 0.0;
+#pragma unroll
+            for (int q = 0; q < 4; ++q) {
+                if (q >= j / 4) {
+                    const int row = lane + 64 * q;
+                    const double dv = col[row];
+                    sacc = __builtin_fma(row >= c ? dv : 0.0, r4[q], sacc);
+                }
+            }
+            sums[j] = sacc;
+        }
+        prune_wave_sums<16>(sums, lane);
+        if (lane < 16) av[16 * lane + wave] = sums[0];
+    }
+    __syncthreads();
+    if (blockIdx.x == 0 && tid < PRED_RB) a[i0 + tid] = av[tid];
+    if (ib == 0) return;
+    double a4[4];
+#pragma unroll
+    for (int q = 0; q < 4; ++q) a4[q] = av[lane + 64 * q];
+    double sums[8];
+    const int cg0 = blockIdx.x * 128 + wave * 8;
+#pragma unroll
+    for (int j = 0; j < 8; ++j) {
+        const double* col = A + (size_t)(cg0 + j) * ld + i0;
+        double sacc = 0.0;
+#pragma unroll
+        for (int q = 0; q < 4; ++q) sacc = __builtin_fma(col[lane + 64 * q], a4[q], sacc);
+        sums[j] = sacc;
+    }
+    prune_wave_sums<8>(sums, lane);
+    if (lane < 8) {
+        const int cg = cg0 + lane;
+        const double base = first ? (cg < N ? A[(size_t)cg * ld + Np] : 0.0) : r[cg];
+        r[cg] = base - sums[0];
+    }
+}
+
+template <class G>
+__global__ __launch_bounds__(G::NTHREADS) __attribute__((amdgpu_waves_per_eu(1, 1))) void prune_head_kernel(
+    const double* __restrict__ A, int ld, int Np, int N, const double* __restrict__ Dinv, const double* __restrict__ Xsc,
+    const double* __restrict__ Csc, int d, int Mp, int kern, double amp2, double* __restrict__ Vscratch, int M, int sblk,
+    double* __restrict__ var_out) {
+    static_assert(G::WC == 1 && G::BM == 2 * BLK && G::PM == 2 && G::WR == 4, "written for the 256-row, 32-candidate geometry");
+    constexpr int RB = G::BM;
+    extern __shared__ double lds[];
+    constexpr int BN = G::BN, TM = G::TM, TN = G::TN, LDR = PredictLds<G>::LDR;
+    double* Rs = lds;
+    double* red = Rs + RB * LDR;
+    const int tid = threadIdx.x, lane = tid & 63;
+    const int wave = __builtin_amdgcn_readfirstlane(tid >> 6);
+    const int wr = wave, wc = 0;
+    const int tile = blockIdx.x, c0 = tile * BN;
+    double* V = Vscratch + (size_t)tile * sblk * RB * BN;
+    double* part = red + 2 * G::WR * G::BN;
+#pragma unroll
+    for (int u = 0; u < TN * 4; ++u) part[u * G::NTHREADS + tid] = 0.0;
+    double* cs = part + (size_t)G::NTHREADS * PredictLds<G>::PART;
+    const bool cs_ok = d <= PRED_CS_MAX_D;
+    if (cs_ok) {
+        for (int idx = tid; idx < d * BN; idx += G::NTHREADS) cs[idx] = Csc[(size_t)(idx / BN) * Mp + c0 + (idx % BN)];
+        __syncthreads();
+    }
+    for (int ib = 0; ib < sblk; ++ib) {
+        v4d acc[TM][TN];
+#pragma unroll
+        for (int m = 0; m < TM; ++m)
+#pragma unroll
+            for (int n = 0; n < TN; ++n) acc[m][n] = v4d{0.0, 0.0, 0.0, 0.0};
+        G::template run<1>(A + (size_t)ib * RB, ld, V, BN, ib * RB, acc);
+        double r2[TM][TN][4];
+#pragma unroll
+        for (int m = 0; m < TM; ++m)
+#pragma unroll
+            for (int n = 0; n < TN; ++n)
+#pragma unroll
+                for (int i = 0; i < 4; ++i) r2[m][n][i] = 0.0;
+        if (cs_ok) {
+            for (int kd0 = 0; kd0 < d; kd0 += 4) {
+                double xr[4][TM];
+#pragma unroll
+                for (int kk = 0; kk < 4; ++kk)
+#pragma unroll
+                    for (int m = 0; m < TM; ++m)
+                        xr[kk][m] = (kd0 + kk < d) ? Xsc[(size_t)(kd0 + kk) * Np + ib * RB + G::row_of(wr, m, lane)] : 0.0;
+#pragma unroll
+                for (int kk = 0; kk < 4; ++kk) {
+                    if (kd0 + kk < d) {
+#pragma unroll
+                        for (int n = 0; n < TN; ++n)
+#pragma unroll
+                            for (int i = 0; i < 4; ++i) {
+                                const double xc = cs[(kd0 + kk) * BN + G::col_of(wc, n, i, lane)];
+#pragma unroll
+                                for (int m = 0; m < TM; ++m) {
+                                    const double diff = xr[kk][m] - xc;
+                                    r2[m][n][i] = __builtin_fma(diff, diff, r2[m][n][i]);
+                                }
+                            }
+                    }
+                }
+            }
+        } else
+        for (int kd = 0; kd < d; ++kd) {
+            double xr[TM], xc[TN][4];
+#pragma unroll
+            for (int m = 0; m < TM; ++m) xr[m] = Xsc[(size_t)kd * Np + ib * RB + G::row_of(wr, m, lane)];
+#pragma unroll
+            for (int n = 0; n < TN; ++n)
+#pragma unroll
+                for (int i = 0; i < 4; ++i) xc[n][i] = Csc[(size_t)kd * Mp + c0 + G::col_of(wc, n, i, lane)];
+#pragma unroll
+            for (int m = 0; m < TM; ++m)
+#pragma unroll
+                for (int n = 0; n < TN; ++n)
+#pragma unroll
+                    for (int i = 0; i < 4; ++i) {
+                        double diff = xr[m] - xc[n][i];
+                        r2[m][n][i] = __builtin_fma(diff, diff, r2[m][n][i]);
+                    }
+        }
+#pragma unroll
+        for (int m = 0; m < TM; ++m) {
+            const int row = G::row_of(wr, m, lane);
+            const bool live = (ib * RB + row) < N;
+#pragma unroll
+            for (int n = 0; n < TN; ++n)
+#pragma unroll
+                for (int i = 0; i < 4; ++i) {
+                    const double ks = live ? amp2 * kappa_r2(kern, r2[m][n][i]) : 0.0;
+                    Rs[row * LDR + G::col_of(wc, n, i, lane)] = ks - acc[m][n][i];
+                }
+        }
+        __syncthreads();
+        v4d acc2[TM][TN];
+#pragma unroll
+        for (int m = 0; m < TM; ++m)
+#pragma unroll
+            for (int n = 0; n < TN; ++n) acc2[m][n] = v4d{0.0, 0.0, 0.0, 0.0};
+        G::run_Blds_tri(Dinv + (size_t)ib * RB * RB, RB, Rs, LDR, acc2);
+#pragma unroll
+        for (int m = 0; m < TM; ++m) {
+            const int row = ib * RB + G::tri_row_of(wr, m, lane);
+#pragma unroll
+            for (int n = 0; n < TN; ++n)
+#pragma unroll
+                for (int i = 0; i < 4; ++i) {
+                    const double v = acc2[m][n][i];
+                    if (ib + 1 < sblk) V[(size_t)row * BN + G::col_of(wc, n, i, lane)] = v;
+                    double* ps = part + (size_t)(n * 4 + i) * G::NTHREADS + tid;
+                    ps[0] = __builtin_fma(v, v, ps[0]);
+                }
+        }
+        __syncthreads();
+    }
+#pragma unroll
+    for (int n = 0; n < TN; ++n)
+#pragma unroll
+        for (int i = 0; i < 4; ++i) {
+            double s = part[(size_t)(n * 4 + i) * G::NTHREADS + tid];
+#pragma unroll
+            for (int off = 1; off < 16; off <<= 1) s += __shfl_xor(s, off);
+            if ((lane & 15) == 0) red[wr * BN + G::col_of(wc, n, i, lane)] = s;
+        }
+    __syncthreads();
+    if (tid < BN) {
+        double s = 0.0;
+#pragma unroll
+        for (int w = 0; w < G::WR; ++w) s += red[w * BN + tid];
+        const int j = c0 + tid;
+        if (j < M) var_out[j] = amp2 - s + PREDICT_JITTER;
+    }
+}
+
+constexpr int PRUNE_MU_STAGE = 64, PRUNE_MU_ROWS = 128, PRUNE_MU_CANDS = 512;
+template <bool REG>
+__global__ __launch_bounds__(256) void prune_mu_kernel(const double* __restrict__ Xsc, int Np, int N, const double* __restrict__ Csc,
+                                                       int d, int Mp, int M, int kern, double amp2, const double* __restrict__ a,
+                                                       double* __restrict__ part) {
+    extern __shared__ double sm[];
+    double* xs = sm;
+    double* as = sm + (size_t)d * PRUNE_MU_STAGE;
+    const int j0 = blockIdx.x * PRUNE_MU_CANDS + threadIdx.x, j1 = j0 + 256;
+    const int jc0 = j0 < Mp ? j0 : Mp - 1, jc1 = j1 < Mp ? j1 : Mp - 1;
+    const int rbase = blockIdx.y * PRUNE_MU_ROWS;
+    double cx0[REG ? 16 : 1], cx1[REG ? 16 : 1];
+    if (REG) {
+#pragma unroll
+        for (int k = 0; k < 16; ++k) {
+            cx0[k] = k < d ? Csc[(size_t)k * Mp + jc0] : 0.0;
+            cx1[k] = k < d ? Csc[(size_t)k * Mp + jc1] : 0.0;
+        }
+    }
+    double acc0 = 0.0, acc1 = 0.0;
+    for (int sub = 0; sub < PRUNE_MU_ROWS / PRUNE_MU_STAGE; ++sub) {
+        const int r0 = rbase + sub * PRUNE_MU_STAGE;
+        __syncthreads();
+        for (int idx = threadIdx.x; idx < d * PRUNE_MU_STAGE; idx += 256)
+            xs[idx] = Xsc[(size_t)(idx / PRUNE_MU_STAGE) * Np + r0 + (idx % PRUNE_MU_STAGE)];
+        if (threadIdx.x < PRUNE_MU_STAGE) as[threadIdx.x] = (r0 + threadIdx.x < N) ? a[r0 + threadIdx.x] : 0.0;
+        __syncthreads();
+        if (r0 >= N) continue;
+        for (int rg = 0; rg < PRUNE_MU_STAGE; rg += 8) {
+            double ra[8], rb[8];
+#pragma unroll
+            for (int i = 0; i < 8; ++i) ra[i] = rb[i] = 0.0;
+            if (REG) {
+#pragma unroll
+                for (int k = 0; k < 16; ++k)
+                    if (k < d) {
+#pragma unroll
+                        for (int i = 0; i < 8; ++i) {
+                            const double x = xs[k * PRUNE_MU_STAGE + rg + i];
+                            const double da = x - cx0[k], db = x - cx1[k];
+                            ra[i] = __builtin_fma(da, da, ra[i]);
+                            rb[i] = __builtin_fma(db, db, rb[i]);
+                        }
+                    }
+            } else {
+                for (int k = 0; k < d; ++k) {
+                    const double ca = Csc[(size_t)k * Mp + jc0], cb = Csc[(size_t)k * Mp + jc1];
+#pragma unroll
+                    for (int i = 0; i < 8; ++i) {
+                        const double x = xs[k * PRUNE_MU_STAGE + rg + i];
+                        const double da = x - ca, db = x - cb;
+                        ra[i] = __builtin_fma(da, da, ra[i]);
+                        rb[i] = __builtin_fma(db, db, rb[i]);
+                    }
+                }
+            }
+#pragma unroll
+            for (int i = 0; i < 8; ++i) {
+                const double ai = as[rg + i];
+                if (r0 + rg + i < N) {
+                    acc0 = __builtin_fma(amp2 * kappa_r2(kern, ra[i]), ai, acc0);
+                    acc1 = __builtin_fma(amp2 * kappa_r2(kern, rb[i]), ai, acc1);
+                }
+            }
+        }
+    }
+    if (j0 < M) part[(size_t)blockIdx.y * M + j0] = acc0;
+    if (j1 < M) part[(size_t)blockIdx.y * M + j1] = acc1;
+}
+
+constexpr int PRUNE_THREADS = 1024;
+struct PrunePar {
+    double coef, best, amp2;
+    double kmu, kvar;
+};
+__device__ __forceinline__ double prune_dmu(const PrunePar& pp, double muf) {
+    return pp.kmu * (fabs(muf) + fabs(pp.best) + fabs(pp.coef) * sqrt(pp.amp2));
+}
+__device__ __forceinline__ double prune_bound(const PrunePar& pp, double mu, double var) {
+    if (var < 0.0) {
+        if (var >= -MAX_NEG_VAR) var = 0.0;
+        else return NAN;
+    }
+    const double muf = pp.coef * mu;
+    const double vf = pp.coef * pp.coef * (var + pp.kvar * pp.amp2);
+    const double sf = sqrt(vf), diff = muf - pp.best + prune_dmu(pp, muf);
+    double ei;
+    if (diff == 0.0 && sf == 0.0) ei = 0.0;
+    else {
+        const double z = diff / sf;
+        ei = diff * normcdf_dev(z) + sf * normpdf_dev(z);
+    }
+    return (ei - ei == 0.0) ? ei : NAN;
+}
+__device__ __forceinline__ unsigned long long prune_key(double v) {
+    if (v != v) return ~0ull;
+    const unsigned long long b = (unsigned long long)__double_as_longlong(v);
+    return (b >> 63) ? ~b : (b | 0x8000000000000000ull);
+}
+__device__ __forceinline__ int prune_exscan(int v, int* buf, int* total) {
+    const int t = threadIdx.x;
+    buf[t] = v;
+    __syncthreads();
+    for (int off = 1; off < PRUNE_THREADS; off <<= 1) {
+        const int add = t >= off ? buf[t - off] : 0;
+        __syncthreads();
+        buf[t] += add;
+        __syncthreads();
+    }
+    const int incl = buf[t];
+    *total = buf[PRUNE_THREADS - 1];
+    __syncthreads();
+    return incl - v;
+}
+
+__global__ __launch_bounds__(256) void prune_bound_kernel(const double* __restrict__ part, int nch, const double* __restrict__ mean_s,
+                                                          const double* __restrict__ var_s, const unsigned char* __restrict__ mask, int M,
+                                                          PrunePar pp, double* __restrict__ mua, double* __restrict__ ub,
+                                                          unsigned long long* __restrict__ keys) {
+    const int j = blockIdx.x * 256 + threadIdx.x;
+    if (j >= M) return;
+    double m = mean_s ? mean_s[j] : 0.0;
+    for (int ch = 0; ch < nch; ++ch) m += part[(size_t)ch * M + j];
+    mua[j] = m;
+    const double u = (mask && !mask[j]) ? 0.0 : prune_bound(pp, m, var_s[j]);
+    ub[j] = u;
+    keys[j] = prune_key(u);
+}
+
+__device__ __forceinline__ void prune_hist_add(int* hist, int bin, bool active, int lane) {
+    unsigned long long todo = __ballot(active);
+    while (todo) {
+        const int leader = __ffsll((long long)todo) - 1;
+        const int b = __shfl(bin, leader);
+        const unsigned long long same = __ballot(active && bin == b);
+        if (lane == leader) atomicAdd(&hist[b], (int)__popcll(same));
+        todo &= ~same;
+    }
+}
+
+constexpr int PRUNE_CPT_MAX = 16;
+__global__ __launch_bounds__(PRUNE_THREADS) void prune_select_kernel(const unsigned long long* __restrict__ keys, int M, int K,
+                                                                     int* __restrict__ sel, unsigned char* __restrict__ insel) {
+    __shared__ int hist[256];
+    __shared__ int scan[PRUNE_THREADS];
+    __shared__ unsigned long long s_prefix;
+    __shared__ int s_remaining;
+    const int t = threadIdx.x, lane = t & 63;
+    unsigned long long kreg[PRUNE_CPT_MAX];
+#pragma unroll
+    for (int i = 0; i < PRUNE_CPT_MAX; ++i) {
+        const int j = t + PRUNE_THREADS * i;
+        kreg[i] = j < M ? keys[j] : 0ull;
+    }
+    if (t == 0) {
+        s_prefix = 0ull;
+        s_remaining = K;
+    }
+    __syncthreads();
+    for (int pass = 7; pass >= 0; --pass) {
+        if (t < 256) hist[t] = 0;
+        __syncthreads();
+        const unsigned long long prefix = s_prefix;
+        const int sh = 8 * pass;
+#pragma unroll
+        for (int i = 0; i < PRUNE_CPT_MAX; ++i) {
+            const unsigned long long k = kreg[i];
+            const bool in = (t + PRUNE_THREADS * i < M) && (pass == 7 || (k >> (sh + 8)) == (prefix >> (sh + 8)));
+            prune_hist_add(hist, (int)((k >> sh) & 255ull), in, lane);
+        }
+        __syncthreads();
+        const int rem = s_remaining;
+        int suf = t < 256 ? hist[t] : 0;
+        for (int off = 1; off < 256; off <<= 1) {
+            const int add = (t < 256 && t + off < 256) ? hist[t + off] : 0;
+            __syncthreads();
+            if (t < 256) {
+                suf += add;
+                hist[t] = suf;
+            }
+            __syncthreads();
+        }
+        const int above = (t < 255) ? hist[t + 1] : 0;
+        __syncthreads();
+        if (t < 256 && suf >= rem && above < rem) {
+            s_remaining = rem - above;
+            s_prefix = prefix | ((unsigned long long)t << sh);
+        }
+        __syncthreads();
+    }
+    const unsigned long long kth = s_prefix;
+    const int want_eq = s_remaining;
+    const int cpt = (M + PRUNE_THREADS - 1) / PRUNE_THREADS;
+    const int j0 = t * cpt, j1 = min(M, j0 + cpt);
+    int ngt = 0, neq = 0;
+    for (int j = j0; j < j1; ++j) {
+        const unsigned long long k = keys[j];
+        ngt += k > kth;
+        neq += k == kth;
+    }
+    int tot_gt, tot_eq;
+    const int eq_off = prune_exscan(neq, scan, &tot_eq);
+    int take = 0, eqr = eq_off;
+    for (int j = j0; j < j1; ++j) {
+        const unsigned long long k = keys[j];
+        if (k > kth) ++take;
+        else if (k == kth) {
+            if (eqr < want_eq) ++take;
+            ++eqr;
+        }
+    }
+    (void)ngt;
+    const int off = prune_exscan(take, scan, &tot_gt);
+    int o = off;
+    eqr = eq_off;
+    for (int j = j0; j < j1; ++j) {
+        const unsigned long long k = keys[j];
+        bool in = k > kth;
+        if (k == kth) {
+            in = eqr < want_eq;
+            ++eqr;
+        }
+        insel[j] = in ? 1 : 0;
+        if (in) {
+            if (o < K) sel[o] = j;
+            ++o;
+        }
+    }
+}
+
+__global__ __launch_bounds__(256) void prune_gather_kernel(const int* __restrict__ list, int n, const double* __restrict__ Craw, int Mp,
+                                                           int d, const double* __restrict__ mean_s, double* __restrict__ Cint, int Mpi,
+                                                           double* __restrict__ mean_int) {
+    const int i = blockIdx.x * 256 + threadIdx.x;
+    if (i >= Mpi) return;
+    const int j = i < n ? list[i] : -1;
+    for (int k = 0; k < d; ++k) Cint[(size_t)k * Mpi + i] = j >= 0 ? Craw[(size_t)k * Mp + j] : 0.0;
+    if (mean_int) mean_int[i] = (j >= 0 && mean_s) ? mean_s[j] : 0.0;
+}
+
+__device__ __forceinline__ void prune_exact_reduce(const int* __restrict__ list, int n, const double* __restrict__ imu,
+                                                   const double* __restrict__ ivar, const double* __restrict__ mua,
+                                                   const unsigned char* __restrict__ mask, const EiPar& par, const PrunePar& pp,
+                                                   double* sv, long* si, double& bv, long& bi, int* bad) {
+    constexpr long NONE = 0x7fffffffffffffffL;
+    const int t = threadIdx.x;
+    double v = -INFINITY;
+    long ix = NONE;
+    for (int i = t; i < n; i += PRUNE_THREADS) {
+        const long j = list[i];
+        const double m = imu[i];
+        double e = ei_value_one(m, ivar[i], par);
+        if (mask && !mask[j]) e = 0.0;
+        else if (!(fabs(pp.coef) * fabs(mua[j] - m) <= 0.1 * prune_dmu(pp, pp.coef * m)) && m == m) atomicOr(bad, 1);
+        if (ix == NONE || better(e, j, v, ix)) {
+            v = e;
+            ix = j;
+        }
+    }
+    sv[t] = v;
+    si[t] = ix;
+    __syncthreads();
+    for (int st = PRUNE_THREADS / 2; st > 0; st >>= 1) {
+        if (t < st) {
+            const double ov = sv[t + st];
+            const long oi = si[t + st];
+            if (oi != NONE && (si[t] == NONE || better(ov, oi, sv[t], si[t]))) {
+                sv[t] = ov;
+                si[t] = oi;
+            }
+        }
+        __syncthreads();
+    }
+    bv = sv[0];
+    bi = si[0];
+    __syncthreads();
+}
+
+__device__ __forceinline__ bool prune_survives(double u, double T, long iT, long j, bool masked) {
+    if (!masked && T < 2.2250738585072014e-308) u += 64 * 4.9406564584124654e-324;
+    if (u < T) return false;
+    if (u > T || u != u || j < iT) return true;
+    return !(masked || T >= 2.2250738585072014e-308);
+}
+
+__global__ __launch_bounds__(PRUNE_THREADS) void prune_decide_kernel(const int* __restrict__ sel, int K, const double* __restrict__ imu,
+                                                                     const double* __restrict__ ivar, const double* __restrict__ mua,
+                                                                     const unsigned char* __restrict__ mask, EiPar par, PrunePar pp, int M,
+                                                                     const double* __restrict__ ub, const unsigned char* __restrict__ insel,
+                                                                     int* __restrict__ surv, double* __restrict__ tpair,
+                                                                     double* __restrict__ res, unsigned long long res_seq) {
+    __shared__ double sv[PRUNE_THREADS];
+    __shared__ long si[PRUNE_THREADS];
+    __shared__ int scan[PRUNE_THREADS];
+    __shared__ int bad;
+    const int t = threadIdx.x;
+    if (t == 0) bad = 0;
+    __syncthreads();
+    double T;
+    long iT;
+    prune_exact_reduce(sel, K, imu, ivar, mua, mask, par, pp, sv, si, T, iT, &bad);
+    const int cpt = (M + PRUNE_THREADS - 1) / PRUNE_THREADS;
+    const int j0 = t * cpt, j1 = min(M, j0 + cpt);
+    int cnt = 0;
+    for (int j = j0; j < j1; ++j) cnt += (!insel[j] && prune_survives(ub[j], T, iT, j, mask && !mask[j])) ? 1 : 0;
+    int total;
+    int o = prune_exscan(cnt, scan, &total);
+    for (int j = j0; j < j1; ++j)
+        if (!insel[j] && prune_survives(ub[j], T, iT, j, mask && !mask[j])) surv[o++] = j;
+    if (t == 0) {
+        tpair[0] = T;
+        reinterpret_cast<long*>(tpair)[1] = iT;
+        res[0] = T;
+        reinterpret_cast<long*>(res)[1] = iT;
+        reinterpret_cast<long*>(res)[2] = total;
+        reinterpret_cast<long*>(res)[3] = bad;
+        __threadfence_system();
+        __hip_atomic_store(reinterpret_cast<unsigned long long*>(res) + 4, res_seq, __ATOMIC_RELAXED, __HIP_MEMORY_SCOPE_SYSTEM);
+    }
+}
+
+__global__ __launch_bounds__(PRUNE_THREADS) void prune_merge_kernel(const int* __restrict__ surv, int n, const double* __restrict__ imu,
+                                                                    const double* __restrict__ ivar, const double* __restrict__ mua,
+                                                                    const unsigned char* __restrict__ mask, EiPar par, PrunePar pp,
+                                                                    const double* __restrict__ tpair, double* __restrict__ res,
+                                                                    unsigned long long res_seq) {
+    __shared__ double sv[PRUNE_THREADS];
+    __shared__ long si[PRUNE_THREADS];
+    __shared__ int bad;
+    if (threadIdx.x == 0) bad = 0;
+    __syncthreads();
+    double v;
+    long iv;
+    prune_exact_reduce(surv, n, imu, ivar, mua, mask, par, pp, sv, si, v, iv, &bad);
+    if (threadIdx.x == 0) {
+        const double T = tpair[0];
+        const long iT = reinterpret_cast<const long*>(tpair)[1];
+        if (!better(v, iv, T, iT)) {
+            v = T;
+            iv = iT;
+        }
+        res[0] = v;
+        reinterpret_cast<long*>(res)[1] = iv;
+        reinterpret_cast<long*>(res)[2] = n;
+        reinterpret_cast<long*>(res)[3] = bad;
+        __threadfence_system();
+        __hip_atomic_store(reinterpret_cast<unsigned long long*>(res) + 4, res_seq, __ATOMIC_RELAXED, __HIP_MEMORY_SCOPE_SYSTEM);
+    }
+}
+
+}
```

New measurement: 910.4 updates/s, median of 6. +1.8%, better.
